# ZYM-PKU/UDiffText

Hardware: AMD Instinct MI355X
Metric: 512x512 50-step denoised images/sec (UDiffText hot path: conditioner + 50 CFG Euler steps + VAE decode) (higher is better)
Workload: dtype bf16; 1 GPU; 512x512, 50 Euler/DDIM(eta 0) steps, CFG 5.0, 9-char labels, noise_iters 0; global batch 4 per step sharded over 1 GPU(s) = 4 images per GPU in micro-batches of 4: every UNet call runs ONE batch of 4 (8 samples with CFG); 3 such batch(es) in flight per GPU on separate launch streams; BASELINE.json configs[1]; global_batch=4, weights=synthetic (name-keyed recipe), 1361.2 M parameters, launch=hipGraph replay of the sampler steps, in_flight=3, batches_per_unet_call=1

## Files before the change

### include/udt_kernels.h

```cpp
#ifndef UDT_KERNELS_H
#define UDT_KERNELS_H

#include <stddef.h>
#include <stdint.h>

#ifdef __cplusplus
extern "C" {
#endif

typedef enum {
  UDT_OK = 0,
  UDT_ERR_BAD_SHAPE = -1,
  UDT_ERR_BAD_ARG = -2,
  UDT_ERR_WORKSPACE = -3,
  UDT_ERR_HIP = -4,
  UDT_ERR_NO_DEVICE = -5,
  UDT_ERR_ASYNC = -6
} udt_status;

typedef enum {
  UDT_DTYPE_F32 = 0,
  UDT_DTYPE_BF16 = 1,
  UDT_DTYPE_FP8_E4M3 = 2
} udt_dtype;

#define UDT_GEMM_OUT_F32     (1 << 0)
#define UDT_GEMM_GEGLU       (1 << 1)
#define UDT_GEMM_RELU        (1 << 2)
#define UDT_GEMM_TRANSPOSED  (1 << 3)
#define UDT_GEMM_CONV        (1 << 4)
#define UDT_GEMM_SILU_OUT    (1 << 5)
#define UDT_GEMM_MX8         (1 << 7)

typedef struct {
  const void* a;
  const void* a2;
  const void* w;
  const float* bias;
  const void* residual;
  const float* rowvec;
  void* out;
  int32_t M, N, K;
  int32_t lda, ldo, ldr;
  int32_t ldw;
  int32_t batch;
  int64_t stride_a, stride_w, stride_out, stride_res;
  int32_t Hin, Win, C1, C2, Hout, Wout;
  int32_t ksize;
  int32_t stride;
  int32_t pad_t, pad_l;
  int32_t upsample;
  int32_t rows_per_batch;
  int32_t ld_rowvec;
  int32_t flags;
  float alpha;
  const float* colscale;
  const float* in_scsh;
  int32_t in_act;
  float* colstats;
  int32_t cu_share;
  const float* ln_colsum;
  float ln_eps;
  const void* a_scale;
  void* q8_out;
  void* q8_scale;
  int32_t ld_q8;
  int32_t q8_fixed_col;
  float q8_fixed_mul;
  float* rowstat_out;
  const float* rowstat_in;
  int32_t rowstat_in_parts;
} udt_gemm_desc;

size_t udt_gemm_workspace_bytes(const udt_gemm_desc* d);
int udt_gemm(const udt_gemm_desc* d, void* workspace, size_t workspace_bytes, void* stream);
int32_t udt_gemm_colstats_rows(const udt_gemm_desc* d);
int32_t udt_gemm_rowstat_parts(const udt_gemm_desc* d);
int32_t udt_gemm_q8_ok(const udt_gemm_desc* d);
int32_t udt_gemm_colstats_slots(const udt_gemm_desc* d);
int32_t udt_gemm_in_scsh_ok(const udt_gemm_desc* d);
int32_t udt_gemm_up4_ok(const udt_gemm_desc* d);
int udt_gn_silu_conv3x3_fwd(const udt_gemm_desc* d, void* workspace, size_t workspace_bytes, void* stream);
int udt_ln_gemm_fwd(const udt_gemm_desc* d, void* workspace, size_t workspace_bytes, void* stream);
int udt_check_async_error(void* workspace, size_t workspace_bytes, void* stream);

int udt_attn_fwd(const void* q, const void* k, const void* vt, void* o,
                 int32_t batch, int32_t heads, int32_t nq, int32_t nk,
                 int32_t ldq, int32_t ldk, int32_t ldvt, int32_t ldo,
                 int64_t q_bstride, int64_t k_bstride, int64_t vt_bstride, int64_t o_bstride,
                 float scale, void* stream);

int udt_xattn_fwd(const void* q, const void* k, const void* v, void* o, float* probs,
                  int32_t batch, int32_t heads, int32_t head_dim, int32_t nq, int32_t L,
                  int32_t ldq, int32_t ldkv, int32_t ldo, float scale, void* stream);

int udt_attn_rowv_fwd(const void* q, const void* k, const void* v, void* o,
                      int32_t batch, int32_t heads, int32_t nq, int32_t nk,
                      int32_t ldq, int32_t ldk, int32_t ldv, int32_t ldo,
                      int64_t q_bstride, int64_t k_bstride, int64_t v_bstride, int64_t o_bstride,
                      float scale, void* stream);
int udt_attn_rowv_q8_fwd(const void* q, const void* k, const void* v, void* o,
                         int32_t batch, int32_t heads, int32_t nq, int32_t nk,
                         int32_t ldq, int32_t ldk, int32_t ldv, int32_t ldo,
                         int64_t q_bstride, int64_t k_bstride, int64_t v_bstride, int64_t o_bstride,
                         float scale, void* q8_out, void* q8_scale, int32_t ld_q8, void* stream);

int udt_attn_mx8_fwd(const void* qkv8, const void* qkv_scale, void* o, int32_t batch, int32_t heads, int32_t n,
                     int32_t ld8, int32_t ldo, float scale, float v_inv, void* q8_out, void* q8_scale, int32_t ld_q8,
                     void* stream);

int udt_attn512_fwd(const void* q, const void* k, const void* v, void* o,
                    int32_t batch, int32_t nq, int32_t nk,
                    int32_t ldq, int32_t ldk, int32_t ldv, int32_t ldo,
                    int64_t q_bstride, int64_t k_bstride, int64_t v_bstride, int64_t o_bstride,
                    float scale, void* stream);

size_t udt_attn512_workspace_bytes(int32_t batch, int32_t nq, int32_t nk);
int udt_attn512_split_fwd(const void* q, const void* k, const void* v, void* o,
                          int32_t batch, int32_t nq, int32_t nk,
                          int32_t ldq, int32_t ldk, int32_t ldv, int32_t ldo,
                          int64_t q_bstride, int64_t k_bstride, int64_t v_bstride, int64_t o_bstride,
                          float scale, void* workspace, size_t workspace_bytes, void* stream);

int udt_mattn_fwd(const void* q, const void* k, const void* v, void* o, const float* mask, const uint8_t* kpm,
                  int32_t batch, int32_t heads, int32_t head_dim, int32_t nq, int32_t lk,
                  int32_t ldq, int32_t ldk, int32_t ldv, int32_t ldo, int32_t ldmask,
                  int64_t q_bstride, int64_t k_bstride, int64_t v_bstride, int64_t o_bstride, float scale, void* stream);

int32_t udt_tattn_hp(int32_t heads);
int udt_tattn_prepare(const void* kv, int32_t ldkv, const void* wq, int32_t ldwq, const void* wo, int32_t ldwo,
                      const float* gamma, const float* beta, void* A, float* sc, void* BmT, int32_t B, int32_t L,
                      int32_t C, int32_t heads, float scale, void* stream);
int udt_tattn_fused(const void* x, void* out, const void* A, const float* sc, const void* BmT, const float* bias,
                    int32_t B, int32_t n_tok, int32_t C, int32_t heads, int32_t zero_samples, float eps, void* stream);
int32_t udt_tattn_rowstat_parts(int32_t B, int32_t n_tok, int32_t C);
int udt_tattn_fused_q8(const void* x, void* out, const void* A, const float* sc, const void* BmT, const float* bias,
                       int32_t B, int32_t n_tok, int32_t C, int32_t heads, int32_t zero_samples, float eps, void* q8_out,
                       void* q8_scale, float* rowstat_out, void* stream);
int udt_tattn_fused_maps(const void* x, void* out, const void* A, const float* sc, const void* BmT, const float* bias,
                         int32_t B, int32_t n_tok, int32_t C, int32_t heads, int32_t zero_samples, float eps, float* maps,
                         int32_t L, int32_t map_from, float weight, int32_t accumulate, void* q8_out, void* q8_scale,
                         float* rowstat_out, void* stream);

int udt_softmax_rows(void* x, int64_t rows, int32_t cols, int32_t ld, void* stream);

int32_t udt_gn_nchunks(int64_t HW, int32_t C);
int udt_gn_stats(const void* x, const void* x2, float* partials, int32_t B, int64_t HW, int32_t C, int32_t C2,
                 int32_t G, void* stream);
int udt_gn_apply(const void* x, const void* x2, void* y, const float* partials, const float* gamma,
                 const float* beta, int32_t B, int64_t HW, int32_t C, int32_t C2, int32_t G, float eps, int32_t act,
                 void* stream);
int32_t udt_gn_strip_ok(int32_t B, int64_t HW, int32_t C1, int32_t C2, int32_t G);
int udt_gn_strip(const void* x, const void* x2, void* y, const float* gamma, const float* beta, int32_t B, int64_t HW,
                 int32_t C1, int32_t C2, int32_t G, float eps, int32_t act, void* stream);

int udt_gn_finalize(const float* stats1, int32_t slots1, int32_t C1, const float* stats2, int32_t slots2, int32_t C2,
                    const float* gamma, const float* beta, float* scsh, int32_t B, int64_t HW, int32_t G, float eps,
                    void* stream);

int udt_gn_apply_scsh(const void* x, const void* x2, void* y, const float* scsh, int32_t B, int64_t HW, int32_t C1,
                      int32_t C2, int32_t act, void* stream);

int udt_gn_strip_stats(const void* x, const void* x2, void* y, const float* stats1, int32_t slots1, const float* stats2,
                       int32_t slots2, const float* gamma, const float* beta, int32_t B, int64_t HW, int32_t C1, int32_t C2,
                       int32_t G, float eps, int32_t act, void* stream);

int udt_layernorm(const void* x, void* y, const float* gamma, const float* beta,
                  int64_t rows, int32_t C, float eps, void* stream);
int udt_unet_input(const float* x, void* xin, int32_t B, int32_t hw, int32_t cpad, float c_in, void* stream);
int udt_unet_input_churn(float* x, const float* noise, void* xin, int32_t B, int32_t hw, int32_t cpad, float c_in, float kn,
                         void* stream);
int udt_cfg_euler_step(float* x, const float* eps, float* denoised_out, int32_t B, int32_t hw, int32_t ld_eps,
                       float c_out, float sigma, float sigma_next, float cfg_scale, void* stream);
typedef struct {
  float kx, kd, ka, kp, kn;
  float c_out, scale;
} udt_sampler_coefs;
int udt_cfg_sampler_step(const float* xin, const float* eps, const float* aux, const float* prev, const float* noise,
                         float* xout, float* denoised_out, int32_t B, int32_t hw, int32_t ld_eps, udt_sampler_coefs k,
                         void* stream);
#define UDT_MULTISTEP_MAX 8
typedef struct {
  float c_out, scale, sigma;
  int32_t n;
  float k[UDT_MULTISTEP_MAX];
  const float* hist[UDT_MULTISTEP_MAX];
} udt_multistep_coefs;
// ... 178 lines not shown
```

### udifftext_amd/csrc/gemm.hip

```cpp
#include "common.h"
#include <stdio.h>
#include <stdlib.h>
#include <string.h>
#include <atomic>
#include <cmath>

hipError_t udt_lean_launch_gemm(int cfg, const void* lparams, int smem, int G, int geglu, int ln, hipStream_t s);
hipError_t udt_lean_launch_conv3(const void* c3params, hipStream_t s);

namespace {
#include "tile_common.h"

struct GemmParams {
  const uint16_t* a;
  const uint16_t* a2;
  const uint16_t* w;
  const uint16_t* zero;
  const float* bias;
  const uint16_t* res;
  const float* rowvec;
  void* out;
  const float* colscale;
  const float* in_scsh;
  float* colstats;
// ... 345 lines not shown

template <int BM, int BN, int WGM, int WGN, bool TRANS>
__global__ void __launch_bounds__(256) gemm_fixup_kernel(const GemmParams p) {
  const int tile = blockIdx.x;
  const long long it0 = (long long)tile * p.n_ktiles;
  const long long it1 = it0 + p.n_ktiles;
  const int g_first = (int)(it0 / p.iters_per_wg);
  const int g_last = (int)((it1 - 1) / p.iters_per_wg);
  if (g_first == g_last) return;
  const int tid = threadIdx.x;
  const int wave = tid >> 6;
  const int lane = tid & 63;
  const int wm = (WGN == 1) ? wave : (wave >> 1);
  const int wn = (WGN == 1) ? 0 : ((WGM == 1) ? wave : (wave & 1));
  f32x16 acc[2][2];
#pragma unroll
  for (int i = 0; i < 2; ++i)
#pragma unroll
    for (int j = 0; j < 2; ++j)
#pragma unroll
      for (int r = 0; r < 16; ++r) acc[i][j][r] = 0.f;
  for (int g = g_first; g <= g_last; ++g) {
    const long long gb = (long long)g * p.iters_per_wg;
    const int slot = (it0 <= gb) ? 0 : 1;
    const f32x4* slab = reinterpret_cast<const f32x4*>(p.slabs) + ((long long)g * 2 + slot) * (16 * 256);
#pragma unroll
    for (int tm = 0; tm < 2; ++tm)
#pragma unroll
      for (int tn = 0; tn < 2; ++tn)
#pragma unroll
        for (int q = 0; q < 4; ++q) {
          const f32x4 v = slab[(tm * 8 + tn * 4 + q) * 256 + tid];
#pragma unroll
          for (int r = 0; r < 4; ++r) acc[tm][tn][q * 4 + r] += v[r];
        }
  }
  int batch, m0, n0;
  decode_tile<BM, BN>(p, tile, batch, m0, n0);
  epilogue<TRANS>(p, acc, m0, n0, batch, wm, wn, lane);
}

#include "gemm8.h"
#include "conv3p.h"
#include "conv_n4.h"
#include "lean_params.h"

struct TilePlan {
  int bm, bn;
  int tiles_m, tiles_n, tiles;
  int nkt;
  long long total;
  int G, ipw;
  bool fixup;
};

constexpr int MAX_DEVICES = 16;
std::atomic<int> g_dev_cus[MAX_DEVICES];

int device_cus() {
  int dev = 0;
  if (hipGetDevice(&dev) != hipSuccess || dev < 0 || dev >= MAX_DEVICES) return 256;
  int v = g_dev_cus[dev].load(std::memory_order_relaxed);
  if (v == 0) {
    v = 256;
    int q = 0;
    if (hipDeviceGetAttribute(&q, hipDeviceAttributeMultiprocessorCount, dev) == hipSuccess && q > 0) v = q;
    g_dev_cus[dev].store(v, std::memory_order_relaxed);
  }
  return v;
}

int resident_slots_all() { return 2 * device_cus(); }

int resident_slots(const udt_gemm_desc* d) {
  const int share = d->cu_share > 0 ? d->cu_share : 1;
  const int s = resident_slots_all() / share;
  return s < 2 ? 2 : s;
}

TilePlan plan_tiles(const udt_gemm_desc* d) {
  TilePlan t;
  const int batch = d->batch > 0 ? d->batch : 1;
  const bool tall = d->M >= 1024;
  if (d->N <= 64 || (tall && (d->N % 128) != 0 && (d->N % 128) <= 64)) {
    t.bm = 256; t.bn = 64;
  } else {
    t.bm = 128; t.bn = 128;
  }
  if (d->flags & (UDT_GEMM_TRANSPOSED | UDT_GEMM_GEGLU)) { t.bm = 128; t.bn = 128; }
  t.tiles_m = (d->M + t.bm - 1) / t.bm;
  t.tiles_n = (d->N + t.bn - 1) / t.bn;
  t.tiles = t.tiles_m * t.tiles_n * batch;
  t.nkt = d->K / BK;
  t.total = (long long)t.tiles * t.nkt;
  const int slots = resident_slots(d);
  const long long share = (t.total + slots - 1) / slots;
  if (t.tiles < slots / 2 && t.nkt >= 16) {
    long long G = t.total / 8;
    if (G < 1) G = 1;
    if (G > slots) G = slots;
    t.ipw = (int)((t.total + G - 1) / G);
  } else if (t.tiles >= 8 * slots) {
    t.ipw = ((t.tiles + slots - 1) / slots) * t.nkt;
  } else if (share >= 160 && (t.tiles % slots) != 0) {
    t.ipw = (int)share;
  } else {
    t.ipw = t.nkt;
  }
  t.G = (int)((t.total + t.ipw - 1) / t.ipw);
  t.fixup = (t.ipw % t.nkt) != 0;
  return t;
}

template <int BM, int BN, int WGM, int WGN, bool CONV, bool TRANS>
hipError_t launch_cfg(const GemmParams& p, const TilePlan& t, hipStream_t s) {
  constexpr int smem = 2 * (BM + BN) * ROW_BYTES;
  static AttrOnce once;
  auto kern = gemm_kernel<BM, BN, WGM, WGN, CONV, TRANS>;
  hipError_t e = once.ensure(reinterpret_cast<const void*>(kern), smem);
  if (e != hipSuccess) return e;
  hipLaunchKernelGGL(kern, dim3(t.G), dim3(256), smem, s, p);
  e = hipGetLastError();
  if (e != hipSuccess) return e;
  if (t.fixup) {
    hipLaunchKernelGGL((gemm_fixup_kernel<BM, BN, WGM, WGN, TRANS>), dim3(t.tiles), dim3(256), 0, s, p);
    e = hipGetLastError();
  }
  return e;
}

constexpr size_t G8_HEADER_BYTES = 4096;

std::atomic<int> g_n_block{-1};
std::atomic<int> g_rows_epi{1};
#ifdef UDT_MEASURE
std::atomic<int> g_dbg_bits{0};
#endif
constexpr int INTERNAL_DIRECT_EPI = 1 << 30;
constexpr int PUBLIC_FLAGS = UDT_GEMM_OUT_F32 | UDT_GEMM_GEGLU | UDT_GEMM_RELU | UDT_GEMM_TRANSPOSED | UDT_GEMM_CONV |
                             UDT_GEMM_SILU_OUT | UDT_GEMM_MX8;
inline int k_tile(const udt_gemm_desc* d) { return (d->flags & UDT_GEMM_MX8) ? 128 : BK; }
inline int elem_bytes(const udt_gemm_desc* d) { return (d->flags & UDT_GEMM_MX8) ? 1 : 2; }

bool use_gemm8(const udt_gemm_desc* d) {
  if (d->N <= 64) return false;
  const long long ldw = d->ldw > 0 ? d->ldw : d->K;
  if (!(d->flags & UDT_GEMM_CONV) && (long long)d->M * d->lda * elem_bytes(d) >= (1LL << 31)) return false;
  return (long long)d->N * ldw * elem_bytes(d) < (1LL << 31);
}


int round_workgroups(int G) { return G > 8 ? ((G + 7) & ~7) : G; }

bool prefer_whole_tiles(const udt_gemm_desc* d, int tiles) {
  if (d->cu_share <= 1) return false;
  return (long long)tiles * 4 >= (long long)(resident_slots(d) / 2) * 3;
}

TilePlan plan_tiles8(const udt_gemm_desc* d) {
  TilePlan t;
  const int batch = d->batch > 0 ? d->batch : 1;
  const bool geglu_or_trans = (d->flags & (UDT_GEMM_TRANSPOSED | UDT_GEMM_GEGLU)) != 0;
  t.bm = 256;
  t.bn = (!geglu_or_trans && d->N % 160 == 0 && d->N % 128 != 0) ? 160 : 128;
  t.tiles_m = (d->M + t.bm - 1) / t.bm;
  t.tiles_n = (d->N + t.bn - 1) / t.bn;
  t.tiles = t.tiles_m * t.tiles_n * batch;
  t.nkt = d->K / k_tile(d);
  t.total = (long long)t.tiles * t.nkt;
  const bool whole = t.nkt < 24 || prefer_whole_tiles(d, t.tiles);
  int slots = (whole ? resident_slots_all() : resident_slots(d)) / 2;
  long long G = t.total / 4;
  if (G < 1) G = 1;
  if (G > slots) G = slots;
  t.ipw = (int)((t.total + G - 1) / G);
  if (whole) t.ipw = ((t.ipw + t.nkt - 1) / t.nkt) * t.nkt;
  t.G = round_workgroups((int)((t.total + t.ipw - 1) / t.ipw));
  t.fixup = (t.ipw % t.nkt) != 0;
  return t;
}

template <int WGM, int WGN, int TM, int TN, bool CONV, bool TRANS, bool STATS = false>
hipError_t launch8(const g8::Params& pp, const TilePlan& t, hipStream_t s) {
  constexpr int BM = WGM * TM * 32, BN = WGN * TN * 32;
  constexpr int smem = (TM == 2 && TN == 2 && !TRANS) ? 160 * 1024 : g8::NSTAGE * (BM + BN) * ROW_BYTES;
  static AttrOnce once;
  auto kern = g8::gemm8_kernel<WGM, WGN, TM, TN, CONV, TRANS, STATS>;
  hipError_t e = once.ensure(reinterpret_cast<const void*>(kern), smem);
  if (e != hipSuccess) return e;
  hipLaunchKernelGGL(kern, dim3(t.G), dim3(g8::NTHREADS), smem, s, pp);
  return hipGetLastError();
}

bool conv3p_geometry(const udt_gemm_desc* d, c3p::Geo& ge, bool gn) {
  if (!gn) return false;
  if (!(d->flags & UDT_GEMM_CONV) || d->ksize != 3 || d->stride != 1) return false;
  const bool ups = d->upsample != 0;
  if (ups) return false;
  if (d->pad_t != 1 || d->pad_l != 1 || d->N <= 64) return false;
  if (d->Hout != (d->Hin << (ups ? 1 : 0)) || d->Wout != (d->Win << (ups ? 1 : 0))) return false;
  if (d->flags & (UDT_GEMM_GEGLU | UDT_GEMM_TRANSPOSED)) return false;
  if (d->C1 <= 0 || d->C1 % 64 != 0 || d->C2 < 0 || d->C2 % 64 != 0 || (d->C2 != 0 && !gn)) return false;
  const int H = d->Hout, W = d->Wout;
  if (W % 32 == 0 && H % 8 == 0) { ge.TW = 32; ge.TH = 8; ge.NI = 1; }
  else if (W % 16 == 0 && H % 16 == 0) { ge.TW = 16; ge.TH = 16; ge.NI = 1; }
  else if (W == 8 && H == 8 && !ups) { ge.TW = 8; ge.TH = 8; ge.NI = 4; }
  else return false;
  ge.B = d->M / (H * W);
  ge.H = d->Hin; ge.W = d->Win; ge.C1 = d->C1; ge.C2 = d->C2; ge.C = d->C1 + d->C2;
  ge.tiles_x = W / ge.TW;
  ge.tiles_y = H / ge.TH;
  ge.img_groups = (ge.B + ge.NI - 1) / ge.NI;
  ge.prow_w = (ups ? ge.TW / 2 : ge.TW) + 2;
  ge.prows_img = ((ups ? ge.TH / 2 : ge.TH) + 2) * ge.prow_w;
  ge.n_pieces = (ge.NI * ge.prows_img + 7) / 8;
  ge.chunks = ge.C / 64;
  if ((long long)d->M * d->C1 * 2 >= (1LL << 31) || (long long)d->M * d->C2 * 2 >= (1LL << 31) || d->M >= (1 << 28)) return false;
  if ((long long)d->N * (d->ldw > 0 ? d->ldw : d->K) * 2 >= (1LL << 31)) return false;
  if ((long long)ge.B * ge.chunks * 512 >= (1LL << 31)) return false;
  const int bn = (d->N % 160 == 0 && d->N % 128 != 0) ? 160 : 128;
  return ge.n_pieces * 8 <= c3p::patch_rows(bn == 160 ? 5 : 2, gn) && ge.n_pieces >= 8;
}

TilePlan plan_tiles3p(const udt_gemm_desc* d, const c3p::Geo& ge) {
  TilePlan t;
  t.bm = 256;
  t.bn = (d->N % 160 == 0 && d->N % 128 != 0) ? 160 : 128;
  t.tiles_m = ge.img_groups * ge.tiles_y * ge.tiles_x;
  t.tiles_n = (d->N + t.bn - 1) / t.bn;
  t.tiles = t.tiles_m * t.tiles_n;
  t.nkt = ge.chunks;
  t.total = (long long)t.tiles * t.nkt;
  const bool whole = t.nkt * 9 < 24 || prefer_whole_tiles(d, t.tiles);
  const int slots = (whole ? resident_slots_all() : resident_slots(d)) / 2;
  long long G = t.total;
  if (G > slots) G = slots;
  t.ipw = (int)((t.total + G - 1) / G);
  if (whole) t.ipw = ((t.ipw + t.nkt - 1) / t.nkt) * t.nkt;
  t.G = round_workgroups((int)((t.total + t.ipw - 1) / t.ipw));
  t.fixup = (t.ipw % t.nkt) != 0;
  return t;
}

template <int WGM, int WGN, int TM, int TN, bool GN, bool STATS, bool UPS = false>
hipError_t launch3p(const c3p::CParams& cp, const TilePlan& t, hipStream_t s) {
  constexpr int BN = WGN * TN * 32;
  constexpr int smem = g8::NSTAGE * BN * ROW_BYTES + 2 * c3p::patch_rows(TN, GN) * ROW_BYTES + (GN ? c3p::SCSH_BYTES : 0);
  static_assert(smem <= 160 * 1024, "one workgroup per CU: at most the CU's 160 KiB of LDS");
  static AttrOnce once;
  auto kern = c3p::conv3p_kernel<WGM, WGN, TM, TN, GN, STATS, UPS>;
  hipError_t e = once.ensure(reinterpret_cast<const void*>(kern), smem);
  if (e != hipSuccess) return e;
  hipLaunchKernelGGL(kern, dim3(t.G), dim3(g8::NTHREADS), smem, s, cp);
  return hipGetLastError();
}

struct LeanPlan;
bool lean_stats_probe(const udt_gemm_desc* d, int& rows, int& slots);
int colstats_rows(const udt_gemm_desc* d) {
  if (d->flags & (UDT_GEMM_OUT_F32 | UDT_GEMM_GEGLU | UDT_GEMM_TRANSPOSED)) return 0;
  if ((d->batch > 1) || d->M <= 0 || d->N <= 0 || d->K <= 0 || d->K % BK != 0) return 0;
  int rows = 0, slots = 0;
  if (lean_stats_probe(d, rows, slots)) return rows;
  c3p::Geo ge;
  if (conv3p_geometry(d, ge, d->in_scsh != nullptr)) {
    rows = (d->N % 160 == 0 && d->N % 128 != 0) ? 32 : 64;
    if ((ge.TW * ge.TH) % rows != 0) return 0;
  } else if (use_gemm8(d) && g_rows_epi.load(std::memory_order_relaxed)) {
    rows = (plan_tiles8(d).bn == 160) ? 32 : 64;
  } else {
    return 0;
  }
  const int rpb = d->rows_per_batch > 0 ? d->rows_per_batch : d->M;
  return (rpb % rows == 0) ? rows : 0;
}

int colstats_slots(const udt_gemm_desc* d) {
  const int rows = colstats_rows(d);
  if (rows == 0) return 0;
  int lrows = 0, lslots = 0;
  if (lean_stats_probe(d, lrows, lslots)) return lslots;
  c3p::Geo ge;
  if (conv3p_geometry(d, ge, d->in_scsh != nullptr)) return ge.img_groups * ge.tiles_y * ge.tiles_x * (256 / rows);
  return ((d->M + 255) / 256) * (256 / rows);
}


std::atomic<int> g_lean{-1};
std::atomic<int> g_lean_splitk{-2};
int lean_splitk_knob() {
  int v = g_lean_splitk.load(std::memory_order_relaxed);
  if (v == -2) {
    const char* e = getenv("UDT_LEAN_SPLITK");
    v = e ? atoi(e) : -1;
// ... 67 lines not shown
  if (d->residual || d->rowvec || d->in_scsh || d->colstats || d->colscale || d->batch > 1 || d->alpha != 1.0f) return false;
  if ((d->ldw > 0 ? d->ldw : d->K) % 8 != 0 || (d->ldw > 0 && d->ldw < d->K)) return false;
  if (d->K != 9 * d->C1 || (d->lda != 0 && d->lda != d->C1) || d->q8_out || d->q8_scale || d->rowstat_out || d->in_act != 0) return false;
  if ((reinterpret_cast<uintptr_t>(d->a) | reinterpret_cast<uintptr_t>(d->w) | reinterpret_cast<uintptr_t>(d->out)) & 15) return false;
  return true;
}

bool lean_plan(const udt_gemm_desc* d, LeanPlan& t, bool want_stats) {
  const int mode = lean_mode();
  if (mode == 0) return false;
  constexpr int unsupported = UDT_GEMM_OUT_F32 | UDT_GEMM_RELU | UDT_GEMM_TRANSPOSED | UDT_GEMM_SILU_OUT;
  if (d->flags & unsupported) return false;
  const bool conv1 = (d->flags & UDT_GEMM_CONV) != 0;
  if (conv1 && (d->ksize != 1 || d->stride != 1 || d->upsample || d->pad_t != 0 || d->pad_l != 0 || d->Hout != d->Hin ||
                d->Wout != d->Win || d->C1 % BK != 0 || d->C2 % BK != 0 || d->ln_colsum || (d->flags & UDT_GEMM_GEGLU)))
    return false;
  const bool mx8 = (d->flags & UDT_GEMM_MX8) != 0;
  const bool emit = d->q8_out != nullptr;
  if (d->batch > 1 || d->in_scsh || (d->colscale != nullptr) != mx8) return false;
  const bool geglu = (d->flags & UDT_GEMM_GEGLU) != 0;
  const bool ln = d->ln_colsum != nullptr;
  if (want_stats && (geglu || ln || !lean_stats_enabled())) return false;
  if (mx8 || emit) {
    if (conv1 || d->rowvec || mode == 0 || (mode > 0 && mode != 1)) return false;
    if (mx8 && (!d->a_scale || d->K % 128 != 0 || d->lda % 16 != 0 || (d->ldw > 0 && d->ldw % 16 != 0))) return false;
    if (mx8 && ln && (!d->rowstat_in || d->rowstat_in_parts <= 0)) return false;
    if (!mx8 && geglu) return false;
    if (mx8 && geglu && !(ln && emit)) return false;
    if (mx8 && !geglu && ln && emit && d->rowstat_out) return false;
    if (emit && (want_stats || !d->q8_scale || d->ld_q8 % 8 != 0 || d->N % (geglu ? 64 : 32) != 0)) return false;
    if (d->rowstat_out && (!emit || geglu)) return false;
    if (d->q8_fixed_col > 0 && (!emit || geglu || d->q8_fixed_col % 32 != 0 || !(d->q8_fixed_mul > 0.f))) return false;
    if ((reinterpret_cast<uintptr_t>(d->q8_out) | reinterpret_cast<uintptr_t>(d->colscale)) & 15) return false;
  } else if (d->rowstat_out || d->rowstat_in) {
    return false;
  }
  const int KT = mx8 ? 128 : BK;
  if (d->N <= 64 || d->N % 8 != 0 || d->K % KT != 0 || (!conv1 && d->lda % 8 != 0) || (d->ldo % 8 != 0 && d->out)) return false;
  if (d->residual && d->ldr % 8 != 0) return false;
  if (geglu && (d->N % 64 != 0 || d->residual || d->rowvec)) return false;
  const long long ldw = d->ldw > 0 ? d->ldw : d->K;
  const long long lda_eff = conv1 ? (d->C1 > d->C2 ? d->C1 : d->C2) : d->lda;
  if ((long long)d->M * lda_eff * 2 >= (1LL << 31) || (long long)d->N * ldw * 2 >= (1LL << 31)) return false;
  if (d->M >= (1 << 28)) return false;
  if ((reinterpret_cast<uintptr_t>(d->out) | reinterpret_cast<uintptr_t>(d->residual) | reinterpret_cast<uintptr_t>(d->bias) |
       reinterpret_cast<uintptr_t>(d->rowvec) | reinterpret_cast<uintptr_t>(d->ln_colsum)) & 15) return false;
  if (d->rowvec && ((d->ld_rowvec > 0 ? d->ld_rowvec : d->N) % 4 != 0)) return false;
  if (mode > 0 && mode != 1 && mode != 6 && mode != 7) return false;
  if (!mx8 && (!emit || (ln && !geglu && !d->rowstat_out)) && (mode == 7 || (mode < 0 && rowres_on()))) {
    const bool emit_fits = !emit || ((d->q8_fixed_col <= 0 || d->q8_fixed_col % 64 == 0) && (long long)d->M * d->ld_q8 < (1LL << 31) &&
                                     (long long)d->M * (d->out ? d->ldo : 0) * 2 < (1LL << 31) && (long long)((d->N + 127) / 128) * d->M * 4 < (1LL << 31));
    if (ln && !want_stats && d->K == 320 && d->N % 64 == 0 && !d->residual && !d->rowvec && !conv1 && emit_fits &&
        (reinterpret_cast<uintptr_t>(d->a) & 15) == 0) {
      const int tiles_m = (d->M + 255) / 256, chunks = d->N / 64;
      int ns = (device_cus() + tiles_m - 1) / tiles_m;
      if (ns > chunks / 4) ns = chunks / 4;
      const int cmax = geglu ? 20 : 16;
      const int ns_min = (chunks + cmax - 1) / cmax;
      if (ns < ns_min) ns = ns_min;
      const long long wgs = (long long)tiles_m * ns;
      if (ns >= 1 && (mode == 7 || emit || (geglu ? wgs * 4 >= 3LL * device_cus() : wgs >= device_cus()))) {
        t.cfg = 7; t.stats_rows = 0; t.nw = 4; t.bm = 256; t.bn = 64; t.smem = 0;
        t.tiles_m = tiles_m; t.kt_per = (chunks + ns - 1) / ns; t.tiles_n = (chunks + t.kt_per - 1) / t.kt_per;
        t.tiles = t.tiles_m * t.tiles_n; t.nkt = d->K / BK; t.splitk = 1; t.n_block = 1;
        t.G = round_workgroups(t.tiles);
        return true;
      }
    }
    if (mode == 7 || (emit && ln)) return false;
  }
  t.cfg = (mode > 0) ? mode : 1;
  if (!mx8 && !emit) {
  if (!geglu && d->N % 160 == 0 && d->N % 128 != 0 && t.cfg == 1) t.cfg = 5;
  if (mode <= 0 && d->N >= 768 && (long long)((d->M + 255) / 256) * ((d->N + 255) / 256) >= 2LL * device_cus() &&
      (d->cu_share <= 1 || lean256_under_lanes())) t.cfg = 6;
  }
  t.stats_rows = 0;
  if (want_stats) {
    if (t.cfg != 1 && t.cfg != 5) {
      if (mode > 0) return false;
      t.cfg = (d->N % 160 == 0 && d->N % 128 != 0) ? 5 : 1;
    }
    if (mx8) t.cfg = 1;
    t.stats_rows = t.cfg == 1 ? 64 : 32;
    const int rpb = d->rows_per_batch > 0 ? d->rows_per_batch : d->M;
    if (rpb % t.stats_rows != 0) return false;
  }
  switch (t.cfg) {
    case 1: t.nw = 4; t.bm = 128; t.bn = 128; t.smem = 2 * (128 + 128) * ROW_BYTES; break;
    case 5: t.nw = 4; t.bm = 128; t.bn = 160; t.smem = 128 * 160 * 4; break;
    case 6: t.nw = 8; t.bm = 256; t.bn = 256; t.smem = 2 * (256 + 256) * ROW_BYTES; break;
    default: return false;
  }
  {
    const int epi = (t.cfg == 6 ? t.bm * t.bn : t.bm * t.bn * 4) + ((ln && t.cfg != 5) ? t.bm * 8 : 0);
    if (t.smem < epi) t.smem = epi;
  }
  t.tiles_m = (d->M + t.bm - 1) / t.bm;
  t.tiles_n = (d->N + t.bn - 1) / t.bn;
  t.tiles = t.tiles_m * t.tiles_n;
  t.nkt = d->K / KT;
  int slots = device_cus() * ((t.cfg == 1 || t.cfg == 5) ? 2 : 1) / share_of(d);
  if (slots < 1) slots = 1;
  int sk = 1;
  const int knob = lean_splitk_knob();
  if (!ln && t.tiles <= 1023) {
    if (knob > 1) sk = knob;
    else if (knob < 0 && t.tiles * 2 <= slots && t.nkt >= (mx8 ? 20 : 40)) { sk = slots / t.tiles; if (sk > t.nkt / (mx8 ? 8 : 16)) sk = t.nkt / (mx8 ? 8 : 16); }
    if (sk > t.nkt / 4) sk = t.nkt / 4;
    while (sk > 1 && (long long)t.tiles * sk * t.bm * t.bn * 4 > (64LL << 20)) --sk;
    if (sk < 1) sk = 1;
  }
  t.kt_per = (t.nkt + sk - 1) / sk;
  t.splitk = (t.nkt + t.kt_per - 1) / t.kt_per;
  const int units = t.tiles * t.splitk;
  t.G = round_workgroups(units);
  int nb = g_n_block.load(std::memory_order_relaxed);
  if (nb <= 0) nb = (t.tiles_m <= 8) ? t.tiles_n : 8;
  if (nb > t.tiles_n) nb = t.tiles_n;
  t.n_block = nb;
  return true;
}

size_t lean_workspace(const LeanPlan& t) {
  return t.splitk > 1 ? G8_HEADER_BYTES + (size_t)t.tiles * t.splitk * t.bm * t.bn * sizeof(float) : 0;
}

std::atomic<int> g_lean_conv{-1};
std::atomic<int> g_wide_conv{-2};
int wide_conv_mode() {
  int v = g_wide_conv.load(std::memory_order_relaxed);
  if (v == -2) {
    const char* e = getenv("UDT_WIDE_CONV");
    v = e ? atoi(e) : -1;
    g_wide_conv.store(v, std::memory_order_relaxed);
  }
  return v;
}
#ifdef UDT_MEASURE
std::atomic<int> g_lconv_dbg{0};
#endif

std::atomic<int> g_wide_lanes_eff{-2};
double wide_lanes_eff() {
  int v = g_wide_lanes_eff.load(std::memory_order_relaxed);
  if (v == -2) {
    const char* e = getenv("UDT_WIDE_LANES_EFF");
    v = e ? atoi(e) : 70;
    g_wide_lanes_eff.store(v, std::memory_order_relaxed);
  }
  return v / 100.0;
}

int conv_chunk_slices(long long tiles, int slots, int chunks, int knob) {
  long long sk = 1;
  if (tiles <= 1023) {
    if (knob > 1) { sk = knob; if (sk > chunks) sk = chunks; }
    else if (knob < 0 && tiles * 2 <= slots && chunks >= 10) { sk = slots / tiles; if (sk > chunks / 4) sk = chunks / 4; }
    if (sk < 1) sk = 1;
  }
  return (int)sk;
}

bool lean_conv_plan(const udt_gemm_desc* d, lg::C3Params& c, bool want_stats) {
  int on = g_lean_conv.load(std::memory_order_relaxed);
  if (on < 0) {
    const char* e = getenv("UDT_LEAN_CONV");
    on = (e && e[0] == '0') ? 0 : 1;
    g_lean_conv.store(on, std::memory_order_relaxed);
  }
  if (!on || lean_mode() == 0) return false;
  if (d->flags != UDT_GEMM_CONV || d->ksize != 3 || d->stride != 1 || d->pad_t != 1 || d->pad_l != 1) return false;
  if (d->C2 != 0 || d->in_scsh || d->colscale || d->batch > 1) return false;
  if (want_stats && !lean_stats_enabled()) return false;
  if (d->N < 128 || d->N % 8 != 0 || d->C1 <= 0 || d->C1 % 64 != 0) return false;
  if (d->upsample != 0 && d->upsample != 1 && d->upsample != 2) return false;
  const bool phase = d->upsample == 2, ups = d->upsample == 1;
  const int nph = phase ? 4 : 1;
  if (d->Hout != (d->Hin << (d->upsample ? 1 : 0)) || d->Wout != (d->Win << (d->upsample ? 1 : 0))) return false;
  if (phase && d->ldw > 0 && d->ldw < 4 * d->C1) return false;
  const int Ht = phase ? d->Hin : d->Hout, Wt = phase ? d->Win : d->Wout;
  c.bn = 128; c.wgm = 2;
  bool wide = false;
  int wide_slots = device_cus();
  {
    const int wm = wide_conv_mode();
    if (wm != 0 && !ups && d->N % 160 == 0 && Wt % 16 == 0 && Ht % 16 == 0) {
      const int cus = device_cus(), share = d->cu_share > 1 ? d->cu_share : 1;
      wide_slots = cus / share > 0 ? cus / share : 1;
      const long long wt = (long long)(d->M / 256) * (d->N / 160);
      const long long sk = conv_chunk_slices(wt, wide_slots, d->C1 / 64, lean_splitk_knob());
      const long long units = wt * sk;
      const long long rounds = (units + cus - 1) / cus;
      const double eff = units > cus ? (double)units / (double)(rounds * cus) : ((double)units * share >= cus ? 1.0 : (double)units * share / cus);
      wide = (wm > 0) || (sk <= 2 && eff >= ((share >= 3 && share_of(d) >= 3) ? wide_lanes_eff() : 0.85));
    }
  }
  if (wide) { c.geo = phase ? 6 : 3; c.tw = 16; c.th = 16; c.bn = 160; c.wgm = 4; }
  else if (Wt % 16 == 0 && Ht % 8 == 0) { c.geo = ups ? 2 : phase ? 4 : 0; c.tw = 16; c.th = 8; }
  else if (!ups && Wt % 8 == 0 && Ht % 8 == 0) { c.geo = phase ? 5 : 1; c.tw = 8; c.th = 8; }
  else return false;
  if (d->ldo % 8 != 0 || (d->residual && d->ldr % 8 != 0)) return false;
  const long long ldw = d->ldw > 0 ? d->ldw : (phase ? 4LL * d->C1 : (long long)d->K);
  if (ldw % 8 != 0) return false;
  c.w_phase = phase ? (d->stride_w > 0 ? d->stride_w : (long long)d->N * ldw) : 0;
  if (phase && (c.w_phase < (long long)d->N * ldw || c.w_phase % 8 != 0)) return false;
  if ((long long)d->M * d->C1 * 2 >= (1LL << 31) || (long long)d->N * ldw * 2 >= (1LL << 31)) return false;
  if ((reinterpret_cast<uintptr_t>(d->out) | reinterpret_cast<uintptr_t>(d->residual) | reinterpret_cast<uintptr_t>(d->bias) |
       reinterpret_cast<uintptr_t>(d->rowvec)) & 15) return false;
  if (d->rowvec && ((d->ld_rowvec > 0 ? d->ld_rowvec : d->N) % 4 != 0)) return false;
  c.dbg = 0;
#ifdef UDT_MEASURE
  c.dbg = g_lconv_dbg.load(std::memory_order_relaxed);
#endif
  c.N = d->N; c.C = d->C1; c.H = d->Hin; c.W = d->Win; c.B = d->M / (d->Hout * d->Wout);
  c.ldw = (int)ldw; c.ldo = d->ldo; c.ldr = d->ldr; c.ldrv = d->ld_rowvec > 0 ? d->ld_rowvec : d->N;
  c.alpha = d->alpha;
  c.tiles_x = Wt / c.tw; c.tiles_y = Ht / c.th;
  c.tiles_m = c.B * c.tiles_x * c.tiles_y;
  c.tiles_n = (d->N + c.bn - 1) / c.bn;
  c.tiles = c.tiles_m * c.tiles_n;
  c.chunks = c.C / 64;
  const int slots = wide ? wide_slots : (2 * device_cus() / share_of(d) > 0 ? 2 * device_cus() / share_of(d) : 1);
  int sk = conv_chunk_slices((long long)c.tiles * nph, slots, c.chunks, lean_splitk_knob());
  while (sk > 1 && (long long)c.tiles * nph * sk * c.tw * c.th * c.bn * 4 > (64LL << 20)) --sk;
  c.ch_per = (c.chunks + sk - 1) / sk;
  c.splitk = (c.chunks + c.ch_per - 1) / c.ch_per;
  c.G = round_workgroups(c.tiles * nph * c.splitk);
  {
    const double patch = (double)((ups ? c.tw / 2 : c.tw) + 2) * ((ups ? c.th / 2 : c.th) + 2) * c.C * 2.0, wtile = (phase ? 4.0 : 9.0) * c.bn * c.C * 2.0;
    int nb = g_n_block.load(std::memory_order_relaxed);
    if (nb <= 0) nb = (int)(std::sqrt(64.0 * patch / wtile) + 0.5);
    if (nb < 1) nb = 1;
    if (nb > c.tiles_n) nb = c.tiles_n;
    c.n_block = nb;
  }
  c.a_bytes = (unsigned)((long long)c.B * d->Hin * d->Win * d->C1 * 2);
  c.w_bytes = (unsigned)((long long)d->N * ldw * 2);
  c.counters = nullptr; c.slabs = nullptr;
  return true;
}

int lean_conv_phases(const lg::C3Params& c) { return c.geo >= 4 ? 4 : 1; }

size_t lean_conv_workspace(const lg::C3Params& c) {
  return c.splitk > 1 ? G8_HEADER_BYTES + (size_t)c.tiles * lean_conv_phases(c) * c.splitk * c.tw * c.th * c.bn * sizeof(float) : 0;
}

bool lean_stats_probe(const udt_gemm_desc* d, int& rows, int& slots) {
  if (d->in_scsh) return false;
  {
    lg::C3Params c3;
    if (lean_conv_plan(d, c3, true)) {
      rows = c3.tw * c3.th / c3.wgm;
      slots = c3.tiles_m * c3.wgm * lean_conv_phases(c3);
      return true;
    }
  }
  if ((d->flags & UDT_GEMM_CONV) && d->ksize == 3) return false;
  LeanPlan lt;
  if (lean_plan(d, lt, true)) {
    rows = lt.stats_rows;
    slots = lt.tiles_m * (lt.bm / lt.stats_rows);
    return true;
  }
  return false;
}
}

extern "C" int udt_debug_set(const char* key, int32_t value) {
  if (!key) return UDT_ERR_BAD_ARG;
  if (!strcmp(key, "n_block")) { g_n_block.store(value); return UDT_OK; }
  if (!strcmp(key, "rows_epi")) { g_rows_epi.store(value ? 1 : 0); return UDT_OK; }
  if (!strcmp(key, "lean")) { g_lean.store(value < 0 ? -2 : value); return UDT_OK; }
  if (!strcmp(key, "rowres")) { g_rowres.store(value < 0 ? 1 : (value ? 1 : 0)); return UDT_OK; }
  if (!strcmp(key, "wide_lanes_eff")) { g_wide_lanes_eff.store(value < 0 ? -2 : value); return UDT_OK; }
  if (!strcmp(key, "conv_n4")) { g_conv_n4.store(value < 0 ? -2 : (value ? 1 : 0)); return UDT_OK; }
  if (!strcmp(key, "lean256_lanes")) { g_lean256_lanes.store(value < 0 ? -2 : (value ? 1 : 0)); return UDT_OK; }
// ... 88 lines not shown
      return G8_HEADER_BYTES + (size_t)t3.G * t3.bm * t3.bn * sizeof(float);
    }
  }
  if (use_gemm8(d)) {
    TilePlan t8 = plan_tiles8(d);
    if (!t8.fixup) return 0;
    return G8_HEADER_BYTES + (size_t)t8.G * t8.bm * t8.bn * sizeof(float);
  }
  TilePlan t = plan_tiles(d);
  if (t.bm != 256 || !t.fixup) return 0;
  return G8_HEADER_BYTES + (size_t)t.G * 2 * SLAB_FLOATS * sizeof(float);
}

extern "C" int udt_gemm(const udt_gemm_desc* d, void* workspace, size_t workspace_bytes, void* stream) {
  if (!d || !d->a || !d->w) return UDT_ERR_BAD_ARG;
  if (d->M <= 0 || d->N <= 0 || d->K <= 0) return UDT_ERR_BAD_SHAPE;
  if (d->K % k_tile(d) != 0) return UDT_ERR_BAD_SHAPE;
  if (d->N % 4 != 0) return UDT_ERR_BAD_SHAPE;
  const bool mx8 = (d->flags & UDT_GEMM_MX8) != 0;
  if (mx8 || d->q8_out || d->rowstat_out || d->rowstat_in) {
    LeanPlan lt8;
    if (!lean_plan(d, lt8, d->colstats != nullptr)) return UDT_ERR_BAD_ARG;
  } else if (d->colscale) {
    return UDT_ERR_BAD_ARG;
  }
  const bool conv = (d->flags & UDT_GEMM_CONV) != 0;
  const bool trans = (d->flags & UDT_GEMM_TRANSPOSED) != 0;
  const int batch = d->batch > 0 ? d->batch : 1;
  if (conv) {
    if (d->ksize != 1 && d->ksize != 3) return UDT_ERR_BAD_SHAPE;
    if (d->C1 <= 0 || d->C1 % BK != 0 || d->C2 % BK != 0) return UDT_ERR_BAD_SHAPE;
    if (d->C2 > 0 && !d->a2) return UDT_ERR_BAD_ARG;
    if (d->K != d->ksize * d->ksize * (d->C1 + d->C2)) return UDT_ERR_BAD_SHAPE;
    if (d->Hout <= 0 || d->Wout <= 0 || d->M % (d->Hout * d->Wout) != 0) return UDT_ERR_BAD_SHAPE;
    if (d->stride != 1 && d->stride != 2) return UDT_ERR_BAD_SHAPE;
    if (trans || batch != 1) return UDT_ERR_BAD_ARG;
  } else {
    if (d->lda < d->K || d->lda % 8 != 0) return UDT_ERR_BAD_SHAPE;
  }
  if (!d->out && !d->q8_out) return UDT_ERR_BAD_ARG;
  if (trans) {
    if (d->rows_per_batch <= 0 || d->rows_per_batch % 4 != 0 || d->M % d->rows_per_batch != 0)
      return UDT_ERR_BAD_SHAPE;
    if (d->flags & (UDT_GEMM_OUT_F32 | UDT_GEMM_GEGLU | UDT_GEMM_RELU | UDT_GEMM_SILU_OUT)) return UDT_ERR_BAD_ARG;
    if (d->residual || d->rowvec || batch != 1) return UDT_ERR_BAD_ARG;
  } else {
    if (d->ldo % 4 != 0) return UDT_ERR_BAD_SHAPE;
    if (d->residual && d->ldr % 4 != 0) return UDT_ERR_BAD_SHAPE;
  }
  if (d->flags & UDT_GEMM_GEGLU) {
    if (d->N % 64 != 0 || (d->flags & UDT_GEMM_OUT_F32) || d->residual || d->rowvec) return UDT_ERR_BAD_ARG;
  }
  if (d->rowvec && d->rows_per_batch <= 0) return UDT_ERR_BAD_ARG;

  hipStream_t s = reinterpret_cast<hipStream_t>(stream);
  if (conv_n4_applies(d)) {
    cn4::Params cp;
    cp.a = reinterpret_cast<const uint16_t*>(d->a); cp.w = reinterpret_cast<const uint16_t*>(d->w); cp.bias = d->bias;
    cp.out = reinterpret_cast<float*>(d->out);
    cp.B = d->M / (d->Hout * d->Wout); cp.H = d->Hin; cp.W = d->Win; cp.C = d->C1;
    cp.ldw = d->ldw > 0 ? d->ldw : d->K; cp.ldo = d->ldo;
    cp.tiles_x = (d->Win + 7) / 8; cp.tiles_y = (d->Hin + 7) / 8;
    const size_t smem = (size_t)100 * (d->C1 + 8) * 2 + (size_t)4 * 9 * d->C1 * 2;
    static AttrOnce once;
    hipError_t ea = once.ensure(reinterpret_cast<const void*>(cn4::conv3x3_n4_kernel), 100 * (512 + 8) * 2 + 4 * 9 * 512 * 2);
    if (ea != hipSuccess) return udt_set_hip_error(ea);
    UdtProfScope profn(0, s);
    if (profn.rec) {
      char tag[96];
      snprintf(tag, sizeof(tag), "conv_n4 M=%d N=%d K=%d %dx%d", d->M, d->N, d->K, d->Hin, d->Win);
      udt_prof_tag(profn.rec, tag);
    }
    hipLaunchKernelGGL(cn4::conv3x3_n4_kernel, dim3((unsigned)(cp.B * cp.tiles_x * cp.tiles_y)), dim3(256), smem, s, cp);
    UDT_CHECK_LAUNCH();
    return UDT_OK;
  }
  TilePlan t = plan_tiles(d);

  GemmParams p;
  p.a = reinterpret_cast<const uint16_t*>(d->a);
  p.a2 = reinterpret_cast<const uint16_t*>(d->a2);
  p.w = reinterpret_cast<const uint16_t*>(d->w);
  p.zero = udt_zero_page();
  if (!p.zero) return UDT_ERR_HIP;
  p.bias = d->bias;
  p.res = reinterpret_cast<const uint16_t*>(d->residual);
  p.rowvec = d->rowvec;
  p.out = d->out;
  p.colscale = d->colscale;
  p.in_scsh = d->in_scsh;
  p.in_act = d->in_act;
  p.colstats = d->colstats;
  p.slabs = nullptr;
  if (d->colstats && colstats_rows(d) == 0) return UDT_ERR_BAD_ARG;
  if (d->in_scsh && !udt_gemm_in_scsh_ok(d)) return UDT_ERR_BAD_ARG;
  if (d->in_act != 0 && d->in_act != 1) return UDT_ERR_BAD_ARG;
  p.M = d->M; p.N = d->N; p.K = d->K;
  p.lda = d->lda; p.ldo = d->ldo; p.ldr = d->ldr;
  p.ldw = d->ldw > 0 ? d->ldw : d->K;
  if (d->upsample == 2) {
    if (!udt_gemm_up4_ok(d)) return UDT_ERR_BAD_SHAPE;
  } else if (p.ldw < d->K || p.ldw % 8 != 0) return UDT_ERR_BAD_SHAPE;
  if (mx8 && d->lda < d->K) return UDT_ERR_BAD_SHAPE;
  p.sA = d->stride_a; p.sW = d->stride_w; p.sO = d->stride_out; p.sR = d->stride_res;
  p.Hin = d->Hin; p.Win = d->Win; p.C1 = d->C1; p.C2 = d->C2; p.Hout = d->Hout; p.Wout = d->Wout;
  p.ksz = d->ksize; p.stride = d->stride; p.pad_t = d->pad_t; p.pad_l = d->pad_l; p.ups = d->upsample ? 1 : 0;
  p.rows_per_batch = d->rows_per_batch > 0 ? d->rows_per_batch : d->M;
  p.ldrv = d->ld_rowvec > 0 ? d->ld_rowvec : d->N;
  if (d->flags & ~PUBLIC_FLAGS) return UDT_ERR_BAD_ARG;
  p.flags = d->flags | (g_rows_epi.load(std::memory_order_relaxed) ? 0 : INTERNAL_DIRECT_EPI);
#ifdef UDT_MEASURE
  p.flags |= g_dbg_bits.load(std::memory_order_relaxed);
#endif
  p.n_block = 1;
  p.alpha = d->alpha;
  const int cls = (conv && d->ksize == 3) ? 0 : 1;
  {
    LeanPlan lt;
    if (lean_plan(d, lt, d->colstats != nullptr)) {
      lg::LParams lp;
      lp.colstats = d->colstats;
      const bool conv1 = (d->flags & UDT_GEMM_CONV) != 0;
      lp.a = p.a; lp.a2 = (conv1 && d->C2 > 0) ? p.a2 : nullptr; lp.w = p.w; lp.bias = p.bias; lp.res = p.res; lp.rowvec = p.rowvec;
      lp.ln_s = d->ln_colsum;
      lp.out = reinterpret_cast<uint16_t*>(d->out);
      lp.M = d->M; lp.N = d->N; lp.K = d->K;
      lp.lda = conv1 ? d->C1 : p.lda; lp.ldw = p.ldw; lp.ldo = p.ldo; lp.ldr = p.ldr; lp.ldrv = p.ldrv; lp.rows_per_batch = p.rows_per_batch;
      lp.lda2 = conv1 ? d->C2 : 0;
      lp.kt_split = (conv1 && d->C2 > 0) ? d->C1 / BK : lt.nkt;
      lp.a2_bytes = (unsigned)((long long)d->M * (conv1 ? d->C2 : 0) * 2);
      lp.alpha = d->alpha; lp.ln_eps = d->ln_eps;
      lp.tiles_m = lt.tiles_m; lp.tiles_n = lt.tiles_n; lp.n_block = lt.n_block; lp.tiles = lt.tiles;
      lp.nkt = lt.nkt; lp.splitk = lt.splitk; lp.kt_per = lt.kt_per;
      lp.a_bytes = (unsigned)((long long)d->M * lp.lda * elem_bytes(d));
      lp.w_bytes = (unsigned)((long long)d->N * p.ldw * elem_bytes(d));
      lp.a_scale = mx8 ? reinterpret_cast<const uint32_t*>(d->a_scale) : nullptr;
      lp.colscale = d->colscale;
      lp.rowstat_in = d->rowstat_in; lp.rowstat_in_parts = d->rowstat_in_parts;
      lp.q8_out = reinterpret_cast<uint8_t*>(d->q8_out); lp.q8_scale = reinterpret_cast<uint32_t*>(d->q8_scale); lp.ld_q8 = d->ld_q8;
      lp.rowstat_out = d->rowstat_out;
      lp.q8_fixed_col = d->q8_fixed_col > 0 ? d->q8_fixed_col : 0x7fffffff;
      lp.q8_fixed_mul = d->q8_fixed_mul;
      lp.G = lt.G;
      lp.counters = nullptr; lp.slabs = nullptr;
      if (lt.splitk > 1) {
        if (!workspace || workspace_bytes < lean_workspace(lt)) return UDT_ERR_WORKSPACE;
        lp.counters = reinterpret_cast<int*>(workspace);
        lp.slabs = reinterpret_cast<float*>(reinterpret_cast<char*>(workspace) + G8_HEADER_BYTES);
      }
      UdtProfScope profl(cls, s);
      if (profl.rec) {
        char tag[96];
        snprintf(tag, sizeof(tag), "lean%d%s%s M=%d N=%d K=%d fl=0x%x ln=%d tile=%dx%d units=%d splitk=%d", lt.cfg, mx8 ? "-mx8" : "", d->q8_out ? "+q8" : "",
                 d->M, d->N, d->K, d->flags, d->ln_colsum ? 1 : 0, lt.bm, lt.bn, lt.tiles * lt.splitk, lt.splitk);
        udt_prof_tag(profl.rec, tag);
      }
      const bool geglu = (d->flags & UDT_GEMM_GEGLU) != 0, ln = d->ln_colsum != nullptr;
      hipError_t el;
      el = udt_lean_launch_gemm(lt.cfg, &lp, lt.smem, lt.G, geglu ? 1 : 0, ln ? 1 : 0, s);
      if (el != hipSuccess) return udt_set_hip_error(el);
      return UDT_OK;
    }
  }
  if (d->ln_colsum) return UDT_ERR_BAD_ARG;
  {
    lg::C3Params c3;
    if (lean_conv_plan(d, c3, d->colstats != nullptr)) {
      c3.colstats = d->colstats;
      c3.a = p.a; c3.w = p.w; c3.bias = p.bias; c3.res = p.res; c3.rowvec = p.rowvec; c3.out = reinterpret_cast<uint16_t*>(d->out);
      if (c3.splitk > 1) {
        if (!workspace || workspace_bytes < lean_conv_workspace(c3)) return UDT_ERR_WORKSPACE;
        c3.counters = reinterpret_cast<int*>(workspace);
        c3.slabs = reinterpret_cast<float*>(reinterpret_cast<char*>(workspace) + G8_HEADER_BYTES);
      }
      UdtProfScope profc(cls, s);
      if (profc.rec) {
        char tag[96];
        snprintf(tag, sizeof(tag), "%s%s M=%d N=%d K=%d %dx%d tile=%dx%d units=%d splitk=%d nb=%d%s", (c3.geo == 3 || c3.geo == 6) ? "wconv3" : "lconv3",
                 (d->upsample && c3.geo != 6) ? "+up" : "", d->M, d->N, d->K,
                 d->Hin, d->Win, c3.tw, c3.th, c3.tiles * lean_conv_phases(c3) * c3.splitk, c3.splitk, c3.n_block,
                 d->upsample == 2 ? " up4" : "");
        udt_prof_tag(profc.rec, tag);
      }
      const hipError_t ec = udt_lean_launch_conv3(&c3, s);
      if (ec != hipSuccess) return udt_set_hip_error(ec);
      return UDT_OK;
    }
  }
  {
    c3p::CParams cp;
    if (conv3p_geometry(d, cp.geo, d->in_scsh != nullptr)) {
      const TilePlan t3 = plan_tiles3p(d, cp.geo);
      p.tiles_m = t3.tiles_m; p.tiles_n = t3.tiles_n; p.tiles_per_batch = t3.tiles_m * t3.tiles_n;
      {
        const double patch = (double)cp.geo.prows_img * cp.geo.NI * cp.geo.C * 2.0;
        const double wtile = 9.0 * t3.bn * cp.geo.C * 2.0;
        const double S = (double)(t3.tiles < t3.G ? t3.tiles : t3.G) / 8.0;
        int nb = (int)(std::sqrt((S < 1.0 ? 1.0 : S) * patch / wtile) + 0.5);
        if (nb < 1) nb = 1;
        if (nb > t3.tiles_n) nb = t3.tiles_n;
        p.n_block = nb;
      }
      p.n_ktiles = t3.nkt;
      p.total_iters = t3.total;
      p.iters_per_wg = t3.ipw;
      p.G = t3.G;
      const long long in_px = (long long)cp.geo.B * d->Hin * d->Win;
      cp.base.a_bytes = (unsigned)(in_px * d->C1 * 2);
      cp.a2_bytes = (unsigned)((long long)d->M * d->C2 * 2);
      cp.scsh_bytes = (unsigned)((long long)cp.geo.B * cp.geo.chunks * 512);
      cp.base.w_bytes = (unsigned)((long long)d->N * p.ldw * 2);
      cp.base.g = p;
      cp.base.flags = nullptr; cp.base.err = nullptr; cp.base.slab_base = nullptr;
      if (t3.fixup) {
        const size_t need = G8_HEADER_BYTES + (size_t)t3.G * t3.bm * t3.bn * sizeof(float);
        if (!workspace || workspace_bytes < need) return UDT_ERR_WORKSPACE;
        cp.base.flags = reinterpret_cast<int*>(workspace);
        cp.base.err = cp.base.flags + 1023;
        cp.base.slab_base = reinterpret_cast<float*>(reinterpret_cast<char*>(workspace) + G8_HEADER_BYTES);
      }
      UdtProfScope prof3(cls, s);
      if (prof3.rec) {
        char tag[96];
        snprintf(tag, sizeof(tag), "conv3p%s%s M=%d N=%d K=%d %dx%d tile=%dx%dx%d bn=%d G=%d ipw=%d", d->in_scsh ? "+gn" : "", d->upsample ? "+up" : "", d->M,
                 d->N, d->K, d->Hin, d->Win, cp.geo.TW, cp.geo.TH, cp.geo.NI, t3.bn, t3.G, t3.ipw);
        udt_prof_tag(prof3.rec, tag);
      }
      hipError_t e3;
      const bool st3 = d->colstats != nullptr;
      if (t3.bn == 160) e3 = st3 ? launch3p<8, 1, 1, 5, true, true>(cp, t3, s) : launch3p<8, 1, 1, 5, true, false>(cp, t3, s);
      else e3 = st3 ? launch3p<4, 2, 2, 2, true, true>(cp, t3, s) : launch3p<4, 2, 2, 2, true, false>(cp, t3, s);
      if (e3 != hipSuccess) return udt_set_hip_error(e3);
      return UDT_OK;
    }
  }
  if (use_gemm8(d)) {
    const TilePlan t8 = plan_tiles8(d);
    p.tiles_m = t8.tiles_m; p.tiles_n = t8.tiles_n; p.tiles_per_batch = t8.tiles_m * t8.tiles_n;
    const int n_block_knob = g_n_block.load(std::memory_order_relaxed);
    if (n_block_knob != 0 && !conv) {
      const long long wt = (long long)t8.bn * d->K * elem_bytes(d);
      long long nb = 1;
      if (n_block_knob > 0) nb = n_block_knob;
      else if (t8.tiles_m <= 8 || trans) nb = t8.tiles_n;
      else if (t8.tiles_n >= 8) nb = (4LL << 20) / (wt > 0 ? wt : 1);
      if (nb < 1) nb = 1;
      if (nb > t8.tiles_n) nb = t8.tiles_n;
      p.n_block = (int)nb;
    }
    p.n_ktiles = t8.nkt;
    p.total_iters = t8.total;
    p.iters_per_wg = t8.ipw;
    p.G = t8.G;
    g8::Params pp;
    pp.g = p;
    pp.flags = nullptr; pp.err = nullptr; pp.slab_base = nullptr;
    pp.a_bytes = conv ? 0u : (unsigned)((long long)d->M * d->lda * elem_bytes(d));
    pp.w_bytes = (unsigned)((long long)d->N * p.ldw * elem_bytes(d));
    if (t8.fixup) {
      const size_t need = G8_HEADER_BYTES + (size_t)t8.G * t8.bm * t8.bn * sizeof(float);
      if (!workspace || workspace_bytes < need) return UDT_ERR_WORKSPACE;
      pp.flags = reinterpret_cast<int*>(workspace);
      pp.err = pp.flags + 1023;
      pp.slab_base = reinterpret_cast<float*>(reinterpret_cast<char*>(workspace) + G8_HEADER_BYTES);
    }
    UdtProfScope prof8(cls, s);
    if (prof8.rec) {
      char tag[96];
      snprintf(tag, sizeof(tag), "gemm8 M=%d N=%d K=%d conv=%d ks=%d fl=0x%x tile=%dx%d G=%d ipw=%d b=%d",
               d->M, d->N, d->K, conv ? 1 : 0, d->ksize, d->flags, t8.bm, t8.bn, t8.G, t8.ipw, batch);
      udt_prof_tag(prof8.rec, tag);
    }
    hipError_t e8;
    const bool st = d->colstats != nullptr;
    if (t8.bn == 160) {
      if (st) e8 = conv ? launch8<8, 1, 1, 5, true, false, true>(pp, t8, s) : launch8<8, 1, 1, 5, false, false, true>(pp, t8, s);
      else e8 = conv ? launch8<8, 1, 1, 5, true, false>(pp, t8, s) : launch8<8, 1, 1, 5, false, false>(pp, t8, s);
    } else if (trans) {
      e8 = launch8<4, 2, 2, 2, false, true>(pp, t8, s);
    } else if (st) {
      e8 = conv ? launch8<4, 2, 2, 2, true, false, true>(pp, t8, s) : launch8<4, 2, 2, 2, false, false, true>(pp, t8, s);
    } else {
      e8 = conv ? launch8<4, 2, 2, 2, true, false>(pp, t8, s) : launch8<4, 2, 2, 2, false, false>(pp, t8, s);
    }
    if (e8 != hipSuccess) return udt_set_hip_error(e8);
    return UDT_OK;
  }

  p.tiles_m = t.tiles_m; p.tiles_n = t.tiles_n; p.tiles_per_batch = t.tiles_m * t.tiles_n;
  p.n_ktiles = t.nkt;
  p.total_iters = t.total;
  p.iters_per_wg = t.ipw;
  p.G = t.G;

  if (t.fixup) {
    const size_t need = G8_HEADER_BYTES + (size_t)t.G * 2 * SLAB_FLOATS * sizeof(float);
    if (!workspace || workspace_bytes < need) return UDT_ERR_WORKSPACE;
    p.slabs = reinterpret_cast<float*>(reinterpret_cast<char*>(workspace) + G8_HEADER_BYTES);
  }

  UdtProfScope prof(cls, s);
  if (prof.rec) {
    char tag[96];
    snprintf(tag, sizeof(tag), "gemm M=%d N=%d K=%d conv=%d ks=%d fl=0x%x tile=%dx%d G=%d ipw=%d b=%d", d->M, d->N, d->K,
             conv ? 1 : 0, d->ksize, d->flags, t.bm, t.bn, t.G, t.ipw, batch);
    udt_prof_tag(prof.rec, tag);
  }

  if (t.bm != 256) return UDT_ERR_BAD_SHAPE;
  const hipError_t e = conv ? launch_cfg<256, 64, 4, 1, true, false>(p, t, s) : launch_cfg<256, 64, 4, 1, false, false>(p, t, s);
  if (e != hipSuccess) return udt_set_hip_error(e);
  return UDT_OK;
}
```

### udifftext_amd/csrc/lean.h

```cpp
#pragma once

namespace lg {

using g8::wait_vm;
UDT_DEVINL void raw_barrier() {
  asm volatile("s_waitcnt lgkmcnt(0)" ::: "memory");
  __builtin_amdgcn_s_barrier();
  asm volatile("" ::: "memory");
}
using g8::buf_lds16;
using g8::OOB;

typedef __attribute__((ext_vector_type(2))) __bf16 bf2_t;
UDT_DEVINL float dot2_bf16(uint32_t a, uint32_t b, float c) {
  return __builtin_amdgcn_fdot2_f32_bf16(__builtin_bit_cast(bf2_t, a), __builtin_bit_cast(bf2_t, b), c, false);
}

template <int CPR, int RPI>
UDT_DEVINL void wave_colstats(char* wl, int lane, const float (&cs)[8], const float (&cq)[8], float* dst, bool col_ok) {
#pragma unroll
  for (int h = 0; h < 2; ++h) {
    f32x4 a = {cs[4 * h + 0], cs[4 * h + 1], cs[4 * h + 2], cs[4 * h + 3]};
    f32x4 b = {cq[4 * h + 0], cq[4 * h + 1], cq[4 * h + 2], cq[4 * h + 3]};
    *reinterpret_cast<f32x4*>(wl + lane * 64 + h * 16) = a;
// ... 404 lines not shown
        uint32_t sb;
        const u32x2 q8 = mx8_quant_row8(f, sb);
        if (m < p.M && col_ok) {
          *reinterpret_cast<u32x2*>(p.q8_out + (long long)m * p.ld_q8 + n_out) = q8;
          if (ch == 0) reinterpret_cast<uint8_t*>(p.q8_scale)[((long long)(n_out >> 7) * p.M + m) * 4 + ((n_out >> 5) & 3)] = (uint8_t)sb;
          if (p.out) *reinterpret_cast<u32x4*>(p.out + (long long)m * p.ldo + n_out) = v;
        }
      } else {
        if (m < p.M && col_ok) *reinterpret_cast<u32x4*>(p.out + (long long)m * p.ldo + n_out) = v;
      }
    }
  } else {
    char* const wl = smem + wave * EPI_WAVE;
    constexpr int PROWS = TMB * 32;
    constexpr int CPR = TN * 4;
    constexpr int RPI = 64 / CPR;
    constexpr int NIT = (PROWS + RPI - 1) / RPI;
    const int rl = lane / CPR;
    const int c8 = lane - rl * CPR;
    const int n = n0 + col0 + c8 * 8;
    const bool col_ok = (rl < RPI) && (n < p.N);
    f32x4 b0 = {0.f, 0.f, 0.f, 0.f}, b1 = b0, s0 = b0, s1 = b0;
    if (p.bias && col_ok) {
      b0 = *reinterpret_cast<const f32x4*>(p.bias + n);
      b1 = *reinterpret_cast<const f32x4*>(p.bias + n + 4);
    }
    if constexpr (LN) {
      if (col_ok) {
        s0 = *reinterpret_cast<const f32x4*>(p.ln_s + n);
        s1 = *reinterpret_cast<const f32x4*>(p.ln_s + n + 4);
      }
    }
    f32x4 w0 = {1.f, 1.f, 1.f, 1.f}, w1 = w0;
    if constexpr (FP8) {
      if (col_ok) {
        w0 = *reinterpret_cast<const f32x4*>(p.colscale + n);
        w1 = *reinterpret_cast<const f32x4*>(p.colscale + n + 4);
      }
    }
    float cs[8], cq[8];
#pragma unroll
    for (int j = 0; j < 8; ++j) cs[j] = cq[j] = 0.f;
#pragma unroll
    for (int pass = 0; pass < TM / TMB; ++pass) {
      const int prow0 = pass * PROWS;
      u32x4 rv[NIT];
      if (p.res) {
#pragma unroll
        for (int i = 0; i < NIT; ++i) {
          const int row = i * RPI + rl;
          const int m = m0 + row0 + prow0 + row;
          u32x4 z = {0u, 0u, 0u, 0u};
          rv[i] = z;
          if (col_ok && row < PROWS && m < p.M) rv[i] = *reinterpret_cast<const u32x4*>(p.res + (long long)m * p.ldr + n);
        }
      }
#pragma unroll
      for (int tb = 0; tb < TMB; ++tb) {
        const int row = tb * 32 + l31;
#pragma unroll
        for (int tn = 0; tn < TN; ++tn)
#pragma unroll
          for (int q = 0; q < 4; ++q) {
            const int chunk = (tn * 8 + q * 2 + hi) ^ (row & 7);
            const f32x16& a16 = acc[pass * TMB + tb][tn];
            f32x4 v = {a16[q * 4 + 0], a16[q * 4 + 1], a16[q * 4 + 2], a16[q * 4 + 3]};
            *reinterpret_cast<f32x4*>(wl + row * EROW + chunk * 16) = v;
          }
      }
#pragma unroll
      for (int i = 0; i < NIT; ++i) {
        const int row = i * RPI + rl;
        const int m = m0 + row0 + prow0 + row;
        const bool ok = col_ok && row < PROWS && m < p.M;
        const int rr = row < PROWS ? row : 0;
        const char* rp = wl + rr * EROW;
        const int sw = rr & 7;
        const f32x4 v0 = *reinterpret_cast<const f32x4*>(rp + (((2 * c8) ^ sw) << 4));
        const f32x4 v1 = *reinterpret_cast<const f32x4*>(rp + (((2 * c8 + 1) ^ sw) << 4));
        float o[8];
#pragma unroll
        for (int j = 0; j < 4; ++j) {
          o[j] = v0[j];
          o[4 + j] = v1[j];
        }
        if constexpr (FP8) {
#pragma unroll
          for (int j = 0; j < 4; ++j) o[j] *= w0[j], o[4 + j] *= w1[j];
        }
        if constexpr (LN) {
          float mean, rstd;
          row_stats(prow0 + rr, mean, rstd);
#pragma unroll
          for (int j = 0; j < 4; ++j) {
            o[j] = rstd * (o[j] - mean * s0[j]);
            o[4 + j] = rstd * (o[4 + j] - mean * s1[j]);
          }
        }
#pragma unroll
        for (int j = 0; j < 4; ++j) {
          o[j] = o[j] * p.alpha + b0[j];
          o[4 + j] = o[4 + j] * p.alpha + b1[j];
        }
        if (p.rowvec && ok) {
          const float* rvp = p.rowvec + (long long)(m / p.rows_per_batch) * p.ldrv + n;
          const f32x4 r0 = *reinterpret_cast<const f32x4*>(rvp);
          const f32x4 r1 = *reinterpret_cast<const f32x4*>(rvp + 4);
// ... 412 lines not shown
```

### udifftext_amd/csrc/lean_params.h

```cpp
#pragma once

namespace lg {

struct LParams {
  const uint16_t* a;
  const uint16_t* a2;
  const uint16_t* w;
  const float* bias;
  const uint16_t* res;
  const float* rowvec;
  const float* ln_s;
  uint16_t* out;
  int M, N, K;
  int lda, ldw, ldo, ldr, ldrv, rows_per_batch;
  float alpha, ln_eps;
  int tiles_m, tiles_n, n_block, tiles;
  int nkt;
  int splitk, kt_per;
  unsigned a_bytes, w_bytes;
  int kt_split, lda2;
  unsigned a2_bytes;
  int G;
  int* counters;
  float* slabs;
  float* colstats;
  const uint32_t* a_scale;
  const float* colscale;
  const float* rowstat_in;
  int rowstat_in_parts;
  uint8_t* q8_out;
  uint32_t* q8_scale;
  int ld_q8;
  int q8_fixed_col;
  float q8_fixed_mul;
  float* rowstat_out;
};

struct C3Params {
  const uint16_t* a;
  const uint16_t* w;
  const float* bias;
  const uint16_t* res;
  const float* rowvec;
  uint16_t* out;
  int N, C;
  int B, H, W;
  int ldw, ldo, ldr, ldrv;
  float alpha;
  int tiles_x, tiles_y, tiles_m, tiles_n, n_block, tiles;
  int chunks, splitk, ch_per;
  unsigned a_bytes, w_bytes;
  int G;
  int* counters;
  float* slabs;
  float* colstats;
  int geo, tw, th;
  int bn, wgm;
  long long w_phase;
  int dbg;
};

}
```

### udifftext_amd/csrc/tattn.hip

```cpp
#include "common.h"
#include <stdio.h>
#include <stdlib.h>

namespace {

constexpr int TA_THREADS = 512;
constexpr int TA_WAVES = TA_THREADS / 64;

struct TattnParams {
  const uint16_t* x;
  uint16_t* out;
  const uint16_t* A;
  const float* sc;
  const uint16_t* BmT;
  const float* bias;
  const uint16_t* zero;
  int M, C, hp, n_tok, zero_samples;
  int nsplit;
  float eps;
  uint8_t* q8_out;
  uint32_t* q8_scale;
  float* rowstat_out;
  float* maps;
  int heads, map_L, map_from, map_acc;
  float map_scale;
};

UDT_DEVINL f32x16 zero16() {
  f32x16 z;
#pragma unroll
  for (int r = 0; r < 16; ++r) z[r] = 0.f;
  return z;
}

template <int TT, int NKT, int NKS, bool Q8 = false, bool MAPS = false>
__global__ void __launch_bounds__(TA_THREADS) tattn_fused_kernel(const TattnParams p) {
  extern __shared__ __attribute__((aligned(16))) char smem[];
  constexpr int C = NKT * 64, hp = NKS * 16;
  constexpr int nkt = NKT;
  constexpr int TA_AHEAD = NKT <= 10 ? NKT : 8;
  char* const xs = smem;
  float* const stats = reinterpret_cast<float*>(smem + (size_t)nkt * TT * 128);
  const int prs = hp * 2 + 16;
  char* const pl = reinterpret_cast<char*>(stats + TT * 2);
  const int tid = threadIdx.x;
  const int wave = __builtin_amdgcn_readfirstlane(tid >> 6);
  const int lane = tid & 63;
  const int l31 = lane & 31, hi = lane >> 5;
  const long long tok0 = (long long)blockIdx.x * TT;
  const int b = (int)(tok0 / p.n_tok);
  const uint16_t* xg = p.x + tok0 * C;
  uint16_t* og = p.out + tok0 * C;
  float* const rst = reinterpret_cast<float*>(pl + (size_t)TT * prs);
  const int ct_lo = (int)blockIdx.y * (C >> 5) / p.nsplit, ct_hi = ((int)blockIdx.y + 1) * (C >> 5) / p.nsplit;
  auto q8_row_stats = [&]() {
    __syncthreads();
    if (tid < TT && tok0 + tid < p.M) {
      float s = 0.f, q = 0.f;
      for (int ct = ct_lo; ct < ct_hi; ++ct) {
        const f32x2 v = *reinterpret_cast<const f32x2*>(rst + ((size_t)tid * (C >> 5) + ct) * 2);
        s += v[0];
        q += v[1];
      }
      f32x2 o = {s, q};
      reinterpret_cast<f32x2*>(p.rowstat_out)[(long long)blockIdx.y * p.M + tok0 + tid] = o;
    }
  };


  const uint16_t* Ab = p.A + (long long)b * hp * C;
  constexpr int jt = hp >> 5;
  constexpr int tiles1 = jt * (TT / 32);
  bf16x8_t ar[TA_AHEAD][4];
  const bool live = b >= p.zero_samples;
  if (live && wave < tiles1) {
    const uint16_t* arow = Ab + (long long)(wave / (TT / 32)) * (32 * C) + lane * 8;
#pragma unroll
    for (int u = 0; u < TA_AHEAD; ++u)
#pragma unroll
      for (int ks = 0; ks < 4; ++ks) ar[u][ks] = *reinterpret_cast<const bf16x8_t*>(arow + (u * 4 + ks) * 512);
  }

  {
    const int pieces = nkt * (TT / 8);
    const int l3 = lane >> 3, ps = lane & 7;
    for (int pc = wave; pc < pieces; pc += TA_WAVES) {
      const int kt = pc / (TT / 8), rg = pc - kt * (TT / 8);
      const int row = rg * 8 + l3;
      const int slot = ps ^ ((row >> 1) & 7);
      const uint16_t* src = (tok0 + row < p.M) ? (xg + (long long)row * C + kt * 64 + slot * 8) : p.zero;
      glds16(src, xs + (size_t)pc * 1024);
    }
    wait_vmcnt0();
  }
  __syncthreads();

  if (b < p.zero_samples) {
    const int ch_lo = ct_lo * 4, ch_hi = ct_hi * 4;
    const int nch = ch_hi - ch_lo;
    for (int i0 = 0; i0 < TT * nch; i0 += TA_THREADS) {
      const int i = i0 + tid;
      const bool act = i < TT * nch;
      const int row = act ? i / nch : 0, ch = ch_lo + (act ? i - row * nch : 0);
      const bool ok = act && tok0 + row < p.M;
// ... 244 lines not shown
  const long long idx = (long long)blockIdx.x * 256 + threadIdx.x;
  if (idx >= (long long)B * C * hp) return;
  const int j = (int)(idx % hp);
  const long long bc = idx / hp;
  const int c = (int)(bc % C), b = (int)(bc / C);
  const int h = j >> 4, i = j & 15;
  float a = 0.f;
  if (h < heads && i < L) {
    const uint16_t* vr = kv + ((long long)b * L + i) * ldkv + v_off + h * 64;
    const uint16_t* wr = wo + (long long)c * ldwo + h * 64;
#pragma unroll 8
    for (int d = 0; d < 64; ++d) a += bf16_bits_to_f32(vr[d]) * bf16_bits_to_f32(wr[d]);
  }
  const long long off = ((((long long)(c >> 5) * (hp >> 4) + (j >> 4)) * 64) + ((j >> 3) & 1) * 32 + (c & 31)) * 8 + (j & 7);
  BmT[(long long)b * C * hp + off] = (uint16_t)(pack_bf16x2(a, 0.f) & 0xffffu);
}

}

extern "C" int32_t udt_tattn_hp(int32_t heads) { return ((heads * 16 + 31) / 32) * 32; }

extern "C" int udt_tattn_prepare(const void* kv, int32_t ldkv, const void* wq, int32_t ldwq, const void* wo, int32_t ldwo,
                                 const float* gamma, const float* beta, void* A, float* sc, void* BmT, int32_t B, int32_t L,
                                 int32_t C, int32_t heads, float scale, void* stream) {
  if (!kv || !wq || !wo || !gamma || !beta || !A || !sc || !BmT) return UDT_ERR_BAD_ARG;
  if (B <= 0 || L <= 0 || L > 12 || heads <= 0 || C != heads * 64 || ldkv < 2 * C || ldwq < C || ldwo < C) return UDT_ERR_BAD_SHAPE;
  const int hp = udt_tattn_hp(heads);
  hipStream_t s = reinterpret_cast<hipStream_t>(stream);
  UdtProfScope prof(3, s);
  hipLaunchKernelGGL(tattn_prepare_a_kernel, dim3(hp, B), dim3(256), 0, s, reinterpret_cast<const uint16_t*>(kv), ldkv,
                     reinterpret_cast<const uint16_t*>(wq), ldwq, gamma, beta, reinterpret_cast<uint16_t*>(A), sc, L, C, hp, heads, scale);
  UDT_CHECK_LAUNCH();
  const long long n = (long long)B * C * hp;
  hipLaunchKernelGGL(tattn_prepare_b_kernel, dim3((unsigned)((n + 255) / 256)), dim3(256), 0, s,
                     reinterpret_cast<const uint16_t*>(kv), ldkv, C, reinterpret_cast<const uint16_t*>(wo), ldwo,
                     reinterpret_cast<uint16_t*>(BmT), B, L, C, hp, heads);
  UDT_CHECK_LAUNCH();
  return UDT_OK;
}

namespace {
int tattn_tt(int C) { return C >= 640 ? 32 : 64; }
int tattn_nsplit(int M, int TT) {
  const unsigned grid = (unsigned)(M / TT);
  constexpr unsigned target = 256u;
  int nsplit = 1;
  while (nsplit < 8 && grid * nsplit < target) nsplit *= 2;
  return nsplit;
}

int tattn_launch(const void* x, void* out, const void* A, const float* sc, const void* BmT, const float* bias, int32_t B, int32_t n_tok,
                 int32_t C, int32_t heads, int32_t zero_samples, float eps, void* q8_out, void* q8_scale, float* rowstat_out, void* stream,
                 bool with_maps = false, float* maps = nullptr, int32_t L = 0, int32_t map_from = 0, float weight = 0.f,
                 int32_t accumulate = 0) {
  if (with_maps && !maps) return UDT_ERR_BAD_ARG;
  if (!x || !out || !bias || (zero_samples < B && (!A || !sc || !BmT))) return UDT_ERR_BAD_ARG;
  if (B <= 0 || n_tok <= 0 || heads <= 0 || C != heads * 64 || C > 1280 || zero_samples < 0 || zero_samples > B) return UDT_ERR_BAD_SHAPE;
  const int TT = tattn_tt(C);
  if (n_tok % TT != 0) return UDT_ERR_BAD_SHAPE;
  if (with_maps && (L < 1 || L > 12 || map_from < zero_samples || map_from > B)) return UDT_ERR_BAD_SHAPE;
  const bool q8 = q8_out != nullptr;
  if (q8 && (!q8_scale || !rowstat_out || C % 128 != 0)) return UDT_ERR_BAD_ARG;
  TattnParams p;
  p.x = reinterpret_cast<const uint16_t*>(x); p.out = reinterpret_cast<uint16_t*>(out);
  p.A = reinterpret_cast<const uint16_t*>(A); p.sc = sc; p.BmT = reinterpret_cast<const uint16_t*>(BmT); p.bias = bias;
  p.zero = udt_zero_page();
  if (!p.zero) return UDT_ERR_HIP;
  p.M = B * n_tok; p.C = C; p.hp = udt_tattn_hp(heads); p.n_tok = n_tok; p.zero_samples = zero_samples; p.eps = eps;
  p.q8_out = reinterpret_cast<uint8_t*>(q8_out); p.q8_scale = reinterpret_cast<uint32_t*>(q8_scale); p.rowstat_out = rowstat_out;
  p.maps = maps; p.heads = heads; p.map_L = L; p.map_from = map_from; p.map_acc = accumulate != 0; p.map_scale = weight / (float)heads;
  const size_t smem = (size_t)TT * C * 2 + (size_t)TT * 2 * sizeof(float) + (size_t)TT * (p.hp * 2 + 16) + (q8 ? (size_t)TT * (C / 32) * 8 : 0);
  hipStream_t s = reinterpret_cast<hipStream_t>(stream);
  UdtProfScope prof(3, s);
  if (prof.rec) {
    char tag[96];
    snprintf(tag, sizeof(tag), "tattn_fused%s%s B=%d n=%d C=%d zero=%d", q8 ? "+q8" : "", with_maps ? "+maps" : "", B, n_tok, C, zero_samples);
    udt_prof_tag(prof.rec, tag);
  }
  static bool attr_done[10] = {};
  const unsigned grid = (unsigned)(p.M / TT);
  p.nsplit = tattn_nsplit(p.M, TT);
  const void* fn = nullptr;
  int which = -1;
#define UDT_TATTN_FN(...) (with_maps ? reinterpret_cast<const void*>(tattn_fused_kernel<__VA_ARGS__, true>) : reinterpret_cast<const void*>(tattn_fused_kernel<__VA_ARGS__, false>))
  if (C == 320 && p.hp == 96 && !q8) { fn = UDT_TATTN_FN(64, 5, 6, false); which = 0; }
  else if (C == 640 && p.hp == 160) { fn = q8 ? UDT_TATTN_FN(32, 10, 10, true) : UDT_TATTN_FN(32, 10, 10, false); which = q8 ? 3 : 1; }
  else if (C == 1280 && p.hp == 320) { fn = q8 ? UDT_TATTN_FN(32, 20, 20, true) : UDT_TATTN_FN(32, 20, 20, false); which = q8 ? 4 : 2; }
#undef UDT_TATTN_FN
  else return UDT_ERR_BAD_SHAPE;
  if (with_maps) which += 5;
  if (!attr_done[which]) {
    hipError_t e = hipFuncSetAttribute(fn, hipFuncAttributeMaxDynamicSharedMemorySize, 128 * 1024);
    if (e != hipSuccess) return udt_set_hip_error(e);
    attr_done[which] = true;
  }
  void* args[] = {&p};
  hipError_t el = hipLaunchKernel(fn, dim3(grid, p.nsplit), dim3(TA_THREADS), args, smem, s);
  if (el != hipSuccess) return udt_set_hip_error(el);
  UDT_CHECK_LAUNCH();
  return UDT_OK;
}
}

extern "C" int udt_tattn_fused(const void* x, void* out, const void* A, const float* sc, const void* BmT, const float* bias,
                               int32_t B, int32_t n_tok, int32_t C, int32_t heads, int32_t zero_samples, float eps, void* stream) {
  return tattn_launch(x, out, A, sc, BmT, bias, B, n_tok, C, heads, zero_samples, eps, nullptr, nullptr, nullptr, stream);
}

extern "C" int32_t udt_tattn_rowstat_parts(int32_t B, int32_t n_tok, int32_t C) {
  if (B <= 0 || n_tok <= 0 || (C != 640 && C != 1280)) return 0;
  const int TT = tattn_tt(C);
  if (n_tok % TT != 0) return 0;
  return tattn_nsplit(B * n_tok, TT);
}

extern "C" int udt_tattn_fused_q8(const void* x, void* out, const void* A, const float* sc, const void* BmT, const float* bias,
                                  int32_t B, int32_t n_tok, int32_t C, int32_t heads, int32_t zero_samples, float eps, void* q8_out,
                                  void* q8_scale, float* rowstat_out, void* stream) {
  if (!q8_out) return UDT_ERR_BAD_ARG;
  return tattn_launch(x, out, A, sc, BmT, bias, B, n_tok, C, heads, zero_samples, eps, q8_out, q8_scale, rowstat_out, stream);
}

extern "C" int udt_tattn_fused_maps(const void* x, void* out, const void* A, const float* sc, const void* BmT, const float* bias,
                                    int32_t B, int32_t n_tok, int32_t C, int32_t heads, int32_t zero_samples, float eps, float* maps,
                                    int32_t L, int32_t map_from, float weight, int32_t accumulate, void* q8_out, void* q8_scale,
                                    float* rowstat_out, void* stream) {
  return tattn_launch(x, out, A, sc, BmT, bias, B, n_tok, C, heads, zero_samples, eps, q8_out, q8_scale, rowstat_out, stream, true, maps, L,
                      map_from, weight, accumulate);
}
```

### udifftext_amd/lib.py

```python
from __future__ import annotations

import ctypes as C
import os

_HERE = os.path.dirname(os.path.abspath(__file__))
LIB_PATH = os.path.join(_HERE, "libudt_kernels.so")

GEMM_OUT_F32 = 1 << 0
DTYPE_F32, DTYPE_BF16, DTYPE_FP8_E4M3 = 0, 1, 2
GEMM_GEGLU = 1 << 1
GEMM_RELU = 1 << 2
GEMM_TRANSPOSED = 1 << 3
GEMM_CONV = 1 << 4
GEMM_SILU_OUT = 1 << 5
GEMM_MX8 = 1 << 7

PROF_CONV3X3, PROF_GEMM, PROF_ATTN, PROF_XATTN, PROF_NORM, PROF_ELEMENTWISE = range(6)


class GemmDesc(C.Structure):
    _fields_ = [
        ("a", C.c_void_p), ("a2", C.c_void_p), ("w", C.c_void_p), ("bias", C.c_void_p),
        ("residual", C.c_void_p), ("rowvec", C.c_void_p), ("out", C.c_void_p),
        ("M", C.c_int32), ("N", C.c_int32), ("K", C.c_int32),
        ("lda", C.c_int32), ("ldo", C.c_int32), ("ldr", C.c_int32), ("ldw", C.c_int32),
        ("batch", C.c_int32),
        ("stride_a", C.c_int64), ("stride_w", C.c_int64), ("stride_out", C.c_int64), ("stride_res", C.c_int64),
        ("Hin", C.c_int32), ("Win", C.c_int32), ("C1", C.c_int32), ("C2", C.c_int32),
        ("Hout", C.c_int32), ("Wout", C.c_int32),
        ("ksize", C.c_int32), ("stride", C.c_int32), ("pad_t", C.c_int32), ("pad_l", C.c_int32),
        ("upsample", C.c_int32), ("rows_per_batch", C.c_int32), ("ld_rowvec", C.c_int32), ("flags", C.c_int32),
        ("alpha", C.c_float), ("colscale", C.c_void_p), ("in_scsh", C.c_void_p), ("in_act", C.c_int32), ("colstats", C.c_void_p),
        ("cu_share", C.c_int32), ("ln_colsum", C.c_void_p), ("ln_eps", C.c_float),
        ("a_scale", C.c_void_p), ("q8_out", C.c_void_p), ("q8_scale", C.c_void_p), ("ld_q8", C.c_int32),
        ("q8_fixed_col", C.c_int32), ("q8_fixed_mul", C.c_float),
        ("rowstat_out", C.c_void_p), ("rowstat_in", C.c_void_p), ("rowstat_in_parts", C.c_int32),
    ]


class SamplerCoefs(C.Structure):
    _fields_ = [("kx", C.c_float), ("kd", C.c_float), ("ka", C.c_float), ("kp", C.c_float), ("kn", C.c_float),
                ("c_out", C.c_float), ("scale", C.c_float)]


class BucketSegment(C.Structure):
    _fields_ = [("p", C.c_void_p), ("shadow", C.c_void_p), ("offset", C.c_int64), ("n", C.c_int64)]


BUCKET_CHUNK = 4096
BUCKET_ADAMW, BUCKET_EMA = 1, 2

MULTISTEP_MAX = 8


class MultistepCoefs(C.Structure):
    _fields_ = [("c_out", C.c_float), ("scale", C.c_float), ("sigma", C.c_float), ("n", C.c_int32),
                ("k", C.c_float * MULTISTEP_MAX), ("hist", C.c_void_p * MULTISTEP_MAX)]


_vp, _i32, _i64, _f32, _fp = C.c_void_p, C.c_int32, C.c_int64, C.c_float, C.c_void_p
SYMBOLS = {
    "udt_gemm_workspace_bytes": (C.c_size_t, [C.POINTER(GemmDesc)]),
    "udt_gemm": (C.c_int, [C.POINTER(GemmDesc), _vp, C.c_size_t, _vp]),
    "udt_gemm_fwd": (C.c_int, [C.POINTER(GemmDesc), _vp, C.c_size_t, _vp]),
    "udt_conv1x1_fwd": (C.c_int, [C.POINTER(GemmDesc), _vp, C.c_size_t, _vp]),
    "udt_workspace_bytes": (C.c_size_t, [C.POINTER(GemmDesc)]),
    "udt_pack_linear": (C.c_int, [_fp, _fp, _i32, _i32, _i32, _i32, C.POINTER(_vp), _vp]),
    "udt_pack_conv": (C.c_int, [_fp, _fp, _i32, _i32, _i32, _i32, C.POINTER(_i32), _i32, _i32, C.POINTER(_vp), _vp]),
    "udt_packed_weight": (_vp, [_vp]),
    "udt_packed_bias": (_vp, [_vp]),
    "udt_packed_colscale": (_vp, [_vp]),
    "udt_packed_dim": (_i32, [_vp, _i32]),
    "udt_free_packed": (C.c_int, [_vp]),
    "udt_check_async_error": (C.c_int, [_vp, C.c_size_t, _vp]),
    "udt_gemm_colstats_rows": (_i32, [C.POINTER(GemmDesc)]),
    "udt_gemm_colstats_slots": (_i32, [C.POINTER(GemmDesc)]),
    "udt_gemm_rowstat_parts": (_i32, [C.POINTER(GemmDesc)]),
    "udt_gemm_q8_ok": (_i32, [C.POINTER(GemmDesc)]),
    "udt_gemm_in_scsh_ok": (_i32, [C.POINTER(GemmDesc)]),
    "udt_gemm_up4_ok": (_i32, [C.POINTER(GemmDesc)]),
    "udt_gn_silu_conv3x3_fwd": (C.c_int, [C.POINTER(GemmDesc), _vp, C.c_size_t, _vp]),
    "udt_ln_gemm_fwd": (C.c_int, [C.POINTER(GemmDesc), _vp, C.c_size_t, _vp]),
    "udt_gn_finalize": (C.c_int, [_fp, _i32, _i32, _fp, _i32, _i32, _fp, _fp, _fp, _i32, _i64, _i32, _f32, _vp]),
    "udt_gn_apply_scsh": (C.c_int, [_vp, _vp, _vp, _fp, _i32, _i64, _i32, _i32, _i32, _vp]),
    "udt_gn_strip_stats": (C.c_int, [_vp, _vp, _vp, _fp, _i32, _fp, _i32, _fp, _fp, _i32, _i64, _i32, _i32, _i32, _f32, _i32, _vp]),
    "udt_attn_fwd": (C.c_int, [_vp, _vp, _vp, _vp, _i32, _i32, _i32, _i32, _i32, _i32, _i32, _i32,
                               _i64, _i64, _i64, _i64, _f32, _vp]),
    "udt_attn_rowv_fwd": (C.c_int, [_vp, _vp, _vp, _vp, _i32, _i32, _i32, _i32, _i32, _i32, _i32, _i32,
                                    _i64, _i64, _i64, _i64, _f32, _vp]),
    "udt_attn_rowv_q8_fwd": (C.c_int, [_vp, _vp, _vp, _vp, _i32, _i32, _i32, _i32, _i32, _i32, _i32, _i32,
                                       _i64, _i64, _i64, _i64, _f32, _vp, _vp, _i32, _vp]),
    "udt_attn_mx8_fwd": (C.c_int, [_vp, _vp, _vp, _i32, _i32, _i32, _i32, _i32, _f32, _f32, _vp, _vp, _i32, _vp]),
    "udt_attn512_fwd": (C.c_int, [_vp, _vp, _vp, _vp, _i32, _i32, _i32, _i32, _i32, _i32, _i32, _i64, _i64, _i64, _i64, _f32, _vp]),
    "udt_attn512_workspace_bytes": (C.c_size_t, [_i32, _i32, _i32]),
    "udt_attn512_split_fwd": (C.c_int, [_vp, _vp, _vp, _vp, _i32, _i32, _i32, _i32, _i32, _i32, _i32, _i64, _i64, _i64, _i64, _f32,
                                        _vp, C.c_size_t, _vp]),
    "udt_xattn_fwd": (C.c_int, [_vp, _vp, _vp, _vp, _fp, _i32, _i32, _i32, _i32, _i32, _i32, _i32, _i32, _f32, _vp]),
    "udt_mattn_fwd": (C.c_int, [_vp, _vp, _vp, _vp, _fp, _vp, _i32, _i32, _i32, _i32, _i32, _i32, _i32, _i32, _i32, _i32,
                                _i64, _i64, _i64, _i64, _f32, _vp]),
    "udt_softmax_rows": (C.c_int, [_vp, _i64, _i32, _i32, _vp]),
    "udt_tattn_hp": (_i32, [_i32]),
    "udt_tattn_prepare": (C.c_int, [_vp, _i32, _vp, _i32, _vp, _i32, _fp, _fp, _vp, _fp, _vp, _i32, _i32, _i32, _i32, _f32, _vp]),
    "udt_tattn_fused": (C.c_int, [_vp, _vp, _vp, _fp, _vp, _fp, _i32, _i32, _i32, _i32, _i32, _f32, _vp]),
    "udt_tattn_rowstat_parts": (_i32, [_i32, _i32, _i32]),
    "udt_tattn_fused_q8": (C.c_int, [_vp, _vp, _vp, _fp, _vp, _fp, _i32, _i32, _i32, _i32, _i32, _f32, _vp, _vp, _fp, _vp]),
    "udt_tattn_fused_maps": (C.c_int, [_vp, _vp, _vp, _fp, _vp, _fp, _i32, _i32, _i32, _i32, _i32, _f32, _fp, _i32, _i32, _f32, _i32,
                                       _vp, _vp, _fp, _vp]),
    "udt_gn_nchunks": (_i32, [_i64, _i32]),
    "udt_gn_stats": (C.c_int, [_vp, _vp, _fp, _i32, _i64, _i32, _i32, _i32, _vp]),
    "udt_gn_apply": (C.c_int, [_vp, _vp, _vp, _fp, _fp, _fp, _i32, _i64, _i32, _i32, _i32, _f32, _i32, _vp]),
    "udt_gn_strip_ok": (_i32, [_i32, _i64, _i32, _i32, _i32]),
    "udt_gn_strip": (C.c_int, [_vp, _vp, _vp, _fp, _fp, _i32, _i64, _i32, _i32, _i32, _f32, _i32, _vp]),
    "udt_layernorm": (C.c_int, [_vp, _vp, _fp, _fp, _i64, _i32, _f32, _vp]),
    "udt_unet_input": (C.c_int, [_fp, _vp, _i32, _i32, _i32, _f32, _vp]),
    "udt_unet_input_churn": (C.c_int, [_fp, _fp, _vp, _i32, _i32, _i32, _f32, _f32, _vp]),
    "udt_cfg_euler_step": (C.c_int, [_fp, _fp, _fp, _i32, _i32, _i32, _f32, _f32, _f32, _f32, _vp]),
    "udt_cfg_sampler_step": (C.c_int, [_fp, _fp, _fp, _fp, _fp, _fp, _fp, _i32, _i32, _i32, SamplerCoefs, _vp]),
    "udt_cfg_multistep_step": (C.c_int, [_fp, _fp, _fp, _fp, _i32, _i32, _i32, MultistepCoefs, _vp]),
    "udt_precond_unet_input": (C.c_int, [_fp, _fp, _vp, _i32, _i32, _i32, _f32, _f32, _i32, _vp]),
    "udt_precond_euler_step": (C.c_int, [_fp, _fp, _fp, _i32, _i32, _i32, _f32, _f32, _f32, _f32, _f32, _i32, _vp]),
    "udt_precond_sampler_step": (C.c_int, [_fp, _fp, _fp, _fp, _fp, _fp, _fp, _i32, _i32, _i32, SamplerCoefs, _f32, _i32, _vp]),
    "udt_precond_multistep_step": (C.c_int, [_fp, _fp, _fp, _fp, _i32, _i32, _i32, MultistepCoefs, _f32, _i32, _vp]),
    "udt_sampler_step": (C.c_int, [_fp, _fp, _fp, _i32, _i32, _i32, _f32, _f32, _f32, _f32, _vp]),
    "udt_posterior_sample": (C.c_int, [_fp, _fp, _fp, _i32, _i32, _i32, _f32, _vp]),
    "udt_nchw_to_nhwc": (C.c_int, [_fp, _vp, _i32, _i32, _i64, _i32, _f32, _vp]),
    "udt_nhwc_to_nchw": (C.c_int, [_vp, _fp, _i32, _i32, _i64, _i32, _i32, _vp]),
    "udt_nhwc_set_channels": (C.c_int, [_fp, _vp, _i32, _i32, _i64, _i32, _i32, _vp]),
    "udt_embed_tokens": (C.c_int, [_vp, _fp, _fp, _vp, _i32, _i32, _i32, _vp]),
    "udt_timestep_embedding": (C.c_int, [_fp, _vp, _i32, _i32, _vp]),
    "udt_mask_downsample": (C.c_int, [_fp, _fp, _i32, _i32, _i32, _vp]),
    "udt_local_loss": (C.c_int, [_fp, _fp, _fp, _fp, _fp, _i32, _i32, _i32, _i32, _i32, _i32, _i32, _vp]),
    "udt_local_loss_tiled": (C.c_int, [_fp, _fp, _fp, _fp, _fp, _i32, _i32, _i32, _i32, _i32, _i32, _i32, _i32, _vp]),
    "udt_attn_bwd": (C.c_int, [_vp, _vp, _vp, _vp, _vp, _vp, _vp, _vp, _fp, _fp, _i32, _i32, _i32, _i32, _i32, _i32, _f32, _vp]),
    "udt_attn512_bwd": (C.c_int, [_vp, _vp, _vp, _vp, _vp, _vp, _vp, _vp, _fp, _fp, _i32, _i32, _i32, _i32, _i32, _i32, _i32, _i32, _i64,
                                  _i64, _i64, _i64, _i64, _i64, _f32, _vp]),
    "udt_denoised_f32": (C.c_int, [_fp, _fp, _fp, _fp, _fp, _i32, _i32, _i32, _vp]),
    "udt_seed_add_bf16": (C.c_int, [_vp, _fp, _fp, _i32, _i32, _i32, _vp]),
    "udt_xattn_bwd": (C.c_int, [_vp, _vp, _fp, _fp, _vp, _vp, _i32, _i32, _i32, _i32, _i32, _i32, _i32, _i32, _f32, _vp]),
    "udt_local_loss_bwd": (C.c_int, [_fp, _fp, _fp, _fp, _fp, _fp, _fp, _i32, _i32, _i32, _i32, _i32, _i32, _i32, _i32, _f32, _vp]),
    "udt_local_loss_bwd_hw": (C.c_int, [_fp, _fp, _fp, _fp, _fp, _fp, _fp, _i32, _i32, _i32, _i32, _i32, _i32, _i32, _i32, _i32, _f32,
                                        _vp]),
    "udt_local_loss_tiled_hw": (C.c_int, [_fp, _fp, _fp, _fp, _fp, _fp, _i32, _i32, _i32, _i32, _i32, _i32, _i32, _i32, _i32, _vp]),
    "udt_layernorm_bwd": (C.c_int, [_vp, _vp, _fp, _vp, _vp, _i64, _i32, _f32, _vp]),
    "udt_gn_bwd": (C.c_int, [_vp, _vp, _fp, _fp, _vp, _vp, _fp, _i32, _i32, _i32, _i32, _f32, _i32, _vp]),
    "udt_geglu_fwd": (C.c_int, [_vp, _vp, _i64, _i32, _vp]),
    "udt_geglu_bwd": (C.c_int, [_vp, _vp, _vp, _i64, _i32, _vp]),
    "udt_sum2x2_bf16": (C.c_int, [_vp, _vp, _i32, _i32, _i32, _i32, _vp]),
    "udt_axpy_f32": (C.c_int, [_fp, _fp, _f32, _i64, _vp]),
    "udt_aae_row_update_f32": (C.c_int, [_fp, _fp, _fp, _vp, _vp, _vp, _i32, _i64, _f32, _f32, _i32, _i32, _vp]),
    "udt_crop_resize_aa_f32": (C.c_int, [_fp, _vp, _fp, _i32, _i32, _i32, _i32, _i32, _i32, _i32, _f32, _f32, _vp]),
    "udt_crop_resize_aa_bwd_f32": (C.c_int, [_fp, _vp, _fp, _i32, _i32, _i32, _i32, _i32, _i32, _i32, _f32, _vp]),
    "udt_resize_bilinear_f32": (C.c_int, [_fp, _fp, _i64, _i32, _i32, _i32, _i32, _vp]),
    "udt_mattn_bwd": (C.c_int, [_vp, _vp, _vp, _vp, _vp, _vp, _vp, _fp, _vp, _i32, _i32, _i32, _i32, _i32,
                                _i32, _i32, _i32, _i32, _i32, _i32, _i32, _i32, _i64, _i64, _i64, _i64, _i64, _i64, _i64, _f32, _vp]),
    "udt_gelu_fwd": (C.c_int, [_vp, _vp, _i64, _i32, _vp]),
    "udt_gelu_bwd": (C.c_int, [_vp, _vp, _vp, _i64, _i32, _vp]),
# ... 81 lines not shown
```

### udifftext_amd/ops.py

```python
from __future__ import annotations

import contextlib
import ctypes as C
import os
import threading
from typing import NamedTuple, Optional, Sequence

import torch

from . import lib as L
from .packing import conv_out_hw

WORKSPACE_BYTES = 96 << 20


class Workspace:

    def __init__(self, device, nbytes: int = WORKSPACE_BYTES):
        if torch.device(device).type != "cuda":
            raise L.UdtError("udifftext_amd workspaces live on the GPU (no CPU fallback)")
        self.buf = torch.zeros(nbytes, dtype=torch.uint8, device=device)

    def check(self, stream: Optional[int] = None) -> None:
        L.check(L.load().udt_check_async_error(self.buf.data_ptr(), self.buf.numel(), _stream() if stream is None else stream),
                "udt_check_async_error")


class _Ctx(threading.local):
    cu_share = 1
    workspace: Optional[Workspace] = None


_ctx = _Ctx()
_default_ws: dict = {}


@contextlib.contextmanager
def launch_context(cu_share: Optional[int] = None, workspace: Optional[Workspace] = None):
    prev = (_ctx.cu_share, _ctx.workspace)
    if cu_share is not None:
        _ctx.cu_share = max(1, int(cu_share))
    if workspace is not None:
        _ctx.workspace = workspace
    try:
        yield
    finally:
        _ctx.cu_share, _ctx.workspace = prev


def _stream() -> int:
    return torch.cuda.current_stream().cuda_stream


def _ptr(t: Optional[torch.Tensor]) -> Optional[int]:
    if t is None:
        return None
    if not t.is_cuda:
        raise L.UdtError("udifftext_amd ops need device tensors (no CPU fallback)")
    return t.data_ptr()


def _ws(nbytes: int, device) -> torch.Tensor:
    ws = _ctx.workspace
    if ws is None:
        key = (device.type, device.index, _stream())
        ws = _default_ws.get(key)
        if ws is None:
            ws = _default_ws[key] = Workspace(device)
    if ws.buf.numel() < nbytes:
        raise L.UdtError(f"stream-K workspace of {ws.buf.numel()} bytes is too small for this launch ({nbytes})")
    return ws.buf


def check_async_errors() -> None:
    for (_, _, stream), ws in list(_default_ws.items()):
        ws.check(stream)


WORK_COUNTER: Optional[dict] = None


def count_work(kind: str, amount: float) -> None:
    if WORK_COUNTER is not None:
        WORK_COUNTER[kind] = WORK_COUNTER.get(kind, 0.0) + amount


def _bf16(t: torch.Tensor) -> None:
    if t.dtype != torch.bfloat16:
        raise ValueError(f"expected bf16 tensor, got {t.dtype}")


class GnStats(NamedTuple):
    data: torch.Tensor
    slots_per_sample: int


def gn_stats_of(t: Optional[torch.Tensor]) -> Optional[GnStats]:
    return getattr(t, "gn_stats", None) if t is not None else None


class Mx8Act(NamedTuple):
    data: torch.Tensor
    scale: torch.Tensor
    stats: Optional[torch.Tensor] = None


def mx8_of(t: Optional[torch.Tensor]) -> Optional[Mx8Act]:
    return getattr(t, "mx8", None) if t is not None else None


def _drop_sidecars(t: torch.Tensor) -> torch.Tensor:
    attrs = vars(t)
    attrs.pop("gn_stats", None)
    attrs.pop("mx8", None)
    return t


def gemm_desc(**kw) -> L.GemmDesc:
    d = L.GemmDesc()
    d.batch = 1
    d.alpha = 1.0
    d.cu_share = _ctx.cu_share
    for k, v in kw.items():
        setattr(d, k, v)
    return d


def run_gemm(d: L.GemmDesc, device, fused_gn: bool = False, entry: str = "udt_gemm", check: bool = True) -> int:
    if fused_gn:
        entry = "udt_gn_silu_conv3x3_fwd"
    lib = L.load()
    need = lib.udt_gemm_workspace_bytes(C.byref(d))
    ws_ptr, ws_bytes = None, 0
    if need:
        ws = _ws(need, device)
        ws_ptr, ws_bytes = ws.data_ptr(), ws.numel()
    rc = getattr(lib, entry)(C.byref(d), ws_ptr, ws_bytes, _stream())
    if check:
        L.check(rc, entry)
    return rc


def _count_gemm(kind: str, flops: float, nbytes: Optional[float] = None) -> None:
    count_work(kind, flops)
    if nbytes is not None:
        count_work(kind + "_bytes", nbytes)
    count_work(kind + "_launches", 1.0)


GN_STRIP = True


def _attach_colstats(d: L.GemmDesc, out: torch.Tensor, n_cols: int, rows_per_batch: int) -> bool:
    lib = L.load()
    rows = lib.udt_gemm_colstats_rows(C.byref(d))
    if rows <= 0:
        return False
    slots = lib.udt_gemm_colstats_slots(C.byref(d))
    st = torch.empty((slots, n_cols, 2), dtype=torch.float32, device=out.device)
    d.colstats = st.data_ptr()
    out.gn_stats = GnStats(st, rows_per_batch // rows)
    return True


def _mx8_alloc(M: int, cols: int, device) -> Mx8Act:
    return Mx8Act(torch.empty((M, cols), dtype=torch.uint8, device=device),
                  torch.empty(((cols + 127) // 128, M), dtype=torch.int32, device=device))


def _attach_q8(d: L.GemmDesc, M: int, cols: int, device, rowstats: bool, fixed: Optional[tuple] = None) -> Optional[Mx8Act]:
    q = _mx8_alloc(M, cols, device)
    d.q8_out, d.q8_scale, d.ld_q8 = q.data.data_ptr(), q.scale.data_ptr(), cols
    if fixed is not None:
        d.q8_fixed_col, d.q8_fixed_mul = int(fixed[0]), float(fixed[1])
    lib = L.load()
    parts = lib.udt_gemm_rowstat_parts(C.byref(d)) if rowstats else 0
    if not lib.udt_gemm_q8_ok(C.byref(d)) or (rowstats and parts <= 0):
        d.q8_out, d.q8_scale, d.ld_q8, d.q8_fixed_col = None, None, 0, 0
        return None
    if rowstats:
        st = torch.empty((parts, M, 2), dtype=torch.float32, device=device)
        d.rowstat_out = st.data_ptr()
        q = Mx8Act(q.data, q.scale, st)
    return q


def linear(x: torch.Tensor, w: torch.Tensor, bias: Optional[torch.Tensor] = None, *, out: Optional[torch.Tensor] = None,
           residual: Optional[torch.Tensor] = None, rowvec: Optional[torch.Tensor] = None, rows_per_batch: int = 0,
           flags: int = 0, alpha: float = 1.0, n_out: Optional[int] = None, colstats: bool = False,
           emit_q8: bool = False, emit_rowstats: bool = False) -> torch.Tensor:
    _bf16(x); _bf16(w)
    K = x.shape[-1]
    x2 = x.reshape(-1, K) if x.is_contiguous() else x
    assert x2.dim() == 2 and x2.stride(1) == 1
    M = x2.shape[0]
    N = w.shape[0] if n_out is None else n_out
    assert w.shape[1] == K and w.is_contiguous()
    n_cols = N // 2 if (flags & L.GEMM_GEGLU) else N
    if out is None:
        dt = torch.float32 if (flags & L.GEMM_OUT_F32) else torch.bfloat16
        if flags & L.GEMM_TRANSPOSED:
            assert rows_per_batch > 0
            out = torch.empty((M // rows_per_batch, N, rows_per_batch), dtype=dt, device=x.device)
        else:
            out = torch.empty((M, n_cols), dtype=dt, device=x.device)
    else:
        _drop_sidecars(out)
    ldo = out.stride(0) if not (flags & L.GEMM_TRANSPOSED) else 0
    d = gemm_desc(a=_ptr(x2), w=_ptr(w), bias=_ptr(bias), residual=_ptr(residual), rowvec=_ptr(rowvec), out=_ptr(out),
                  M=M, N=N, K=K, lda=x2.stride(0), ldo=ldo, ldr=(residual.stride(0) if residual is not None else 0),
                  rows_per_batch=rows_per_batch, ld_rowvec=(rowvec.stride(0) if rowvec is not None else 0), flags=flags,
                  alpha=alpha)
    if colstats and rows_per_batch > 0 and out.is_contiguous():
        _attach_colstats(d, out, n_cols, rows_per_batch)
    q8 = None
    if emit_q8 and not (flags & (L.GEMM_OUT_F32 | L.GEMM_TRANSPOSED | L.GEMM_GEGLU)) and d.colstats is None and rowvec is None:
        q8 = _attach_q8(d, M, n_cols, x.device, emit_rowstats)
    run_gemm(d, x.device)
    if q8 is not None:
        out.mx8 = q8
    if WORK_COUNTER is not None:
        _count_gemm("gemm", 2.0 * M * N * K, 2.0 * (M * K + N * K) + out.numel() * out.element_size()
                    + (2.0 * M * n_cols if residual is not None else 0.0))
    return out


def linear_mx8(x: Mx8Act, wq: torch.Tensor, colscale: torch.Tensor, bias: Optional[torch.Tensor] = None, *,
               out: Optional[torch.Tensor] = None, residual: Optional[torch.Tensor] = None, rows_per_batch: int = 0,
               flags: int = 0, n_out: Optional[int] = None, colstats: bool = False, emit_q8: bool = False,
               emit_rowstats: bool = False, ln_c: Optional[torch.Tensor] = None, ln_s: Optional[torch.Tensor] = None,
               eps: float = 1e-5, want_bf16: bool = True, q8_fixed: Optional[tuple] = None):
    xq = x.data
    assert xq.dtype == torch.uint8 and wq.dtype == torch.uint8 and xq.is_contiguous() and wq.is_contiguous()
    M, K = xq.shape
    N = wq.shape[0] if n_out is None else n_out
    assert wq.shape[1] == K and K % 128 == 0 and colscale.dtype == torch.float32 and colscale.numel() >= N
    assert x.scale.dtype == torch.int32 and x.scale.shape == (K // 128, M) and x.scale.is_contiguous()
    geglu = bool(flags & L.GEMM_GEGLU)
    n_cols = N // 2 if geglu else N
    only_q8 = emit_q8 and not want_bf16
    if out is not None:
        _drop_sidecars(out)
    elif not only_q8:
        out = torch.empty((M, n_cols), dtype=torch.bfloat16, device=xq.device)
    d = gemm_desc(a=_ptr(xq), w=_ptr(wq), bias=_ptr(ln_c if ln_c is not None else bias), residual=_ptr(residual),
                  out=_ptr(out), M=M, N=N, K=K, lda=K, ldo=(out.stride(0) if out is not None else 0),
                  ldr=(residual.stride(0) if residual is not None else 0), rows_per_batch=rows_per_batch,
                  flags=flags | L.GEMM_MX8, colscale=_ptr(colscale), a_scale=_ptr(x.scale))
    if ln_s is not None:
        if x.stats is None:
            raise L.UdtError("linear_mx8: a LayerNorm-folded MX8 GEMM needs the row statistics of its input (Mx8Act.stats)")
        assert x.stats.dtype == torch.float32 and x.stats.is_contiguous() and x.stats.shape[1:] == (M, 2)
        d.ln_colsum, d.ln_eps = _ptr(ln_s), eps
        d.rowstat_in, d.rowstat_in_parts = _ptr(x.stats), x.stats.shape[0]
    if out is not None and colstats and rows_per_batch > 0 and out.is_contiguous():
        _attach_colstats(d, out, n_cols, rows_per_batch)
    q8 = None
    if emit_q8:
        q8 = _attach_q8(d, M, n_cols, xq.device, emit_rowstats and not geglu, fixed=q8_fixed)
        if q8 is None:
            raise L.UdtError(f"udt_gemm has no MX8-emitting plan for M={M} N={N} K={K} flags={flags:#x}")
    run_gemm(d, xq.device)
    if WORK_COUNTER is not None:
        _count_gemm("gemm_fp8", 2.0 * M * N * K)
    if only_q8:
# ... 15 lines not shown
    N = w_folded.shape[0] if n_out is None else n_out
    n_cols = N // 2 if (flags & L.GEMM_GEGLU) else N
    only_q8 = emit_q8 and not want_bf16
    if out is not None:
        _drop_sidecars(out)
    elif not only_q8:
        out = torch.empty((M, n_cols), dtype=torch.bfloat16, device=x.device)
    d = gemm_desc(a=_ptr(x2), w=_ptr(w_folded), bias=_ptr(c), residual=_ptr(residual), out=_ptr(out), M=M, N=N, K=K,
                  lda=x2.stride(0), ldo=(out.stride(0) if out is not None else 0),
                  ldr=(residual.stride(0) if residual is not None else 0), flags=flags, ln_colsum=_ptr(s), ln_eps=eps)
    q8 = None
    if emit_q8:
        q8 = _attach_q8(d, M, n_cols, x.device, False, fixed=q8_fixed)
        if q8 is None:
            if q8_or_none:
                return None
            raise L.UdtError(f"udt_ln_gemm_fwd has no MX8-emitting plan for M={M} N={N} K={K}")
    rc = run_gemm(d, x.device, entry="udt_ln_gemm_fwd", check=False)
    if rc in (-1, -2) and x.is_cuda:
        raise L.UdtError(f"udt_ln_gemm_fwd declined M={M} N={N} K={K} flags={flags:#x} (status {rc}): the LayerNorm-folded GEMM "
                         "needs the lean kernel family (UDT_LEAN / udt_debug_set('lean') != 0) and 16-byte aligned operands; "
                         "set UDT_LN_GEMM=0 to run layernorm + GEMM instead")
    L.check(rc, "udt_ln_gemm_fwd")
    if WORK_COUNTER is not None:
        _count_gemm("gemm", 2.0 * M * N * K, 2.0 * (M * K + N * K) + (2.0 if out is not None else 0.0) * M * n_cols
                    + (1.0 * M * n_cols if q8 is not None else 0.0) + (2.0 * M * n_cols if residual is not None else 0.0))
    if only_q8:
        return q8
    if q8 is not None:
        out.mx8 = q8
    return out


def bmm_nt(a: torch.Tensor, w: torch.Tensor, *, out: Optional[torch.Tensor] = None, alpha: float = 1.0) -> torch.Tensor:
    _bf16(a); _bf16(w)
    B, M, K = a.shape
    N = w.shape[1]
    assert a.stride(2) == 1 and w.stride(2) == 1 and w.shape[0] == B and w.shape[2] == K
    out = _drop_sidecars(out) if out is not None else torch.empty((B, M, N), dtype=torch.bfloat16, device=a.device)
    d = gemm_desc(a=_ptr(a), w=_ptr(w), out=_ptr(out), M=M, N=N, K=K, lda=a.stride(1), ldw=w.stride(1),
                  ldo=out.stride(1), batch=B, stride_a=a.stride(0), stride_w=w.stride(0), stride_out=out.stride(0),
                  alpha=alpha)
    run_gemm(d, a.device)
    if WORK_COUNTER is not None:
        _count_gemm("gemm", 2.0 * B * M * N * K, 2.0 * B * (M * K + N * K + M * N))
    return out


def conv2d(x: torch.Tensor, w: torch.Tensor, bias: Optional[torch.Tensor] = None, *, ksize: int = 3, stride: int = 1,
           pad: Optional[tuple] = None, upsample: bool = False, x2: Optional[torch.Tensor] = None,
           out_hw: Optional[tuple] = None, residual: Optional[torch.Tensor] = None,
           rowvec: Optional[torch.Tensor] = None, flags: int = 0, n_out: Optional[int] = None,
           out: Optional[torch.Tensor] = None, colstats: bool = False, in_scsh: Optional[torch.Tensor] = None,
           in_act: int = 0, probe_in_scsh: bool = False, w_up4: Optional[torch.Tensor] = None):
    _bf16(x); _bf16(w)
    assert x.is_contiguous() and w.is_contiguous()
    B, H, W_, C1 = x.shape
    C2 = 0
    if x2 is not None:
        _bf16(x2)
        assert x2.is_contiguous() and x2.shape[:3] == x.shape[:3]
        C2 = x2.shape[3]
    if pad is None:
        pad = (ksize // 2, ksize // 2)
    Ho, Wo = conv_out_hw(H, W_, ksize, stride, pad, upsample) if out_hw is None else out_hw
    N = w.shape[0] if n_out is None else n_out
    K = ksize * ksize * (C1 + C2)
    assert w.shape[1] == K, (w.shape, K)
    M = B * Ho * Wo
    if probe_in_scsh:
        pass
    elif out is None:
        dt = torch.float32 if (flags & L.GEMM_OUT_F32) else torch.bfloat16
        out = torch.empty((B, Ho, Wo, N), dtype=dt, device=x.device)
    else:
        _drop_sidecars(out)
    d = gemm_desc(a=_ptr(x), a2=_ptr(x2), w=_ptr(w), bias=_ptr(bias), residual=_ptr(residual), rowvec=_ptr(rowvec),
                  out=_ptr(out), M=M, N=N, K=K, lda=0, ldo=(out.stride(2) if out is not None else N),
                  ldr=(residual.stride(2) if residual is not None else 0),
                  Hin=H, Win=W_, C1=C1, C2=C2, Hout=Ho, Wout=Wo, ksize=ksize, stride=stride, pad_t=pad[0], pad_l=pad[1],
                  upsample=1 if upsample else 0, rows_per_batch=Ho * Wo,
                  ld_rowvec=(rowvec.stride(0) if rowvec is not None else 0), flags=flags | L.GEMM_CONV)
    if probe_in_scsh:
        return bool(L.load().udt_gemm_in_scsh_ok(C.byref(d)))
    if w_up4 is not None and upsample and ksize == 3 and x2 is None and in_scsh is None:
        _bf16(w_up4)
        assert w_up4.is_contiguous() and w_up4.dim() == 3 and w_up4.shape[0] == 4 and w_up4.shape[1] >= N and w_up4.shape[2] == 4 * C1, \
            (w_up4.shape, N, C1)
        d.upsample, d.w, d.ldw, d.stride_w = 2, _ptr(w_up4), w_up4.shape[2], w_up4.stride(0)
        if not L.load().udt_gemm_up4_ok(C.byref(d)):
            d.upsample, d.w, d.ldw, d.stride_w = 1, _ptr(w), 0, 0
    if in_scsh is not None:
        assert in_scsh.dtype == torch.float32 and in_scsh.is_contiguous() and in_scsh.numel() == B * (C1 + C2) * 2
        d.in_scsh = in_scsh.data_ptr()
        d.in_act = int(in_act)
    if colstats:
        _attach_colstats(d, out, N, Ho * Wo)
    run_gemm(d, x.device, fused_gn=in_scsh is not None)
    return out


def _strides(*views: Optional[torch.Tensor], between: tuple = ()) -> tuple:
    return (*[0 if t is None else t.stride(1) for t in views], *between, *[0 if t is None else t.stride(0) for t in views])


def _count_attn(kind: str, flops: float, nbytes: float) -> None:
    count_work(kind, flops)
    count_work(kind + "_bytes", nbytes)
    count_work(kind + "_launches", 1.0)


def attention(q: torch.Tensor, k: torch.Tensor, vt: torch.Tensor, heads: int, scale: float,
              out: Optional[torch.Tensor] = None) -> torch.Tensor:
    _bf16(q); _bf16(k); _bf16(vt)
    B, Nq = q.shape[0], q.shape[1]
    Nk = k.shape[1]
    assert q.stride(2) == 1 and k.stride(2) == 1 and vt.stride(2) == 1
    out = _drop_sidecars(out) if out is not None else torch.empty((B, Nq, heads * 64), dtype=torch.bfloat16, device=q.device)
    L.check(L.load().udt_attn_fwd(_ptr(q), _ptr(k), _ptr(vt), _ptr(out), B, heads, Nq, Nk, *_strides(q, k, vt, out), scale, _stream()),
            "udt_attn_fwd")
    if WORK_COUNTER is not None:
        _count_attn("attn", 4.0 * B * heads * Nq * Nk * 64, 2.0 * B * heads * 64 * (2 * Nq + 2 * Nk))
    return out


def attention_rowv(q: torch.Tensor, k: torch.Tensor, v: torch.Tensor, heads: int, scale: float,
                   out: Optional[torch.Tensor] = None, emit_q8: bool = False) -> torch.Tensor:
    _bf16(q); _bf16(k); _bf16(v)
    B, Nq = q.shape[0], q.shape[1]
    Nk = k.shape[1]
    assert q.stride(2) == 1 and k.stride(2) == 1 and v.stride(2) == 1 and v.shape[1] == Nk
    out = _drop_sidecars(out) if out is not None else torch.empty((B, Nq, heads * 64), dtype=torch.bfloat16, device=q.device)
    args = (_ptr(q), _ptr(k), _ptr(v), _ptr(out), B, heads, Nq, Nk, *_strides(q, k, v, out), scale)
    if emit_q8 and heads % 2 == 0 and out.is_contiguous():
        q8 = _mx8_alloc(B * Nq, heads * 64, q.device)
# ... 65 lines not shown

def _masks(mask: Optional[torch.Tensor], key_padding_mask: Optional[torch.Tensor], B: int, Nq: int, Lk: int) -> tuple:
    if mask is not None:
        mask = mask.float().contiguous()
        assert mask.shape == (Nq, Lk)
    if key_padding_mask is not None:
        key_padding_mask = key_padding_mask.to(torch.uint8).contiguous()
        assert key_padding_mask.shape == (B, Lk)
    return mask, key_padding_mask


def masked_attention(q: torch.Tensor, k: torch.Tensor, v: torch.Tensor, heads: int, scale: float,
                     mask: Optional[torch.Tensor] = None, key_padding_mask: Optional[torch.Tensor] = None,
                     out: Optional[torch.Tensor] = None) -> torch.Tensor:
    _bf16(q); _bf16(k); _bf16(v)
    B, Nq, Cq = q.shape
    Lk = k.shape[1]
    D = Cq // heads
    assert q.stride(2) == 1 and k.stride(2) == 1 and v.stride(2) == 1
    out = _drop_sidecars(out) if out is not None else torch.empty((B, Nq, heads * D), dtype=torch.bfloat16, device=q.device)
    mask, key_padding_mask = _masks(mask, key_padding_mask, B, Nq, Lk)
    L.check(L.load().udt_mattn_fwd(_ptr(q), _ptr(k), _ptr(v), _ptr(out), _ptr(mask), _ptr(key_padding_mask), B, heads, D,
                                   Nq, Lk, *_strides(q, k, v, out, between=(Lk,)), scale, _stream()), "udt_mattn_fwd")
    return out


class TattnTables(NamedTuple):
    A: torch.Tensor
    sc: torch.Tensor
    BmT: torch.Tensor

    def rows(self, begin: int, end: Optional[int] = None) -> "TattnTables":
        return TattnTables(self.A[begin:end], self.sc[begin:end], self.BmT[begin:end])


def tattn_prepare(kv: torch.Tensor, wq: torch.Tensor, wo: torch.Tensor, gamma: torch.Tensor, beta: torch.Tensor, heads: int,
                  scale: float, out: Optional[TattnTables] = None) -> TattnTables:
    _bf16(kv); _bf16(wq); _bf16(wo)
    B, Lc, two_c = kv.shape
    Cc = heads * 64
    assert two_c == 2 * Cc and kv.is_contiguous() and wq.is_contiguous() and wo.is_contiguous()
    hp = L.load().udt_tattn_hp(heads)
    if out is None:
        out = TattnTables(torch.empty((B, hp, Cc), dtype=torch.bfloat16, device=kv.device),
                          torch.empty((B, hp, 2), dtype=torch.float32, device=kv.device),
                          torch.empty((B, Cc, hp), dtype=torch.bfloat16, device=kv.device))
    L.check(L.load().udt_tattn_prepare(_ptr(kv), two_c, _ptr(wq), wq.stride(0), _ptr(wo), wo.stride(0), _ptr(gamma), _ptr(beta),
                                       _ptr(out.A), _ptr(out.sc), _ptr(out.BmT), B, Lc, Cc, heads, scale, _stream()),
            "udt_tattn_prepare")
    return out


def tattn_fused(x: torch.Tensor, tables: Optional[TattnTables], bias: torch.Tensor, heads: int, zero_samples: int, eps: float,
                out: Optional[torch.Tensor] = None, emit_q8: bool = False) -> torch.Tensor:
    _bf16(x)
    assert x.is_contiguous()
    B, N, Cc = x.shape
    out = _drop_sidecars(out) if out is not None else torch.empty_like(x)
    assert out.is_contiguous()
    if tables is not None:
        assert tables.A.is_contiguous() and tables.sc.is_contiguous() and tables.BmT.is_contiguous() and tables.A.shape[0] == B
    parts = L.load().udt_tattn_rowstat_parts(B, N, Cc) if emit_q8 else 0
    if parts > 0:
        q = _mx8_alloc(B * N, Cc, x.device)
        q = Mx8Act(q.data, q.scale, torch.empty((parts, B * N, 2), dtype=torch.float32, device=x.device))
        L.check(L.load().udt_tattn_fused_q8(_ptr(x), _ptr(out), _ptr(tables.A) if tables else None, _ptr(tables.sc) if tables else None,
                                            _ptr(tables.BmT) if tables else None, _ptr(bias), B, N, Cc, heads, zero_samples, eps,
                                            _ptr(q.data), _ptr(q.scale), _ptr(q.stats), _stream()), "udt_tattn_fused_q8")
        out.mx8 = q
        return out
    L.check(L.load().udt_tattn_fused(_ptr(x), _ptr(out), _ptr(tables.A) if tables else None, _ptr(tables.sc) if tables else None,
                                     _ptr(tables.BmT) if tables else None, _ptr(bias), B, N, Cc, heads, zero_samples, eps, _stream()),
            "udt_tattn_fused")
    return out


def tattn_fused_maps(x: torch.Tensor, tables: TattnTables, bias: torch.Tensor, heads: int, zero_samples: int, eps: float,
                     maps: torch.Tensor, map_from: int, weight: float = 1.0, accumulate: bool = False,
                     out: Optional[torch.Tensor] = None, emit_q8: bool = False) -> torch.Tensor:
    _bf16(x)
    assert x.is_contiguous()
    B, N, Cc = x.shape
    out = _drop_sidecars(out) if out is not None else torch.empty_like(x)
    assert out.is_contiguous()
    assert tables is not None and tables.A.is_contiguous() and tables.sc.is_contiguous() and tables.BmT.is_contiguous()
    assert tables.A.shape[0] == B
    assert maps.dtype == torch.float32 and maps.dim() == 3 and maps.is_contiguous() and maps.device == x.device
    assert maps.shape[0] == B - map_from and maps.shape[2] == N, f"maps {tuple(maps.shape)} for B={B} map_from={map_from} N={N}"
    Lc = maps.shape[1]
    q = None
    parts = L.load().udt_tattn_rowstat_parts(B, N, Cc) if emit_q8 else 0
    if parts > 0:
        q = _mx8_alloc(B * N, Cc, x.device)
        q = Mx8Act(q.data, q.scale, torch.empty((parts, B * N, 2), dtype=torch.float32, device=x.device))
    L.check(L.load().udt_tattn_fused_maps(_ptr(x), _ptr(out), _ptr(tables.A), _ptr(tables.sc), _ptr(tables.BmT), _ptr(bias), B, N, Cc, heads,
                                          zero_samples, eps, _ptr(maps), Lc, map_from, float(weight), int(bool(accumulate)),
                                          _ptr(q.data) if q else None, _ptr(q.scale) if q else None, _ptr(q.stats) if q else None,
                                          _stream()), "udt_tattn_fused_maps")
    if q is not None:
        out.mx8 = q
    return out


def softmax_rows_(x: torch.Tensor) -> torch.Tensor:
    _bf16(x)
    assert x.is_contiguous()
    cols = x.shape[-1]
    _drop_sidecars(x)
    L.check(L.load().udt_softmax_rows(_ptr(x), x.numel() // cols, cols, cols, _stream()), "udt_softmax_rows")
    return x
# ... 934 lines not shown
```

### udifftext_amd/sgm/modules/attention.py

```python
from __future__ import annotations

import os
from typing import List, Optional

import torch
import torch.nn as nn

from udifftext_amd import ops, packing

from . import hipnn as H
from .diffusionmodules.util import zero_module


TATTN_FUSED = True

FF_PROJ = os.environ.get("UDT_FF_PROJ", "1") != "0"


class GEGLU(H._Packed):
    def __init__(self, dim_in: int, dim_out: int):
        super().__init__()
        self.proj = H.Linear(dim_in, dim_out * 2)

    def _sources(self):
# ... 148 lines not shown
        B, N, C = x.shape
        x2 = x.reshape(B * N, C)
        mx = ln is not None and x8 is not None
        a8 = ln is not None and H.fp8_attention() and N % 4 == 0
        scale = self.dim_head ** -0.5
        o = None
        if mx:
            wq, cs, c, sv = self.packed_ln_mx8(ln)
            if a8:
                qkv8 = ops.linear_mx8(x8, wq, cs, ln_c=c, ln_s=sv, eps=ln.eps, emit_q8=True, want_bf16=False,
                                      q8_fixed=(2 * inner, self.v_mul8))
                o = ops.attention_mx8(qkv8, B, self.heads, scale, self.v_mul8, emit_q8=True)
            else:
                qkv = ops.linear_mx8(x8, wq, cs, ln_c=c, ln_s=sv, eps=ln.eps).reshape(B, N, 3 * inner)
        elif ln is not None:
            wf, c, sv = self.packed_ln(ln)
            qkv8 = None
            if a8 and C == 320:
                qkv8 = ops.ln_linear(x2, wf, c, sv, eps=ln.eps, emit_q8=True, want_bf16=False, q8_fixed=(2 * inner, self.v_mul),
                                     q8_or_none=True)
            if qkv8 is not None:
                o = ops.attention_mx8(qkv8, B, self.heads, scale, self.v_mul)
            else:
                qkv = ops.ln_linear(x2, wf, c, sv, eps=ln.eps).reshape(B, N, 3 * inner)
        else:
            qkv = ops.linear(x2, self.packed()[0]).reshape(B, N, 3 * inner)
        if o is None:
            o = ops.attention_rowv(qkv[..., :inner], qkv[..., inner:2 * inner], qkv[..., 2 * inner:], self.heads, scale, emit_q8=mx)
        res = residual.reshape(B * N, -1) if residual is not None else None
        return self.to_out[0](o.reshape(B * N, inner), residual=res, x8=ops.mx8_of(o) if mx else None).reshape(B, N, -1)


class BasicTransformerBlock(nn.Module):
    def __init__(self, dim, n_heads, d_head, dropout=0.0, t_context_dim=None, v_context_dim=None, gated_ff=True):
        super().__init__()
        self.attn1 = MemoryEfficientCrossAttention(query_dim=dim, heads=n_heads, dim_head=d_head)
        if t_context_dim is not None and t_context_dim > 0:
            self.t_attn = CrossAttention(query_dim=dim, context_dim=t_context_dim, heads=n_heads, dim_head=d_head)
            self.t_norm = H.LayerNorm(dim)
        if v_context_dim is not None and v_context_dim > 0:
            raise NotImplementedError("v_attn is not configured in UDiffText (v_context_dim unset)")
        self.norm1 = H.LayerNorm(dim)
        self.norm3 = H.LayerNorm(dim)
        self.ff = FeedForward(dim, dropout=dropout, glu=gated_ff)

    char_map = None

    def fused_tattn_ok(self, n_tokens: int) -> bool:
        C = self.t_attn.heads * self.t_attn.dim_head
        return (TATTN_FUSED and self.t_attn.dim_head == 64 and C in (320, 640, 1280) and self.t_attn.heads * 64 == C
                and n_tokens % (32 if C >= 640 else 64) == 0)

    def forward(self, x, t_context=None, v_context=None, t_kv=None, emit_map: bool = False, zero_ctx_rows: int = 0,
                t_fused=None, x8=None, emit_rowstats: bool = False, defer_ff_out: bool = False, hw=None):
        fold = H.LN_GEMM
        mx = fold and x8 is not None and H.mx8_width(x.shape[-1])
        x = self.attn1(x, residual=x, ln=self.norm1, x8=x8 if mx else None) if fold else self.attn1(self.norm1(x), residual=x)
        if hasattr(self, "t_attn"):
            n0 = 0 if emit_map else min(int(zero_ctx_rows), x.shape[0])
            if self.char_map is not None:
                if emit_map or t_fused is None or n0 >= x.shape[0] or not self.fused_tattn_ok(x.shape[1]):
                    raise NotImplementedError(f"character maps of a t_attn layer with {x.shape[1]} tokens: the fused text attention "
                                              "does not run here (no tables, a map-emitting call, or a token count it does not take)")
                maps, map_from, weight, acc = self.char_map
                _, bo = self.t_attn.to_out[0].packed()
                x = ops.tattn_fused_maps(x, t_fused, bo, self.t_attn.heads, n0, self.t_norm.eps, maps, map_from, weight, acc, emit_q8=mx)
            elif t_fused is not None and not emit_map and n0 < x.shape[0] and self.fused_tattn_ok(x.shape[1]):
                _, bo = self.t_attn.to_out[0].packed()
                x = ops.tattn_fused(x, t_fused, bo, self.t_attn.heads, n0, self.t_norm.eps, emit_q8=mx)
            elif n0 > 0 and t_kv is not None:
                y = torch.empty_like(x)
                self.t_attn.zero_context_residual(x[:n0], y[:n0])
                if n0 < x.shape[0]:
                    xc = x[n0:]
                    self.t_attn(self.t_norm(xc), kv=t_kv[n0:], residual=xc, out=y[n0:])
                x = y
            else:
                x = self.t_attn(self.t_norm(x), context=t_context, kv=t_kv, residual=x, emit_map=emit_map, hw=hw)
        B, N, C = x.shape
        x2 = x.reshape(B * N, C)
        if fold:
            x8b = ops.mx8_of(x) if mx else None
            if defer_ff_out and x8b is None:
                return self.ff.net[0](x2, ln=self.norm3), x2
            out = self.ff(x2, residual=x2, ln=self.norm3, x8=x8b, emit_q8=x8b is not None, emit_rowstats=emit_rowstats)
            return H.carry_mx8(out.reshape(B, N, C), out)
        return self.ff(self.norm3(x2), residual=x2).reshape(B, N, C)

    def prepare_ln(self) -> int:
        folded = ((self.attn1, self.norm1), (self.ff.net[0], self.norm3))
        pks = [mod.packed_ln(norm) for mod, norm in folded]
        if H.mx8_width(self.norm1.dim):
            pks += [mod.packed_ln_mx8(norm) for mod, norm in folded]
            pks += [lin.packed_fp8() for lin in (self.attn1.to_out[0], self.ff.net[2])]
        return H.nbytes(*pks)


class SpatialTransformer(nn.Module):
    def __init__(self, in_channels, n_heads, d_head, depth=1, dropout=0.0, t_context_dim=None, v_context_dim=None,
                 use_linear=False):
        super().__init__()
        if not use_linear:
            raise NotImplementedError("use_linear_in_transformer: True is the UDiffText configuration")
        self.in_channels = in_channels
        inner = n_heads * d_head
        self.norm = H.GroupNorm(32, in_channels, eps=1e-6)
        self.proj_in = H.Linear(in_channels, inner)
        self.transformer_blocks = nn.ModuleList(
            [BasicTransformerBlock(inner, n_heads, d_head, dropout=dropout, t_context_dim=t_context_dim,
                                   v_context_dim=v_context_dim) for _ in range(depth)])
        self.proj_out = zero_module(H.Linear(inner, in_channels))
        self.use_linear = use_linear

    def project_context(self, context_bf16) -> List[torch.Tensor]:
        return [blk.t_attn.project_context(context_bf16) for blk in self.transformer_blocks]

    def prepare_fused(self, kv_list, out=None) -> list:
        return [blk.t_attn.prepare_fused(kv, blk.t_norm, out=(out[i] if out is not None else None))
                for i, (blk, kv) in enumerate(zip(self.transformer_blocks, kv_list))]

    def forward(self, x, t_context=None, v_context=None, t_kv: Optional[list] = None, emit_map: bool = False,
                zero_ctx_rows: int = 0, t_fused: Optional[list] = None):
        B, Hh, Ww, C = x.shape
        N = Hh * Ww
        mx = H.mx8_width(self.proj_in.out_features)
        t2 = self.proj_in(self.norm(x).reshape(B * N, C), emit_q8=mx, emit_rowstats=mx)
        t = H.carry_mx8(t2.reshape(B, N, -1), t2)
        nb = len(self.transformer_blocks)
        defer = FF_PROJ and H.LN_GEMM and not mx
        for i, blk in enumerate(self.transformer_blocks):
            t = blk(t, t_context=t_context, t_kv=(t_kv[i] if t_kv is not None else None), emit_map=emit_map,
                    zero_ctx_rows=zero_ctx_rows, t_fused=(t_fused[i] if t_fused is not None else None),
                    x8=ops.mx8_of(t) if mx else None, emit_rowstats=(i + 1 < nb), defer_ff_out=(defer and i + 1 == nb),
                    hw=(Hh, Ww))
        if isinstance(t, tuple):
            hid, t3 = t
            w, b = self.packed_ffproj()
            st = H.want_stats(B, N, w.shape[0])
            out = ops.conv2d(hid.reshape(B, Hh, Ww, -1), w, b, x2=t3.reshape(B, Hh, Ww, -1), ksize=1, pad=(0, 0), residual=x,
                             n_out=w.shape[0], colstats=st)
            if ops.WORK_COUNTER is not None:
                inner = hid.shape[-1]
                H.count_flops("gemm", 2.0 * B * N * C * (inner + C))
                H.count_flops("gemm_bytes", 2.0 * B * N * (inner + 3 * C) + 2.0 * C * (inner + C))
                H.count_flops("gemm_launches", 1.0)
            return out
        out = self.proj_out(t.reshape(B * N, -1), residual=x.reshape(B * N, C), rows_per_batch=N, colstats=True,
                            x8=ops.mx8_of(t) if mx else None)
        return H.carry_stats(out.reshape(B, Hh, Ww, C), out)

    def _sources(self):
        lin2, po = self.transformer_blocks[-1].ff.net[2], self.proj_out
        return lin2.weight, lin2.bias, po.weight, po.bias

    def _pack_ffproj(self):
        lin2, po = self.transformer_blocks[-1].ff.net[2], self.proj_out
        w2, wpo = lin2.weight.float(), po.weight.float()
        wf = torch.cat([wpo @ w2, wpo], dim=1)
        bias = wpo @ lin2.bias.float() + po.bias.float()
        return packing.pack_conv(wf[:, :, None, None], [w2.shape[1], wpo.shape[1]]), packing.pad_bias(bias)

    def packed_ffproj(self):
        return H.layout(self, "ffproj", self._pack_ffproj)

    def prepare_ffproj(self) -> int:
        return H.nbytes(self.packed_ffproj()) if FF_PROJ and H.LN_GEMM else 0

    def prepare_mx8(self) -> int:
        return H.nbytes(self.proj_out.packed_fp8()) if H.mx8_width(self.proj_in.out_features) else 0
```

### udifftext_amd/sgm/modules/diffusionmodules/openaimodel.py

```python
from __future__ import annotations

import os

from typing import List, Optional

import torch
import torch.nn as nn

from udifftext_amd import ops, packing

from ...util import default, exists, require_gpu
from .. import hipnn as H
from ..attention import SpatialTransformer
from .util import zero_module

CPAD = packing.KPAD


class Timestep(nn.Module):
    def __init__(self, dim):
        super().__init__()
        self.dim = dim

    def forward(self, t):
# ... 15 lines not shown
        self.conv.upsamples = True

    def forward(self, x):
        assert x.shape[-1] == self.channels
        return self.conv(x, upsample=True)


class Downsample(nn.Module):
    def __init__(self, channels, use_conv, dims=2, out_channels=None, padding=1, third_down=False):
        super().__init__()
        assert dims == 2 and use_conv
        self.channels = channels
        self.out_channels = out_channels or channels
        self.op = H.Conv2d(channels, self.out_channels, 3, stride=2, padding=padding)
        self.op.emit_colstats = True

    def forward(self, x):
        assert x.shape[-1] == self.channels
        return self.op(x)


class ResBlock(TimestepBlock):
    def __init__(self, channels, emb_channels, dropout, out_channels=None, use_conv=False, use_scale_shift_norm=False,
                 dims=2, up=False, down=False, kernel_size=3, exchange_temb_dims=False, skip_t_emb=False):
        super().__init__()
        if use_scale_shift_norm or up or down or use_conv or skip_t_emb or dims != 2 or kernel_size != 3:
            raise NotImplementedError("ResBlock variant not used by configs/test/textdesign_sd_2.yaml")
        self.channels = channels
        self.emb_channels = emb_channels
        self.out_channels = out_channels or channels
        self.in_layers = nn.Sequential(H.GroupNorm(32, channels), nn.Identity(),
                                       H.Conv2d(channels, self.out_channels, 3, padding=1))
        self.emb_layers = nn.Sequential(nn.Identity(), H.Linear(emb_channels, self.out_channels))
        self.out_layers = nn.Sequential(H.GroupNorm(32, self.out_channels), nn.Identity(), nn.Identity(),
                                        zero_module(H.Conv2d(self.out_channels, self.out_channels, 3, padding=1)))
        if self.out_channels == channels:
            self.skip_connection = nn.Identity()
        else:
            self.skip_connection = H.Conv2d(channels, self.out_channels, 1)

    def forward(self, x, emb_rows, x2=None):
        emb_out = emb_rows[:, self.emb_offset:self.emb_offset + self.out_channels]
        h = self.in_layers[2](x, x2=x2, rowvec=emb_out, norm=self.in_layers[0], norm_silu=True, colstats=True)
        if isinstance(self.skip_connection, nn.Identity):
            assert x2 is None
            skip = x
        else:
            skip = self.skip_connection(x, x2=x2)
        return self.out_layers[3](h, residual=skip, norm=self.out_layers[0], norm_silu=True, colstats=True)


class TimestepEmbedSequential(nn.Sequential, TimestepBlock):
    def forward(self, x, emb_rows=None, t_context=None, v_context=None, x2=None, t_kv=None, emit_map=False,
                zero_ctx_rows=0, t_fused=None):
        for layer in self:
            if isinstance(layer, ResBlock):
                x = layer(x, emb_rows, x2=x2)
                x2 = None
            elif isinstance(layer, SpatialTransformer):
                kv = t_kv[layer.st_index] if t_kv is not None else None
                tf = t_fused[layer.st_index] if t_fused is not None else None
                x = layer(x, t_context, v_context, t_kv=kv, emit_map=emit_map, zero_ctx_rows=zero_ctx_rows, t_fused=tf)
            else:
                x = layer(x)
        return x


class UnifiedUNetModel(nn.Module):
    def __init__(self, in_channels, ctrl_channels, model_channels, out_channels, num_res_blocks, attention_resolutions,
                 dropout=0, channel_mult=(1, 2, 4, 8), save_attn_type=None, save_attn_layers=[], conv_resample=True,
                 dims=2, use_label=None, num_heads=-1, num_head_channels=-1, num_heads_upsample=-1,
                 use_scale_shift_norm=False, resblock_updown=False, transformer_depth=1, t_context_dim=None,
                 v_context_dim=None, num_attention_blocks=None, use_linear_in_transformer=False, adm_in_channels=None,
                 transformer_depth_middle=None):
        super().__init__()
        if ctrl_channels or use_label is not None or resblock_updown or dims != 2 or not conv_resample:
            raise NotImplementedError("option not used by configs/test/textdesign_sd_2.yaml")
        if num_head_channels == -1:
            assert num_heads != -1, "Either num_heads or num_head_channels has to be set"
        self.in_channels, self.ctrl_channels = in_channels, ctrl_channels
        self.model_channels, self.out_channels = model_channels, out_channels
        channel_mult = tuple(channel_mult)
        depth = len(channel_mult) * [transformer_depth]
        depth_mid = default(transformer_depth_middle, depth[-1])
        self.num_res_blocks = len(channel_mult) * [num_res_blocks]
        self.attention_resolutions = tuple(attention_resolutions)
        self.channel_mult = channel_mult
        self.use_label = use_label
        self.num_heads, self.num_head_channels = num_heads, num_head_channels

        ted = model_channels * 4
        self.time_embed = nn.Sequential(H.Linear(model_channels, ted), nn.Identity(), H.Linear(ted, ted))

        def heads_of(ch):
            return (num_heads, ch // num_heads) if num_head_channels == -1 else (ch // num_head_channels, num_head_channels)

        def transformer(ch, d):
            nh, dh = heads_of(ch)
            st = SpatialTransformer(ch, nh, dh, depth=d, t_context_dim=t_context_dim, v_context_dim=v_context_dim,
                                    use_linear=use_linear_in_transformer)
            st.ds = ds
            return st

        self.input_blocks = nn.ModuleList([TimestepEmbedSequential(H.Conv2d(in_channels, model_channels, 3, padding=1))])
        self.input_blocks[0][0].emit_colstats = True
        chans = [model_channels]
        ch, ds = model_channels, 1
        for level, mult in enumerate(channel_mult):
            for nr in range(self.num_res_blocks[level]):
                layers = [ResBlock(ch, ted, dropout, out_channels=mult * model_channels)]
                ch = mult * model_channels
                if ds in self.attention_resolutions and (not exists(num_attention_blocks) or nr < num_attention_blocks[level]):
                    layers.append(transformer(ch, depth[level]))
                self.input_blocks.append(TimestepEmbedSequential(*layers))
                chans.append(ch)
# ... 94 lines not shown

    def char_map_plan(self, h: int, w: int, n_ctx: int, layers=None):
        blocks = self.char_map_blocks(layers)
        hws = {(-(-h // ds), -(-w // ds)) for _, _, ds in blocks}
        if len(hws) != 1:
            raise RuntimeError(f"character maps: the selected layers have different map sizes {sorted(hws)}")
        hm, wm = next(iter(hws))
        for name, blk, _ in blocks:
            if not 2 <= n_ctx <= 12 or not blk.fused_tattn_ok(hm * wm):
                raise NotImplementedError(f"character maps: {name} with {hm * wm} tokens ({hm} x {wm}) and a context of {n_ctx} "
                                          "tokens is not covered by the fused text attention (udt_tattn_fused_maps)")
        return blocks, (hm, wm)

    def char_maps_from_cache(self, rows_from: int = 0, layers=None, attn_type="t_attn") -> torch.Tensor:
        blocks = self.char_map_blocks(layers, attn_type)
        items = [getattr(blk, attn_type).attn_map_cache for _, blk, _ in blocks]
        if any(it is None or it["attn_map"] is None for it in items):
            raise RuntimeError("character maps: a selected layer has no cached map — run a map-emitting UNet call first")
        hws = {it["hw"] for it in items}
        if len(hws) != 1:
            raise RuntimeError(f"character maps: the selected layers have different map sizes {sorted(hws)}")
        hm, wm = next(iter(hws))
        m = torch.stack([it["attn_map"].detach().float() for it in items], dim=0).mean(dim=0)
        _, n, l = m.shape
        m = m.reshape(-1, items[0]["heads"], n, l).mean(dim=1)
        return m[rows_from:].permute(0, 2, 1).reshape(-1, l, hm, wm).contiguous()

    def _sources(self):
        return [p for rb in self._resblocks for p in (rb.emb_layers[1].weight, rb.emb_layers[1].bias)]

    def _pack_emb(self):
        lins = [rb.emb_layers[1] for rb in self._resblocks]
        return (packing.pack_linear(torch.cat([m.weight for m in lins], 0)),
                torch.cat([m.bias for m in lins], 0).float().contiguous())

    def _emb_pack(self):
        return H.layout(self, "emb", self._pack_emb)

    def time_embedding_rows(self, timesteps: torch.Tensor) -> torch.Tensor:
        t_emb = ops.timestep_embedding(timesteps.float().contiguous(), self.model_channels)
        e = self.time_embed[0](t_emb, flags=H.GEMM_SILU_OUT)
        se = self.time_embed[2](e, flags=H.GEMM_SILU_OUT)
        w, b = self._emb_pack()
        return ops.linear(se, w, b, flags=H.GEMM_OUT_F32)

    def project_context(self, t_context: torch.Tensor) -> List[list]:
        ctx = t_context.to(torch.bfloat16).contiguous()
        return [st.project_context(ctx) for st in self._transformers]

    def prepare_fused_tattn(self, t_kv: List[list], out: Optional[List[list]] = None) -> List[list]:
        return [st.prepare_fused(kv, out=(out[i] if out is not None else None))
                for i, (st, kv) in enumerate(zip(self._transformers, t_kv))]

    def forward_nhwc(self, xin: torch.Tensor, emb_rows: torch.Tensor, t_kv: List[list], emit_maps: bool = False,
                     zero_ctx_rows: int = 0, t_fused: Optional[List[list]] = None, char_maps: Optional[torch.Tensor] = None,
                     map_from: int = 0, map_layers=None) -> torch.Tensor:
        asked = []
        if char_maps is not None:
            B, hl, wl, _ = xin.shape
            if emit_maps or t_fused is None:
                raise NotImplementedError("character maps come out of the fused text attention: not from a map-emitting call, and not "
                                          "without its tables")
            blocks, (hm, wm) = self.char_map_plan(hl, wl, char_maps.shape[1], map_layers)
            assert char_maps.dtype == torch.float32 and char_maps.is_contiguous()
            assert char_maps.shape[0] == B - map_from and char_maps[0, 0].numel() == hm * wm and map_from >= min(zero_ctx_rows, B), \
                f"char_maps {tuple(char_maps.shape)}: expected [{B - map_from}, L, {hm} * {wm}] with map_from >= {zero_ctx_rows}"
            flat = char_maps.view(char_maps.shape[0], char_maps.shape[1], hm * wm)
            for i, (_, blk, _) in enumerate(blocks):
                blk.char_map = (flat, int(map_from), 1.0 / len(blocks), i > 0)
                asked.append(blk)
        hs = []
        h = xin
        kw = dict(t_kv=t_kv, emit_map=emit_maps, zero_ctx_rows=zero_ctx_rows, t_fused=t_fused)
        try:
            for block in self.input_blocks:
                h = block(h, emb_rows, **kw)
                hs.append(h)
            h = self.middle_block(h, emb_rows, **kw)
            for block in self.output_blocks:
                h = block(h, emb_rows, x2=hs.pop(), **kw)
        finally:
            for blk in asked:
                blk.char_map = None
        return self.out[2](h, norm=self.out[0], norm_silu=True, flags=H.GEMM_OUT_F32, colstats=False)

    def forward(self, x, timesteps=None, t_context=None, v_context=None, y=None, **kwargs):
        assert (y is not None) == (self.use_label is not None), \
            "must specify y if and only if the model is class-conditional"
        require_gpu(x, "UnifiedUNetModel.forward")
        self.clear_attn_map()
        B, Cc, h, w = x.shape
        assert Cc == self.in_channels
        xin = ops.nchw_to_nhwc(x.float().contiguous(), CPAD)
        emb_rows = self.time_embedding_rows(timesteps)
        t_kv = self.project_context(t_context)
        eps = self.forward_nhwc(xin, emb_rows, t_kv, emit_maps=self.cache_attn_maps)
        return ops.nhwc_to_nchw(eps, self.out_channels).type(x.dtype)
```

### udifftext_amd/sgm/modules/diffusionmodules/sampling.py

```python
from __future__ import annotations

import os
import sys
from typing import Dict, NamedTuple, Optional, Union

import numpy as np
import torch

from udifftext_amd import ops, packing, rng

from ...util import default, instantiate_from_config, require_gpu
from .denoiser import Denoiser, DiscreteDenoiser
from .denoiser_scaling import EDMScaling, EpsScaling, VScaling
from .guiders import IdentityGuider, VanillaCFG
from .sampling_utils import NoDynamicThresholding, to_d

DEFAULT_GUIDER = {"target": "sgm.modules.diffusionmodules.guiders.IdentityGuider"}


class BaseDiffusionSampler:
    def __init__(self, discretization_config, num_steps: Union[int, None] = None, guider_config=None,
                 verbose: bool = False, device: str = "cuda"):
        self.num_steps = num_steps
        self.discretization = instantiate_from_config(discretization_config)
        self.guider = instantiate_from_config(default(guider_config, DEFAULT_GUIDER))
        self.verbose = verbose
        self.device = device

    def prepare_sampling_loop(self, x, cond, uc=None, num_steps=None):
        sigmas = self.discretization(self.num_steps if num_steps is None else num_steps, device=self.device)
        uc = default(uc, cond)
        x *= torch.sqrt(1.0 + sigmas[0] ** 2.0)
        s_in = x.new_ones([x.shape[0]])
        return x, s_in, sigmas, len(sigmas), cond, uc

    def denoise(self, x, model, sigma, cond, uc):
        denoised = model.denoiser(model.model, *self.guider.prepare_inputs(x, sigma, cond, uc))
        return self.guider(denoised, sigma)

    def get_sigma_gen(self, num_sigmas, init_step=0):
        gen = range(init_step, num_sigmas - 1)
        if self.verbose:
            try:
                from tqdm import tqdm
                gen = tqdm(gen, total=num_sigmas - 1 - init_step,
                           desc=f"Sampling with {self.__class__.__name__} for {num_sigmas - 1 - init_step} steps")
            except ImportError:
                pass
        return gen


class SingleStepDiffusionSampler(BaseDiffusionSampler):
    def sampler_step(self, sigma, next_sigma, denoiser, x, cond, uc, *args, **kwargs):
        raise NotImplementedError

    def euler_step(self, x, d, dt):
        return x + dt * d


class EDMSampler(SingleStepDiffusionSampler):
    def __init__(self, s_churn=0.0, s_tmin=0.0, s_tmax=float("inf"), s_noise=1.0, *args, **kwargs):
        super().__init__(*args, **kwargs)
        self.s_churn, self.s_tmin, self.s_tmax, self.s_noise = s_churn, s_tmin, s_tmax, s_noise


NOISE_BATCH = os.environ.get("UDT_NOISE_BATCH", "1") != "0"
DUAL_STREAM = os.environ.get("UDT_DUAL_STREAM", "0") != "0"


def _all_zero(t: torch.Tensor) -> bool:
    flag = getattr(t, "_udt_all_zero", None)
    return bool(flag) if flag is not None else not bool(t.any())


class Precond(NamedTuple):
    c_skip: float
    c_out: float
    c_in: float
    c_noise: float


def _quantise(table: torch.Tensor, value: float):
    idx = int((table - value).abs().argmin())
    return idx, float(table[idx])


def check_denoiser(denoiser) -> None:
    if type(denoiser) not in (Denoiser, DiscreteDenoiser):
        raise NotImplementedError(f"the fused MI355X step implements Denoiser and DiscreteDenoiser, not {type(denoiser).__name__}")
    if type(denoiser.scaling) not in (EpsScaling, VScaling, EDMScaling):
        raise NotImplementedError(f"the fused MI355X step implements EpsScaling, VScaling and EDMScaling, not "
                                  f"{type(denoiser.scaling).__name__}")


def precond_coefs(denoiser, sigma: float, table: Optional[torch.Tensor] = None) -> Precond:
    check_denoiser(denoiser)
    if type(denoiser) is DiscreteDenoiser:
        table = denoiser.sigmas.detach().float().cpu() if table is None else table
        s = _quantise(table, sigma)[1]
    else:
        s = float(sigma)
    scaling = denoiser.scaling
    if type(scaling) is EpsScaling:
        p = Precond(1.0, -s, 1.0 / (s * s + 1.0) ** 0.5, s)
    elif type(scaling) is VScaling:
        d = s * s + 1.0
        p = Precond(1.0 / d, -s / d ** 0.5, 1.0 / d ** 0.5, s)
    else:
        sd = float(scaling.sigma_data)
        d = s * s + sd * sd
        log_s = float(torch.log(torch.tensor(s, dtype=torch.float64)))
        p = Precond(sd * sd / d, s * sd / d ** 0.5, 1.0 / d ** 0.5, 0.25 * log_s)
    if type(denoiser) is DiscreteDenoiser and denoiser.quantize_c_noise:
        p = p._replace(c_noise=float(_quantise(table, p.c_noise)[0]))
    return p


def _table_key(denoiser):
    sigmas = getattr(denoiser, "sigmas", None)
    if sigmas is None:
        return None
    state = (sigmas.data_ptr(), sigmas._version)
    cached = denoiser.__dict__.get("_udt_table_key")
    if cached is None or cached[0] != state:
        cached = (state, hash(sigmas.detach().float().cpu().numpy().tobytes()))
# ... 76 lines not shown
    return e.churn if isinstance(e, (EulerEval, Eval)) else 0.0


def plan_noise_slots(plans) -> Dict[int, int]:
    if any(isinstance(e, Eval) and e.kn != 0.0 for _, plan in plans for e in plan):
        return {i: k for k, (i, _) in enumerate(plans)}
    churned = [i for i, plan in plans if any(_churn(e) != 0.0 for e in plan)]
    return {i: k for k, i in enumerate(churned)}


def char_map_step(n_sigmas: int, init_step: int = 0) -> int:
    mid = (n_sigmas - 1) // 2
    if init_step > mid:
        raise ValueError(f"character maps are taken at step {mid} of {n_sigmas - 1}; init_step {init_step} starts behind it")
    return mid


def plans_with_char_maps(plans, n_sigmas: int, init_step: int = 0) -> list:
    mid = char_map_step(n_sigmas, init_step)
    out = [(i, ((plan[0]._replace(maps=True),) + tuple(plan[1:])) if i == mid else plan) for i, plan in plans]
    assert sum(e.maps for _, plan in out for e in plan) == 1, f"step {mid} is not among the plans"
    return out


def plans_emit_maps(plans) -> bool:
    return any(e.maps for _, plan in plans for e in plan)


def plans_add_noise(plans) -> bool:
    return bool(plan_noise_slots(plans))


class _Stepper:

    def __init__(self, model, cond: dict, uc: dict, batch_size: int, latent_hw, scale: float, two_streams=None, pair: bool = True):
        self.engine = model
        self.unet = model.model.diffusion_model
        self.scale = float(scale)
        self.B = batch_size
        self.pair = bool(pair)
        self.rows = 2 * batch_size if self.pair else batch_size
        h, w = latent_hw
        dev = cond["concat"].device
        self.den = model.denoiser
        sigmas = getattr(self.den, "sigmas", None)
        self.table = sigmas.detach().float().cpu() if sigmas is not None else None
        self.eps_cfg = self.pair and type(self.den) is DiscreteDenoiser and type(self.den.scaling) is EpsScaling
        ctx = torch.cat((uc["t_crossattn"], cond["t_crossattn"]), 0) if self.pair else cond["t_crossattn"]
        self.ctx_len = int(ctx.shape[1])
        self.latent_hw = (int(h), int(w))
        self.t_kv = self.unet.project_context(ctx)
        self.t_fused = self.unet.prepare_fused_tattn(self.t_kv)
        self.zero_ctx_rows = batch_size if self.pair and _all_zero(uc["t_crossattn"]) else 0
        self.dual = self.pair and (DUAL_STREAM if two_streams is None else bool(two_streams))
        if self.dual:
            self.side = torch.cuda.Stream(device=dev)
            self.eps = torch.empty((2 * batch_size, h, w, 4), dtype=torch.float32, device=dev)
            self.t_kv_u = [[kv[:batch_size] for kv in lst] for lst in self.t_kv]
            self.t_kv_c = [[kv[batch_size:] for kv in lst] for lst in self.t_kv]
            self.t_fused_u = [[tb.rows(0, batch_size) if tb is not None else None for tb in lst] for lst in self.t_fused]
            self.t_fused_c = [[tb.rows(batch_size) if tb is not None else None for tb in lst] for lst in self.t_fused]
        self.xin = torch.zeros((self.rows, h, w, packing.KPAD), dtype=torch.bfloat16, device=dev)
        concat = (torch.cat((uc["concat"], cond["concat"]), 0) if self.pair else cond["concat"]).float().contiguous()
        ops.nhwc_set_channels(concat, self.xin, 4)
        self._emb_cache: Dict[float, torch.Tensor] = {}
        self.dev = dev
        self.ws = ops.Workspace(dev)
        self.ws_side = ops.Workspace(dev) if self.dual else None
        self.cu_share = max(1, int(ops._ctx.cu_share))

    def coefs(self, sigma: float) -> Precond:
        return precond_coefs(self.den, sigma, self.table)

    def emb_rows(self, c_noise: float) -> torch.Tensor:
        c_noise = float(c_noise)
        rows = self._emb_cache.get(c_noise)
        if rows is None:
            t = torch.full((self.rows,), c_noise, dtype=torch.float32, device=self.dev)
            rows = self.unet.time_embedding_rows(t)
            self._emb_cache[c_noise] = rows
        return rows

    def new_char_maps(self) -> torch.Tensor:
        _, (hm, wm) = self.unet.char_map_plan(*self.latent_hw, self.ctx_len)
        return torch.zeros((self.B, self.ctx_len, hm, wm), dtype=torch.float32, device=self.dev)

    def unet_eps(self, x: torch.Tensor, sigma: float, emit_maps: bool = False, churn: float = 0.0,
                 noise: Optional[torch.Tensor] = None, char_maps: Optional[torch.Tensor] = None):
        k = self.coefs(sigma)
        if churn != 0.0 and noise is None:
            raise ValueError("a churned evaluation needs the step's draw (draw_step_noise)")
        if not self.eps_cfg:
            ops.precond_unet_input(x, self.xin, k.c_in, self.pair, noise if churn != 0.0 else None, churn)
        elif churn != 0.0:
            ops.unet_input_churn(x, noise, self.xin, k.c_in, churn)
        else:
            ops.unet_input(x, self.xin, k.c_in)
        if emit_maps:
            self.unet.clear_attn_map()
        emb = self.emb_rows(k.c_noise)
        if self.dual and not emit_maps:
            eps = self._forward_two_streams(emb, char_maps)
        else:
            with ops.launch_context(cu_share=self.cu_share, workspace=self.ws):
                eps = self.unet.forward_nhwc(self.xin, emb, self.t_kv, emit_maps=emit_maps, zero_ctx_rows=self.zero_ctx_rows,
                                             t_fused=self.t_fused, char_maps=char_maps, map_from=self.B if self.pair else 0)
        return eps, k

    def step(self, x: torch.Tensor, sigma: float, sigma_next: float, emit_maps: bool = False,
             denoised: Optional[torch.Tensor] = None, churn: float = 0.0, noise: Optional[torch.Tensor] = None,
             char_maps: Optional[torch.Tensor] = None) -> None:
        eps, k = self.unet_eps(x, sigma, emit_maps, churn, noise, char_maps)
        if self.eps_cfg:
            ops.cfg_euler_step(x, eps, sigma, sigma_next, self.scale, denoised=denoised, c_out=k.c_out)
        else:
            ops.precond_euler_step(x, eps, k.c_skip, k.c_out, sigma, sigma_next, self.scale, self.pair, denoised=denoised)

    def run_plan(self, bufs: Dict[str, torch.Tensor], plan, noise: Optional[torch.Tensor] = None,
                 char_maps: Optional[torch.Tensor] = None) -> None:
        for e in plan:
            src = bufs[e.src]
            cm = char_maps if e.maps else None
            if e.maps and cm is None:
                raise ValueError("an evaluation of the plan emits character maps and no buffer was given (new_char_maps)")
            if isinstance(e, EulerEval):
                self.step(src, e.sigma, e.sigma_next, churn=e.churn, noise=noise, char_maps=cm)
                continue
            if isinstance(e, MultistepEval):
                eps, k = self.unet_eps(src, e.sigma, char_maps=cm)
                ms = dict(hist=[bufs[b] for b, _ in e.hist], d_out=bufs[e.d_out], out=bufs[e.out])
                ks = (e.k0,) + tuple(kj for _, kj in e.hist)
                if self.eps_cfg:
                    ops.cfg_multistep_step(src, eps, k.c_out, self.scale, e.sigma, ks, **ms)
                else:
                    ops.precond_multistep_step(src, eps, k.c_skip, k.c_out, self.scale, self.pair, e.sigma, ks, **ms)
                continue
            eps, k = self.unet_eps(src, e.sigma, churn=e.churn, noise=noise, char_maps=cm)
            terms = dict(aux=bufs[e.aux] if e.aux else None, ka=e.ka, prev=bufs[e.prev] if e.prev else None, kp=e.kp,
                         noise=noise if e.kn != 0.0 else None, kn=e.kn, out=bufs[e.out],
                         denoised=bufs[e.den_out] if e.den_out else None)
            if self.eps_cfg:
                ops.cfg_sampler_step(src, eps, k.c_out, self.scale, e.kx, e.kd, **terms)
            else:
                ops.precond_sampler_step(src, eps, k.c_skip, k.c_out, self.scale, self.pair, e.kx, e.kd, **terms)

    def check(self) -> None:
        self.ws.check()
        if self.ws_side is not None:
            self.ws_side.check(self.side.cuda_stream)

    def _forward_two_streams(self, emb: torch.Tensor, char_maps: Optional[torch.Tensor] = None) -> torch.Tensor:
        B = self.B
        main = torch.cuda.current_stream()
        share = 2 * self.cu_share
        self.side.wait_stream(main)
        with torch.cuda.stream(self.side), ops.launch_context(cu_share=share, workspace=self.ws_side):
            eps_c = self.unet.forward_nhwc(self.xin[B:], emb[B:], self.t_kv_c, zero_ctx_rows=0, t_fused=self.t_fused_c,
                                           char_maps=char_maps, map_from=0)
            self.eps[B:].copy_(eps_c)
        with ops.launch_context(cu_share=share, workspace=self.ws):
            eps_u = self.unet.forward_nhwc(self.xin[:B], emb[:B], self.t_kv_u, zero_ctx_rows=self.zero_ctx_rows,
                                           t_fused=self.t_fused_u)
            self.eps[:B].copy_(eps_u)
        main.wait_stream(self.side)
        return self.eps


class _GraphedSteps:

    def __init__(self, model, cond, uc, batch_size, latent_hw, scale, sig, cu_share: int = 1, plans=None, pair: bool = True):
        self.cu_share = int(cu_share)
        self.st = _Stepper(model, cond, uc, batch_size, latent_hw, scale, two_streams=None if cu_share == 1 else False, pair=pair)
        self.st.cu_share = self.cu_share
        self.fingerprint = weights_fingerprint(model)
        if plans is None:
            plans = [(i, (EulerEval(sig[i], sig[i + 1]),)) for i in range(len(sig) - 1)]
        self.plans = dict(plans)
        h, w = latent_hw
        self.x = torch.zeros((batch_size, 4, h, w), dtype=torch.float32, device=self.st.dev)
        self.bufs = {"x": self.x}
        for name in plan_buffers(plans):
            self.bufs[name] = torch.zeros_like(self.x)
        self.slots = plan_noise_slots(plans)
        self.noise = (torch.zeros((len(self.slots),) + tuple(self.x.shape), dtype=torch.float32, device=self.st.dev)
                      if self.slots else None)
        self.maps = self.st.new_char_maps() if plans_emit_maps(plans) else None
        self.graphs: Dict[int, torch.cuda.CUDAGraph] = {}
        self.pool = torch.cuda.graph_pool_handle()
        self.capture_stream = torch.cuda.Stream(device=self.st.dev)
        self.warm = False
        self.last_replay: Optional[torch.cuda.Event] = None

    def rebind(self, cond, uc) -> bool:
        st = self.st
        zero_rows = st.B if st.pair and _all_zero(uc["t_crossattn"]) else 0
        if zero_rows != st.zero_ctx_rows or cond["concat"].shape[0] != st.B:
            return False
        ctx = torch.cat((uc["t_crossattn"], cond["t_crossattn"]), 0) if st.pair else cond["t_crossattn"]
        for dst_list, src_list in zip(st.t_kv, st.unet.project_context(ctx)):
            for dst, src in zip(dst_list, src_list):
                dst.copy_(src)
        st.unet.prepare_fused_tattn(st.t_kv, out=st.t_fused)
        concat = (torch.cat((uc["concat"], cond["concat"]), 0) if st.pair else cond["concat"]).float().contiguous()
        ops.nhwc_set_channels(concat, st.xin, 4)
        return True

    def load(self, x: torch.Tensor, noise: Optional[torch.Tensor] = None) -> None:
        self.x.copy_(x)
        if self.noise is not None and noise is not None:
            self.noise.copy_(noise)

    def _capture(self, i: int) -> torch.cuda.CUDAGraph:
        st, plan = self.st, self.plans[i]
        noise = self.noise[self.slots[i]] if i in self.slots else None
        for e in plan:
            st.emb_rows(st.coefs(e.sigma).c_noise)
        if not self.warm:
            torch.cuda.synchronize()
            with torch.cuda.stream(self.capture_stream):
                keep = {k: v.clone() for k, v in self.bufs.items()}
                st.run_plan(self.bufs, plan, noise, self.maps)
                for k, v in keep.items():
                    self.bufs[k].copy_(v)
            torch.cuda.synchronize()
            self.warm = True
        g = torch.cuda.CUDAGraph()
        with torch.cuda.graph(g, pool=self.pool, stream=self.capture_stream, capture_error_mode="thread_local"):
            st.run_plan(self.bufs, plan, noise, self.maps)
        self.graphs[i] = g
        return g

    def capture(self) -> None:
        missing = [i for i in self.plans if i not in self.graphs]
        if missing:
            lane = torch.cuda.current_stream()
            self.capture_stream.wait_stream(lane)
            for i in missing:
                self._capture(i)
            lane.wait_stream(self.capture_stream)


class _RunnerKey(NamedTuple):
    model: int
    shape: tuple
    scale: float
    device: Optional[int]
    plans: tuple
    slot: int = 0
    n_lanes: int = 1
# ... 629 lines not shown
```

### udifftext_amd/sgm/modules/hipnn.py

```python
from __future__ import annotations

import math
import os
from typing import Optional

import torch
import torch.nn as nn

from udifftext_amd import lib as L
from udifftext_amd import ops, packing

from ..util import init_skipped


def count_flops(kind: str, flops: float) -> None:
    ops.count_work(kind, flops)


FUSE_GN = os.environ.get("UDT_FUSE_GN", "0") != "0"

GN_EPI = os.environ.get("UDT_GN_EPI", "1") != "0" and os.environ.get("UDT_LEAN", "") != "0"
EMIT_STATS = FUSE_GN or GN_EPI


def want_stats(B: int, HW: int, C: int) -> bool:
    return FUSE_GN or (GN_EPI and C % 8 == 0)


FP8_LINEARS = os.environ.get("UDT_FP8", "0") != "0"


FP8_ATTENTION = os.environ.get("UDT_FP8_ATTN", "1") != "0"


def fp8_attention() -> bool:
    return FP8_LINEARS and LN_GEMM and FP8_ATTENTION


def v_fixed_mul(w_v: torch.Tensor, c_v: torch.Tensor) -> float:
    bound = 12.0 * float(w_v.float().norm(dim=1).max()) + float(c_v.float().abs().max())
    return float(2.0 ** math.floor(math.log2(448.0 / max(bound, 1e-20))))


def mx8_width(c: int) -> bool:
    return FP8_LINEARS and LN_GEMM and c % 128 == 0

LN_GEMM = os.environ.get("UDT_LN_GEMM", "1") != "0" and os.environ.get("UDT_LEAN", "") != "0"


def carry_stats(dst: torch.Tensor, src: torch.Tensor) -> torch.Tensor:
    st = ops.gn_stats_of(src)
    if st is not None:
        dst.gn_stats = st
    return dst


def carry_mx8(dst: torch.Tensor, src: torch.Tensor) -> torch.Tensor:
    q = ops.mx8_of(src)
    if q is not None:
        dst.mx8 = q
    return dst


def _init_uniform_(p: torch.Tensor, fan_in: int) -> None:
    if init_skipped():
        return
    bound = 1.0 / math.sqrt(max(fan_in, 1))
    with torch.no_grad():
        p.uniform_(-bound, bound)


class _Layouts(dict):
    frozen = False


def _layouts(mod: nn.Module) -> _Layouts:
    store = mod.__dict__.get("_layouts")
    if store is None:
        store = mod.__dict__["_layouts"] = _Layouts()
    return store


def layout(mod: nn.Module, tag: str, build, *inputs):
    store = _layouts(mod)
    hit = store.get(tag)
    if store.frozen:
        if hit is None:
            raise L.UdtError(f"{type(mod).__name__}: layout {tag!r} was not built before prepare(free_masters=True) released the "
                             "fp32 masters; reload the checkpoint into a fresh engine to change the launch path")
        return hit[1]
    key = [(t.data_ptr(), t._version, t.device) if isinstance(t, torch.Tensor) else t for t in (*mod._sources(), *inputs)]
    if hit is None or hit[0] != key:
        with torch.no_grad():
            hit = store[tag] = (key, build())
    return hit[1]


def has_layout(mod: nn.Module, tag: str) -> bool:
    return tag in mod.__dict__.get("_layouts", ())

# ... 5 lines not shown
def drop_layouts(root: nn.Module) -> None:
    for m in root.modules():
        store = m.__dict__.get("_layouts")
        if store is not None and not store.frozen:
            store.clear()


def nbytes(*layouts) -> int:
    ts = [t for pk in layouts for t in (pk if isinstance(pk, (tuple, list)) else (pk,))]
    return sum(t.numel() * t.element_size() for t in ts if isinstance(t, torch.Tensor))


class _Packed(nn.Module):

    def _sources(self):
        return self._parameters.values()

    def fused_children(self):
        return []

    def packed(self):
        return layout(self, "plain", self._pack)

    def packed_fp8(self):
        return layout(self, "fp8", self._pack_fp8)

    def packed_ln(self, norm):
        return layout(self, "ln", lambda: self._pack_ln(norm.weight, norm.bias), norm.weight, norm.bias)

    def packed_ln_mx8(self, norm):
        return layout(self, "ln_mx8", lambda: self._pack_ln_mx8(norm.weight, norm.bias), norm.weight, norm.bias)


class Linear(_Packed):
    def __init__(self, in_features: int, out_features: int, bias: bool = True):
        super().__init__()
        self.in_features, self.out_features = in_features, out_features
        self.weight = nn.Parameter(torch.empty(out_features, in_features))
        _init_uniform_(self.weight, in_features)
        if bias:
            self.bias = nn.Parameter(torch.empty(out_features))
            _init_uniform_(self.bias, in_features)
        else:
            self.register_parameter("bias", None)

    def _pack(self):
        return packing.pack_linear(self.weight), packing.pad_bias(self.bias)

    def _pack_fp8(self):
        wq, cs = packing.pack_linear_fp8(self.weight)
        return wq, cs, packing.pad_bias(self.bias)

    def forward(self, x, residual=None, flags: int = 0, out=None, rowvec=None, rows_per_batch: int = 0,
                colstats: bool = False, x8=None, emit_q8: bool = False, emit_rowstats: bool = False):
        if x8 is not None:
            wq, cs, b = self.packed_fp8()
            M = x8.data.shape[0]
            if colstats:
                rpb = rows_per_batch if rows_per_batch > 0 else M
                colstats = want_stats(M // rpb, rpb, wq.shape[0])
            return ops.linear_mx8(x8, wq, cs, b, residual=residual, flags=flags, out=out, rows_per_batch=rows_per_batch,
                                  colstats=bool(colstats), emit_q8=emit_q8, emit_rowstats=emit_rowstats)
        w, b = self.packed()
        if colstats:
            rpb = rows_per_batch if rows_per_batch > 0 else x.shape[0]
            colstats = want_stats(x.shape[0] // rpb, rpb, w.shape[0])
        return ops.linear(x, w, b, residual=residual, flags=flags, out=out, rowvec=rowvec, rows_per_batch=rows_per_batch,
                          colstats=bool(colstats), emit_q8=emit_q8, emit_rowstats=emit_rowstats)


class Conv2d(_Packed):

    def __init__(self, in_channels: int, out_channels: int, kernel_size: int, stride: int = 1, padding: int = 0):
        super().__init__()
        self.in_channels, self.out_channels = in_channels, out_channels
        self.kernel_size, self.stride, self.padding = kernel_size, stride, padding
        self.weight = nn.Parameter(torch.empty(out_channels, in_channels, kernel_size, kernel_size))
        self.bias = nn.Parameter(torch.empty(out_channels))
        fan_in = in_channels * kernel_size * kernel_size
        _init_uniform_(self.weight, fan_in)
        _init_uniform_(self.bias, fan_in)
        self.segments = None
        self.n_pad = 4
        self.emit_colstats = False

    def _pack(self):
        return packing.pack_conv(self.weight, self.segments, self.n_pad), packing.pad_bias(self.bias, self.n_pad)

    def packed(self):
        return layout(self, "plain", self._pack, self.segments, self.n_pad)

    def packed_up4(self):
        return layout(self, "up4", lambda: packing.pack_conv_up4(self.weight, self.n_pad), self.n_pad)

    def forward(self, x, x2=None, residual=None, rowvec=None, upsample: bool = False, flags: int = 0,
                pad: Optional[tuple] = None, out_hw: Optional[tuple] = None, norm: Optional["GroupNorm"] = None,
                norm_silu: bool = False, colstats: Optional[bool] = None):
        if x2 is not None and self.segments is None and (x.shape[-1] % 64 != 0 or x2.shape[-1] % 64 != 0):
            self.segments = (x.shape[-1], x2.shape[-1])
        w, b = self.packed()
        if pad is None:
            pad = (self.padding, self.padding)
        if colstats is None:
            colstats = self.emit_colstats
        if colstats:
            oh, ow = out_hw if out_hw is not None else ops.conv_out_hw(x.shape[1], x.shape[2], self.kernel_size, self.stride, pad, upsample)
            colstats = want_stats(x.shape[0], oh * ow, w.shape[0])
        colstats = bool(colstats)
        kw = dict(ksize=self.kernel_size, stride=self.stride, pad=pad, upsample=upsample, out_hw=out_hw, residual=residual,
                  rowvec=rowvec, flags=flags, n_out=w.shape[0], colstats=colstats)
        if upsample and norm is None and x2 is None and self.kernel_size == 3 and self.stride == 1:
            kw["w_up4"] = self.packed_up4()
        in_scsh = None
        if norm is not None:
            st1, st2 = ops.gn_stats_of(x), ops.gn_stats_of(x2)
            if (FUSE_GN and st1 is not None and (x2 is None or st2 is not None)
                    and ops.conv2d(x, w, b, x2=x2, probe_in_scsh=True, **kw)):
                B = x.shape[0]
                in_scsh = ops.gn_finalize(st1, x.shape[-1], st2, x2.shape[-1] if x2 is not None else 0, norm.weight,
                                          norm.bias, B, x.shape[1] * x.shape[2], norm.num_groups, norm.eps)
                count_flops("fused_gn_convs", 1)
# ... 63 lines not shown
```

Measured before the change: 10.55 images/s.

## Share first input ResBlock across CFG pair when cond and uncond inputs match

When the unconditional branch has an all-zero text context and otherwise identical inputs, the first input ResBlock and the self-attention prefix of its SpatialTransformer are computed once on half the batch. Tokens are expanded back to the full CFG batch only where text cross-attention makes them diverge. GEMM and tattn kernels gain residual_rows/x_samples wrap-around indexing, so the shared half can be read as both halves. A plan_rows pin keeps tile plans consistent with the full-size shapes. This removes redundant compute on the 64x64 stage at the cost of extra plan logic and shape checks.

```diff
diff --git a/include/udt_kernels.h b/include/udt_kernels.h
--- a/include/udt_kernels.h
+++ b/include/udt_kernels.h
@@ -70,6 +70,8 @@
   float* rowstat_out;
   const float* rowstat_in;
   int32_t rowstat_in_parts;
+  int32_t residual_rows;
+  int32_t plan_rows;
 } udt_gemm_desc;
 
 size_t udt_gemm_workspace_bytes(const udt_gemm_desc* d);
@@ -133,6 +135,9 @@
                       int32_t C, int32_t heads, float scale, void* stream);
 int udt_tattn_fused(const void* x, void* out, const void* A, const float* sc, const void* BmT, const float* bias,
                     int32_t B, int32_t n_tok, int32_t C, int32_t heads, int32_t zero_samples, float eps, void* stream);
+int udt_tattn_fused_src(const void* x, void* out, const void* A, const float* sc, const void* BmT, const float* bias,
+                        int32_t B, int32_t n_tok, int32_t C, int32_t heads, int32_t zero_samples, float eps, int32_t x_samples,
+                        void* stream);
 int32_t udt_tattn_rowstat_parts(int32_t B, int32_t n_tok, int32_t C);
 int udt_tattn_fused_q8(const void* x, void* out, const void* A, const float* sc, const void* BmT, const float* bias,
                        int32_t B, int32_t n_tok, int32_t C, int32_t heads, int32_t zero_samples, float eps, void* q8_out,
diff --git a/udifftext_amd/csrc/gemm.hip b/udifftext_amd/csrc/gemm.hip
--- a/udifftext_amd/csrc/gemm.hip
+++ b/udifftext_amd/csrc/gemm.hip
@@ -421,7 +421,22 @@
   long long total;
   int G, ipw;
   bool fixup;
+  bool bad = false;
 };
+
+inline int plan_m(const udt_gemm_desc* d) { return d->plan_rows > d->M ? d->plan_rows : d->M; }
+inline bool plan_pinned(const udt_gemm_desc* d) { return d->plan_rows > d->M; }
+
+template <class F>
+TilePlan pinned_plan(const udt_gemm_desc* d, F plan) {
+  if (!plan_pinned(d)) return plan(d, false);
+  udt_gemm_desc pd = *d;
+  pd.M = d->plan_rows; pd.plan_rows = 0;
+  const TilePlan tp = plan(&pd, false);
+  TilePlan t = plan(d, true);
+  t.bad = tp.fixup || tp.bm != t.bm || tp.bn != t.bn;
+  return t;
+}
 
 constexpr int MAX_DEVICES = 16;
 std::atomic<int> g_dev_cus[MAX_DEVICES];
@@ -447,7 +462,7 @@
   return s < 2 ? 2 : s;
 }
 
-TilePlan plan_tiles(const udt_gemm_desc* d) {
+TilePlan plan_tiles_rule(const udt_gemm_desc* d, bool whole_only) {
   TilePlan t;
   const int batch = d->batch > 0 ? d->batch : 1;
   const bool tall = d->M >= 1024;
@@ -464,7 +479,9 @@
   t.total = (long long)t.tiles * t.nkt;
   const int slots = resident_slots(d);
   const long long share = (t.total + slots - 1) / slots;
-  if (t.tiles < slots / 2 && t.nkt >= 16) {
+  if (whole_only) {
+    t.ipw = t.nkt;
+  } else if (t.tiles < slots / 2 && t.nkt >= 16) {
     long long G = t.total / 8;
     if (G < 1) G = 1;
     if (G > slots) G = slots;
@@ -480,6 +497,7 @@
   t.fixup = (t.ipw % t.nkt) != 0;
   return t;
 }
+TilePlan plan_tiles(const udt_gemm_desc* d) { return pinned_plan(d, plan_tiles_rule); }
 
 template <int BM, int BN, int WGM, int WGN, bool CONV, bool TRANS>
 hipError_t launch_cfg(const GemmParams& p, const TilePlan& t, hipStream_t s) {
@@ -526,7 +544,7 @@
   return (long long)tiles * 4 >= (long long)(resident_slots(d) / 2) * 3;
 }
 
-TilePlan plan_tiles8(const udt_gemm_desc* d) {
+TilePlan plan_tiles8_rule(const udt_gemm_desc* d, bool whole_only) {
   TilePlan t;
   const int batch = d->batch > 0 ? d->batch : 1;
   const bool geglu_or_trans = (d->flags & (UDT_GEMM_TRANSPOSED | UDT_GEMM_GEGLU)) != 0;
@@ -537,7 +555,7 @@
   t.tiles = t.tiles_m * t.tiles_n * batch;
   t.nkt = d->K / k_tile(d);
   t.total = (long long)t.tiles * t.nkt;
-  const bool whole = t.nkt < 24 || prefer_whole_tiles(d, t.tiles);
+  const bool whole = whole_only || t.nkt < 24 || prefer_whole_tiles(d, t.tiles);
   int slots = (whole ? resident_slots_all() : resident_slots(d)) / 2;
   long long G = t.total / 4;
   if (G < 1) G = 1;
@@ -548,6 +566,7 @@
   t.fixup = (t.ipw % t.nkt) != 0;
   return t;
 }
+TilePlan plan_tiles8(const udt_gemm_desc* d) { return pinned_plan(d, plan_tiles8_rule); }
 
 template <int WGM, int WGN, int TM, int TN, bool CONV, bool TRANS, bool STATS = false>
 hipError_t launch8(const g8::Params& pp, const TilePlan& t, hipStream_t s) {
@@ -591,7 +610,7 @@
   return ge.n_pieces * 8 <= c3p::patch_rows(bn == 160 ? 5 : 2, gn) && ge.n_pieces >= 8;
 }
 
-TilePlan plan_tiles3p(const udt_gemm_desc* d, const c3p::Geo& ge) {
+TilePlan plan_tiles3p_rule(const udt_gemm_desc* d, const c3p::Geo& ge, bool whole_only) {
   TilePlan t;
   t.bm = 256;
   t.bn = (d->N % 160 == 0 && d->N % 128 != 0) ? 160 : 128;
@@ -600,7 +619,7 @@
   t.tiles = t.tiles_m * t.tiles_n;
   t.nkt = ge.chunks;
   t.total = (long long)t.tiles * t.nkt;
-  const bool whole = t.nkt * 9 < 24 || prefer_whole_tiles(d, t.tiles);
+  const bool whole = whole_only || t.nkt * 9 < 24 || prefer_whole_tiles(d, t.tiles);
   const int slots = (whole ? resident_slots_all() : resident_slots(d)) / 2;
   long long G = t.total;
   if (G > slots) G = slots;
@@ -609,6 +628,13 @@
   t.G = round_workgroups((int)((t.total + t.ipw - 1) / t.ipw));
   t.fixup = (t.ipw % t.nkt) != 0;
   return t;
+}
+TilePlan plan_tiles3p(const udt_gemm_desc* d, const c3p::Geo& ge) {
+  return pinned_plan(d, [&](const udt_gemm_desc* q, bool whole_only) {
+    c3p::Geo gq = ge;
+    if (q != d) { gq.B = q->M / (q->Hout * q->Wout); gq.img_groups = (gq.B + gq.NI - 1) / gq.NI; }
+    return plan_tiles3p_rule(q, gq, whole_only);
+  });
 }
 
 template <int WGM, int WGN, int TM, int TN, bool GN, bool STATS, bool UPS = false>
@@ -782,7 +808,7 @@
                                      (long long)d->M * (d->out ? d->ldo : 0) * 2 < (1LL << 31) && (long long)((d->N + 127) / 128) * d->M * 4 < (1LL << 31));
     if (ln && !want_stats && d->K == 320 && d->N % 64 == 0 && !d->residual && !d->rowvec && !conv1 && emit_fits &&
         (reinterpret_cast<uintptr_t>(d->a) & 15) == 0) {
-      const int tiles_m = (d->M + 255) / 256, chunks = d->N / 64;
+      const int tiles_m = (plan_m(d) + 255) / 256, chunks = d->N / 64;
       int ns = (device_cus() + tiles_m - 1) / tiles_m;
       if (ns > chunks / 4) ns = chunks / 4;
       const int cmax = geglu ? 20 : 16;
@@ -791,7 +817,7 @@
       const long long wgs = (long long)tiles_m * ns;
       if (ns >= 1 && (mode == 7 || emit || (geglu ? wgs * 4 >= 3LL * device_cus() : wgs >= device_cus()))) {
         t.cfg = 7; t.stats_rows = 0; t.nw = 4; t.bm = 256; t.bn = 64; t.smem = 0;
-        t.tiles_m = tiles_m; t.kt_per = (chunks + ns - 1) / ns; t.tiles_n = (chunks + t.kt_per - 1) / t.kt_per;
+        t.tiles_m = (d->M + 255) / 256; t.kt_per = (chunks + ns - 1) / ns; t.tiles_n = (chunks + t.kt_per - 1) / t.kt_per;
         t.tiles = t.tiles_m * t.tiles_n; t.nkt = d->K / BK; t.splitk = 1; t.n_block = 1;
         t.G = round_workgroups(t.tiles);
         return true;
@@ -802,7 +828,7 @@
   t.cfg = (mode > 0) ? mode : 1;
   if (!mx8 && !emit) {
   if (!geglu && d->N % 160 == 0 && d->N % 128 != 0 && t.cfg == 1) t.cfg = 5;
-  if (mode <= 0 && d->N >= 768 && (long long)((d->M + 255) / 256) * ((d->N + 255) / 256) >= 2LL * device_cus() &&
+  if (mode <= 0 && d->N >= 768 && (long long)((plan_m(d) + 255) / 256) * ((d->N + 255) / 256) >= 2LL * device_cus() &&
       (d->cu_share <= 1 || lean256_under_lanes())) t.cfg = 6;
   }
   t.stats_rows = 0;
@@ -830,15 +856,16 @@
   t.tiles_n = (d->N + t.bn - 1) / t.bn;
   t.tiles = t.tiles_m * t.tiles_n;
   t.nkt = d->K / KT;
+  const int ptiles_m = (plan_m(d) + t.bm - 1) / t.bm, ptiles = ptiles_m * t.tiles_n;
   int slots = device_cus() * ((t.cfg == 1 || t.cfg == 5) ? 2 : 1) / share_of(d);
   if (slots < 1) slots = 1;
   int sk = 1;
   const int knob = lean_splitk_knob();
-  if (!ln && t.tiles <= 1023) {
+  if (!ln && ptiles <= 1023) {
     if (knob > 1) sk = knob;
-    else if (knob < 0 && t.tiles * 2 <= slots && t.nkt >= (mx8 ? 20 : 40)) { sk = slots / t.tiles; if (sk > t.nkt / (mx8 ? 8 : 16)) sk = t.nkt / (mx8 ? 8 : 16); }
+    else if (knob < 0 && ptiles * 2 <= slots && t.nkt >= (mx8 ? 20 : 40)) { sk = slots / ptiles; if (sk > t.nkt / (mx8 ? 8 : 16)) sk = t.nkt / (mx8 ? 8 : 16); }
     if (sk > t.nkt / 4) sk = t.nkt / 4;
-    while (sk > 1 && (long long)t.tiles * sk * t.bm * t.bn * 4 > (64LL << 20)) --sk;
+    while (sk > 1 && (long long)ptiles * sk * t.bm * t.bn * 4 > (64LL << 20)) --sk;
     if (sk < 1) sk = 1;
   }
   t.kt_per = (t.nkt + sk - 1) / sk;
@@ -846,7 +873,7 @@
   const int units = t.tiles * t.splitk;
   t.G = round_workgroups(units);
   int nb = g_n_block.load(std::memory_order_relaxed);
-  if (nb <= 0) nb = (t.tiles_m <= 8) ? t.tiles_n : 8;
+  if (nb <= 0) nb = (ptiles_m <= 8) ? t.tiles_n : 8;
   if (nb > t.tiles_n) nb = t.tiles_n;
   t.n_block = nb;
   return true;
@@ -918,7 +945,7 @@
     if (wm != 0 && !ups && d->N % 160 == 0 && Wt % 16 == 0 && Ht % 16 == 0) {
       const int cus = device_cus(), share = d->cu_share > 1 ? d->cu_share : 1;
       wide_slots = cus / share > 0 ? cus / share : 1;
-      const long long wt = (long long)(d->M / 256) * (d->N / 160);
+      const long long wt = (long long)(plan_m(d) / 256) * (d->N / 160);
       const long long sk = conv_chunk_slices(wt, wide_slots, d->C1 / 64, lean_splitk_knob());
       const long long units = wt * sk;
       const long long rounds = (units + cus - 1) / cus;
@@ -952,8 +979,9 @@
   c.tiles = c.tiles_m * c.tiles_n;
   c.chunks = c.C / 64;
   const int slots = wide ? wide_slots : (2 * device_cus() / share_of(d) > 0 ? 2 * device_cus() / share_of(d) : 1);
-  int sk = conv_chunk_slices((long long)c.tiles * nph, slots, c.chunks, lean_splitk_knob());
-  while (sk > 1 && (long long)c.tiles * nph * sk * c.tw * c.th * c.bn * 4 > (64LL << 20)) --sk;
+  const long long ptiles = (long long)(plan_m(d) / (d->Hout * d->Wout)) * c.tiles_x * c.tiles_y * c.tiles_n;
+  int sk = conv_chunk_slices(ptiles * nph, slots, c.chunks, lean_splitk_knob());
+  while (sk > 1 && ptiles * nph * sk * c.tw * c.th * c.bn * 4 > (64LL << 20)) --sk;
   c.ch_per = (c.chunks + sk - 1) / sk;
   c.splitk = (c.chunks + c.ch_per - 1) / c.ch_per;
   c.G = round_workgroups(c.tiles * nph * c.splitk);
@@ -1148,6 +1176,17 @@
     if (d->N % 64 != 0 || (d->flags & UDT_GEMM_OUT_F32) || d->residual || d->rowvec) return UDT_ERR_BAD_ARG;
   }
   if (d->rowvec && d->rows_per_batch <= 0) return UDT_ERR_BAD_ARG;
+  if (d->plan_rows < 0 || (d->plan_rows > 0 && (d->plan_rows < d->M || d->plan_rows % d->M != 0))) return UDT_ERR_BAD_SHAPE;
+  if (plan_pinned(d) && batch != 1) return UDT_ERR_BAD_ARG;
+  if (d->residual_rows < 0 || d->residual_rows > d->M) return UDT_ERR_BAD_SHAPE;
+  const bool res_wraps = d->residual_rows > 0 && d->residual_rows < d->M;
+  if (res_wraps) {
+    LeanPlan ltr;
+    if (!d->residual || !d->out || !lean_plan(d, ltr, d->colstats != nullptr) || ltr.cfg == 7) return UDT_ERR_BAD_ARG;
+    const uintptr_t r0 = reinterpret_cast<uintptr_t>(d->residual), o0 = reinterpret_cast<uintptr_t>(d->out);
+    const uintptr_t r1 = r0 + (uintptr_t)d->residual_rows * d->ldr * 2, o1 = o0 + (uintptr_t)d->M * d->ldo * 2;
+    if (r0 < o1 && o0 < r1) return UDT_ERR_BAD_ARG;
+  }
 
   hipStream_t s = reinterpret_cast<hipStream_t>(stream);
   if (conv_n4_applies(d)) {
@@ -1235,6 +1274,7 @@
       lp.rowstat_in = d->rowstat_in; lp.rowstat_in_parts = d->rowstat_in_parts;
       lp.q8_out = reinterpret_cast<uint8_t*>(d->q8_out); lp.q8_scale = reinterpret_cast<uint32_t*>(d->q8_scale); lp.ld_q8 = d->ld_q8;
       lp.rowstat_out = d->rowstat_out;
+      lp.res_rows = res_wraps ? d->residual_rows : d->M;
       lp.q8_fixed_col = d->q8_fixed_col > 0 ? d->q8_fixed_col : 0x7fffffff;
       lp.q8_fixed_mul = d->q8_fixed_mul;
       lp.G = lt.G;
@@ -1287,6 +1327,7 @@
     c3p::CParams cp;
     if (conv3p_geometry(d, cp.geo, d->in_scsh != nullptr)) {
       const TilePlan t3 = plan_tiles3p(d, cp.geo);
+      if (t3.bad) return UDT_ERR_BAD_ARG;
       p.tiles_m = t3.tiles_m; p.tiles_n = t3.tiles_n; p.tiles_per_batch = t3.tiles_m * t3.tiles_n;
       {
         const double patch = (double)cp.geo.prows_img * cp.geo.NI * cp.geo.C * 2.0;
@@ -1332,6 +1373,7 @@
   }
   if (use_gemm8(d)) {
     const TilePlan t8 = plan_tiles8(d);
+    if (t8.bad) return UDT_ERR_BAD_ARG;
     p.tiles_m = t8.tiles_m; p.tiles_n = t8.tiles_n; p.tiles_per_batch = t8.tiles_m * t8.tiles_n;
     const int n_block_knob = g_n_block.load(std::memory_order_relaxed);
     if (n_block_knob != 0 && !conv) {
@@ -1383,6 +1425,7 @@
     return UDT_OK;
   }
 
+  if (t.bad) return UDT_ERR_BAD_ARG;
   p.tiles_m = t.tiles_m; p.tiles_n = t.tiles_n; p.tiles_per_batch = t.tiles_m * t.tiles_n;
   p.n_ktiles = t.nkt;
   p.total_iters = t.total;
diff --git a/udifftext_amd/csrc/lean.h b/udifftext_amd/csrc/lean.h
--- a/udifftext_amd/csrc/lean.h
+++ b/udifftext_amd/csrc/lean.h
@@ -480,7 +480,8 @@
           const int m = m0 + row0 + prow0 + row;
           u32x4 z = {0u, 0u, 0u, 0u};
           rv[i] = z;
-          if (col_ok && row < PROWS && m < p.M) rv[i] = *reinterpret_cast<const u32x4*>(p.res + (long long)m * p.ldr + n);
+          const int mr = m < p.res_rows ? m : m % p.res_rows;
+          if (col_ok && row < PROWS && m < p.M) rv[i] = *reinterpret_cast<const u32x4*>(p.res + (long long)mr * p.ldr + n);
         }
       }
 #pragma unroll
diff --git a/udifftext_amd/csrc/lean_params.h b/udifftext_amd/csrc/lean_params.h
--- a/udifftext_amd/csrc/lean_params.h
+++ b/udifftext_amd/csrc/lean_params.h
@@ -34,6 +34,7 @@
   int q8_fixed_col;
   float q8_fixed_mul;
   float* rowstat_out;
+  int res_rows;
 };
 
 struct C3Params {
diff --git a/udifftext_amd/csrc/tattn.hip b/udifftext_amd/csrc/tattn.hip
--- a/udifftext_amd/csrc/tattn.hip
+++ b/udifftext_amd/csrc/tattn.hip
@@ -16,6 +16,7 @@
   const float* bias;
   const uint16_t* zero;
   int M, C, hp, n_tok, zero_samples;
+  int x_rows;
   int nsplit;
   float eps;
   uint8_t* q8_out;
@@ -49,7 +50,7 @@
   const int l31 = lane & 31, hi = lane >> 5;
   const long long tok0 = (long long)blockIdx.x * TT;
   const int b = (int)(tok0 / p.n_tok);
-  const uint16_t* xg = p.x + tok0 * C;
+  const uint16_t* xg = p.x + (tok0 % p.x_rows) * C;
   uint16_t* og = p.out + tok0 * C;
   float* const rst = reinterpret_cast<float*>(pl + (size_t)TT * prs);
   const int ct_lo = (int)blockIdx.y * (C >> 5) / p.nsplit, ct_hi = ((int)blockIdx.y + 1) * (C >> 5) / p.nsplit;
@@ -400,8 +401,14 @@
 int tattn_launch(const void* x, void* out, const void* A, const float* sc, const void* BmT, const float* bias, int32_t B, int32_t n_tok,
                  int32_t C, int32_t heads, int32_t zero_samples, float eps, void* q8_out, void* q8_scale, float* rowstat_out, void* stream,
                  bool with_maps = false, float* maps = nullptr, int32_t L = 0, int32_t map_from = 0, float weight = 0.f,
-                 int32_t accumulate = 0) {
+                 int32_t accumulate = 0, int32_t x_samples = 0) {
   if (with_maps && !maps) return UDT_ERR_BAD_ARG;
+  if (x_samples < 0 || x_samples > B) return UDT_ERR_BAD_SHAPE;
+  if (x_samples > 0 && x_samples < B && x && out) {
+    const uintptr_t x0 = reinterpret_cast<uintptr_t>(x), o0 = reinterpret_cast<uintptr_t>(out);
+    const uintptr_t x1 = x0 + (uintptr_t)x_samples * n_tok * C * 2, o1 = o0 + (uintptr_t)B * n_tok * C * 2;
+    if (x0 < o1 && o0 < x1) return UDT_ERR_BAD_ARG;
+  }
   if (!x || !out || !bias || (zero_samples < B && (!A || !sc || !BmT))) return UDT_ERR_BAD_ARG;
   if (B <= 0 || n_tok <= 0 || heads <= 0 || C != heads * 64 || C > 1280 || zero_samples < 0 || zero_samples > B) return UDT_ERR_BAD_SHAPE;
   const int TT = tattn_tt(C);
@@ -415,6 +422,7 @@
   p.zero = udt_zero_page();
   if (!p.zero) return UDT_ERR_HIP;
   p.M = B * n_tok; p.C = C; p.hp = udt_tattn_hp(heads); p.n_tok = n_tok; p.zero_samples = zero_samples; p.eps = eps;
+  p.x_rows = (x_samples > 0 ? x_samples : B) * n_tok;
   p.q8_out = reinterpret_cast<uint8_t*>(q8_out); p.q8_scale = reinterpret_cast<uint32_t*>(q8_scale); p.rowstat_out = rowstat_out;
   p.maps = maps; p.heads = heads; p.map_L = L; p.map_from = map_from; p.map_acc = accumulate != 0; p.map_scale = weight / (float)heads;
   const size_t smem = (size_t)TT * C * 2 + (size_t)TT * 2 * sizeof(float) + (size_t)TT * (p.hp * 2 + 16) + (q8 ? (size_t)TT * (C / 32) * 8 : 0);
@@ -455,6 +463,13 @@
   return tattn_launch(x, out, A, sc, BmT, bias, B, n_tok, C, heads, zero_samples, eps, nullptr, nullptr, nullptr, stream);
 }
 
+extern "C" int udt_tattn_fused_src(const void* x, void* out, const void* A, const float* sc, const void* BmT, const float* bias,
+                                   int32_t B, int32_t n_tok, int32_t C, int32_t heads, int32_t zero_samples, float eps, int32_t x_samples,
+                                   void* stream) {
+  return tattn_launch(x, out, A, sc, BmT, bias, B, n_tok, C, heads, zero_samples, eps, nullptr, nullptr, nullptr, stream, false, nullptr, 0, 0,
+                      0.f, 0, x_samples);
+}
+
 extern "C" int32_t udt_tattn_rowstat_parts(int32_t B, int32_t n_tok, int32_t C) {
   if (B <= 0 || n_tok <= 0 || (C != 640 && C != 1280)) return 0;
   const int TT = tattn_tt(C);
diff --git a/udifftext_amd/lib.py b/udifftext_amd/lib.py
--- a/udifftext_amd/lib.py
+++ b/udifftext_amd/lib.py
@@ -35,6 +35,7 @@
         ("a_scale", C.c_void_p), ("q8_out", C.c_void_p), ("q8_scale", C.c_void_p), ("ld_q8", C.c_int32),
         ("q8_fixed_col", C.c_int32), ("q8_fixed_mul", C.c_float),
         ("rowstat_out", C.c_void_p), ("rowstat_in", C.c_void_p), ("rowstat_in_parts", C.c_int32),
+        ("residual_rows", C.c_int32), ("plan_rows", C.c_int32),
     ]
 
 
@@ -102,6 +103,7 @@
     "udt_tattn_hp": (_i32, [_i32]),
     "udt_tattn_prepare": (C.c_int, [_vp, _i32, _vp, _i32, _vp, _i32, _fp, _fp, _vp, _fp, _vp, _i32, _i32, _i32, _i32, _f32, _vp]),
     "udt_tattn_fused": (C.c_int, [_vp, _vp, _vp, _fp, _vp, _fp, _i32, _i32, _i32, _i32, _i32, _f32, _vp]),
+    "udt_tattn_fused_src": (C.c_int, [_vp, _vp, _vp, _fp, _vp, _fp, _i32, _i32, _i32, _i32, _i32, _f32, _i32, _vp]),
     "udt_tattn_rowstat_parts": (_i32, [_i32, _i32, _i32]),
     "udt_tattn_fused_q8": (C.c_int, [_vp, _vp, _vp, _fp, _vp, _fp, _i32, _i32, _i32, _i32, _i32, _f32, _vp, _vp, _fp, _vp]),
     "udt_tattn_fused_maps": (C.c_int, [_vp, _vp, _vp, _fp, _vp, _fp, _i32, _i32, _i32, _i32, _i32, _f32, _fp, _i32, _i32, _f32, _i32,
diff --git a/udifftext_amd/ops.py b/udifftext_amd/ops.py
--- a/udifftext_amd/ops.py
+++ b/udifftext_amd/ops.py
@@ -29,6 +29,7 @@
 class _Ctx(threading.local):
     cu_share = 1
     workspace: Optional[Workspace] = None
+    plan_scale = 1
 
 
 _ctx = _Ctx()
@@ -36,16 +37,18 @@
 
 
 @contextlib.contextmanager
-def launch_context(cu_share: Optional[int] = None, workspace: Optional[Workspace] = None):
-    prev = (_ctx.cu_share, _ctx.workspace)
+def launch_context(cu_share: Optional[int] = None, workspace: Optional[Workspace] = None, plan_scale: Optional[int] = None):
+    prev = (_ctx.cu_share, _ctx.workspace, _ctx.plan_scale)
     if cu_share is not None:
         _ctx.cu_share = max(1, int(cu_share))
     if workspace is not None:
         _ctx.workspace = workspace
+    if plan_scale is not None:
+        _ctx.plan_scale = max(1, int(plan_scale))
     try:
         yield
     finally:
-        _ctx.cu_share, _ctx.workspace = prev
+        _ctx.cu_share, _ctx.workspace, _ctx.plan_scale = prev
 
 
 def _stream() -> int:
@@ -123,6 +126,8 @@
     d.cu_share = _ctx.cu_share
     for k, v in kw.items():
         setattr(d, k, v)
+    if _ctx.plan_scale > 1 and d.batch == 1 and d.plan_rows == 0:
+        d.plan_rows = d.M * _ctx.plan_scale
     return d
 
 
@@ -188,7 +193,7 @@
 def linear(x: torch.Tensor, w: torch.Tensor, bias: Optional[torch.Tensor] = None, *, out: Optional[torch.Tensor] = None,
            residual: Optional[torch.Tensor] = None, rowvec: Optional[torch.Tensor] = None, rows_per_batch: int = 0,
            flags: int = 0, alpha: float = 1.0, n_out: Optional[int] = None, colstats: bool = False,
-           emit_q8: bool = False, emit_rowstats: bool = False) -> torch.Tensor:
+           emit_q8: bool = False, emit_rowstats: bool = False, residual_rows: int = 0) -> torch.Tensor:
     _bf16(x); _bf16(w)
     K = x.shape[-1]
     x2 = x.reshape(-1, K) if x.is_contiguous() else x
@@ -211,6 +216,9 @@
                   M=M, N=N, K=K, lda=x2.stride(0), ldo=ldo, ldr=(residual.stride(0) if residual is not None else 0),
                   rows_per_batch=rows_per_batch, ld_rowvec=(rowvec.stride(0) if rowvec is not None else 0), flags=flags,
                   alpha=alpha)
+    if residual_rows:
+        assert residual is not None and residual.shape[0] == residual_rows, (residual.shape, M, residual_rows)
+        d.residual_rows = int(residual_rows)
     if colstats and rows_per_batch > 0 and out.is_contiguous():
         _attach_colstats(d, out, n_cols, rows_per_batch)
     q8 = None
@@ -332,7 +340,7 @@
            out_hw: Optional[tuple] = None, residual: Optional[torch.Tensor] = None,
            rowvec: Optional[torch.Tensor] = None, flags: int = 0, n_out: Optional[int] = None,
            out: Optional[torch.Tensor] = None, colstats: bool = False, in_scsh: Optional[torch.Tensor] = None,
-           in_act: int = 0, probe_in_scsh: bool = False, w_up4: Optional[torch.Tensor] = None):
+           in_act: int = 0, probe_in_scsh: bool = False, w_up4: Optional[torch.Tensor] = None, residual_rows: int = 0):
     _bf16(x); _bf16(w)
     assert x.is_contiguous() and w.is_contiguous()
     B, H, W_, C1 = x.shape
@@ -361,6 +369,9 @@
                   Hin=H, Win=W_, C1=C1, C2=C2, Hout=Ho, Wout=Wo, ksize=ksize, stride=stride, pad_t=pad[0], pad_l=pad[1],
                   upsample=1 if upsample else 0, rows_per_batch=Ho * Wo,
                   ld_rowvec=(rowvec.stride(0) if rowvec is not None else 0), flags=flags | L.GEMM_CONV)
+    if residual_rows:
+        assert residual is not None and residual.numel() == residual_rows * residual.shape[-1], (residual.shape, M, residual_rows)
+        d.residual_rows = int(residual_rows)
     if probe_in_scsh:
         return bool(L.load().udt_gemm_in_scsh_ok(C.byref(d)))
     if w_up4 is not None and upsample and ksize == 3 and x2 is None and in_scsh is None:
@@ -532,10 +543,20 @@
 
 
 def tattn_fused(x: torch.Tensor, tables: Optional[TattnTables], bias: torch.Tensor, heads: int, zero_samples: int, eps: float,
-                out: Optional[torch.Tensor] = None, emit_q8: bool = False) -> torch.Tensor:
+                out: Optional[torch.Tensor] = None, emit_q8: bool = False, out_samples: int = 0) -> torch.Tensor:
     _bf16(x)
     assert x.is_contiguous()
     B, N, Cc = x.shape
+    if out_samples > B:
+        assert not emit_q8 and out_samples % B == 0 and out is not x
+        out = _drop_sidecars(out) if out is not None else torch.empty((out_samples, N, Cc), dtype=x.dtype, device=x.device)
+        assert out.is_contiguous() and out.shape == (out_samples, N, Cc)
+        if tables is not None:
+            assert tables.A.is_contiguous() and tables.sc.is_contiguous() and tables.BmT.is_contiguous() and tables.A.shape[0] == out_samples
+        L.check(L.load().udt_tattn_fused_src(_ptr(x), _ptr(out), _ptr(tables.A) if tables else None, _ptr(tables.sc) if tables else None,
+                                             _ptr(tables.BmT) if tables else None, _ptr(bias), out_samples, N, Cc, heads, zero_samples, eps,
+                                             B, _stream()), "udt_tattn_fused_src")
+        return out
     out = _drop_sidecars(out) if out is not None else torch.empty_like(x)
     assert out.is_contiguous()
     if tables is not None:
diff --git a/udifftext_amd/sgm/modules/attention.py b/udifftext_amd/sgm/modules/attention.py
--- a/udifftext_amd/sgm/modules/attention.py
+++ b/udifftext_amd/sgm/modules/attention.py
@@ -224,11 +224,18 @@
                 and n_tokens % (32 if C >= 640 else 64) == 0)
 
     def forward(self, x, t_context=None, v_context=None, t_kv=None, emit_map: bool = False, zero_ctx_rows: int = 0,
-                t_fused=None, x8=None, emit_rowstats: bool = False, defer_ff_out: bool = False, hw=None):
+                t_fused=None, x8=None, emit_rowstats: bool = False, defer_ff_out: bool = False, hw=None, pair: int = 1):
         fold = H.LN_GEMM
         mx = fold and x8 is not None and H.mx8_width(x.shape[-1])
-        x = self.attn1(x, residual=x, ln=self.norm1, x8=x8 if mx else None) if fold else self.attn1(self.norm1(x), residual=x)
-        if hasattr(self, "t_attn"):
+        if pair > 1:
+            assert fold and not mx and not emit_map and self.char_map is None and t_fused is not None
+            with ops.launch_context(plan_scale=pair):
+                x = self.attn1(x, residual=x, ln=self.norm1)
+            _, bo = self.t_attn.to_out[0].packed()
+            x = ops.tattn_fused(x, t_fused, bo, self.t_attn.heads, int(zero_ctx_rows), self.t_norm.eps, out_samples=pair * x.shape[0])
+        else:
+            x = self.attn1(x, residual=x, ln=self.norm1, x8=x8 if mx else None) if fold else self.attn1(self.norm1(x), residual=x)
+        if pair == 1 and hasattr(self, "t_attn"):
             n0 = 0 if emit_map else min(int(zero_ctx_rows), x.shape[0])
             if self.char_map is not None:
                 if emit_map or t_fused is None or n0 >= x.shape[0] or not self.fused_tattn_ok(x.shape[1]):
@@ -291,35 +298,45 @@
         return [blk.t_attn.prepare_fused(kv, blk.t_norm, out=(out[i] if out is not None else None))
                 for i, (blk, kv) in enumerate(zip(self.transformer_blocks, kv_list))]
 
+    def pair_prefix_ok(self, n_tokens: int, t_fused: Optional[list], emit_map: bool = False) -> bool:
+        blk = self.transformer_blocks[0]
+        return (H.LN_GEMM and not H.FP8_LINEARS and not emit_map and hasattr(blk, "t_attn") and blk.char_map is None
+                and t_fused is not None and t_fused[0] is not None and blk.fused_tattn_ok(n_tokens))
+
     def forward(self, x, t_context=None, v_context=None, t_kv: Optional[list] = None, emit_map: bool = False,
-                zero_ctx_rows: int = 0, t_fused: Optional[list] = None):
+                zero_ctx_rows: int = 0, t_fused: Optional[list] = None, pair: int = 1):
         B, Hh, Ww, C = x.shape
         N = Hh * Ww
         mx = H.mx8_width(self.proj_in.out_features)
-        t2 = self.proj_in(self.norm(x).reshape(B * N, C), emit_q8=mx, emit_rowstats=mx)
+        if pair > 1:
+            with ops.launch_context(plan_scale=pair):
+                t2 = self.proj_in(self.norm(x).reshape(B * N, C))
+        else:
+            t2 = self.proj_in(self.norm(x).reshape(B * N, C), emit_q8=mx, emit_rowstats=mx)
         t = H.carry_mx8(t2.reshape(B, N, -1), t2)
+        Bo, res_rows = pair * B, (B * N if pair > 1 else 0)
         nb = len(self.transformer_blocks)
         defer = FF_PROJ and H.LN_GEMM and not mx
         for i, blk in enumerate(self.transformer_blocks):
             t = blk(t, t_context=t_context, t_kv=(t_kv[i] if t_kv is not None else None), emit_map=emit_map,
                     zero_ctx_rows=zero_ctx_rows, t_fused=(t_fused[i] if t_fused is not None else None),
                     x8=ops.mx8_of(t) if mx else None, emit_rowstats=(i + 1 < nb), defer_ff_out=(defer and i + 1 == nb),
-                    hw=(Hh, Ww))
+                    hw=(Hh, Ww), pair=(pair if i == 0 else 1))
         if isinstance(t, tuple):
             hid, t3 = t
             w, b = self.packed_ffproj()
-            st = H.want_stats(B, N, w.shape[0])
-            out = ops.conv2d(hid.reshape(B, Hh, Ww, -1), w, b, x2=t3.reshape(B, Hh, Ww, -1), ksize=1, pad=(0, 0), residual=x,
-                             n_out=w.shape[0], colstats=st)
+            st = H.want_stats(Bo, N, w.shape[0])
+            out = ops.conv2d(hid.reshape(Bo, Hh, Ww, -1), w, b, x2=t3.reshape(Bo, Hh, Ww, -1), ksize=1, pad=(0, 0), residual=x,
+                             n_out=w.shape[0], colstats=st, residual_rows=res_rows)
             if ops.WORK_COUNTER is not None:
                 inner = hid.shape[-1]
-                H.count_flops("gemm", 2.0 * B * N * C * (inner + C))
-                H.count_flops("gemm_bytes", 2.0 * B * N * (inner + 3 * C) + 2.0 * C * (inner + C))
+                H.count_flops("gemm", 2.0 * Bo * N * C * (inner + C))
+                H.count_flops("gemm_bytes", 2.0 * Bo * N * (inner + 3 * C) + 2.0 * C * (inner + C))
                 H.count_flops("gemm_launches", 1.0)
             return out
-        out = self.proj_out(t.reshape(B * N, -1), residual=x.reshape(B * N, C), rows_per_batch=N, colstats=True,
-                            x8=ops.mx8_of(t) if mx else None)
-        return H.carry_stats(out.reshape(B, Hh, Ww, C), out)
+        out = self.proj_out(t.reshape(Bo * N, -1), residual=x.reshape(B * N, C), rows_per_batch=N, colstats=True,
+                            x8=ops.mx8_of(t) if mx else None, residual_rows=res_rows)
+        return H.carry_stats(out.reshape(Bo, Hh, Ww, C), out)
 
     def _sources(self):
         lin2, po = self.transformer_blocks[-1].ff.net[2], self.proj_out
diff --git a/udifftext_amd/sgm/modules/diffusionmodules/openaimodel.py b/udifftext_amd/sgm/modules/diffusionmodules/openaimodel.py
--- a/udifftext_amd/sgm/modules/diffusionmodules/openaimodel.py
+++ b/udifftext_amd/sgm/modules/diffusionmodules/openaimodel.py
@@ -91,15 +91,19 @@
 
 class TimestepEmbedSequential(nn.Sequential, TimestepBlock):
     def forward(self, x, emb_rows=None, t_context=None, v_context=None, x2=None, t_kv=None, emit_map=False,
-                zero_ctx_rows=0, t_fused=None):
+                zero_ctx_rows=0, t_fused=None, pair=1):
         for layer in self:
             if isinstance(layer, ResBlock):
-                x = layer(x, emb_rows, x2=x2)
+                if pair > 1:
+                    with ops.launch_context(plan_scale=pair):
+                        x = layer(x, emb_rows, x2=x2)
+                else:
+                    x = layer(x, emb_rows, x2=x2)
                 x2 = None
             elif isinstance(layer, SpatialTransformer):
                 kv = t_kv[layer.st_index] if t_kv is not None else None
                 tf = t_fused[layer.st_index] if t_fused is not None else None
-                x = layer(x, t_context, v_context, t_kv=kv, emit_map=emit_map, zero_ctx_rows=zero_ctx_rows, t_fused=tf)
+                x = layer(x, t_context, v_context, t_kv=kv, emit_map=emit_map, zero_ctx_rows=zero_ctx_rows, t_fused=tf, pair=pair)
             else:
                 x = layer(x)
         return x
@@ -300,9 +304,18 @@
         return [st.prepare_fused(kv, out=(out[i] if out is not None else None))
                 for i, (st, kv) in enumerate(zip(self._transformers, t_kv))]
 
+    def pair_prefix_block(self, n_tokens: int, t_fused, emit_maps: bool = False):
+        if len(self.input_blocks) < 2:
+            return None
+        blk = self.input_blocks[1]
+        if len(blk) != 2 or not isinstance(blk[0], ResBlock) or not isinstance(blk[1], SpatialTransformer):
+            return None
+        tf = t_fused[blk[1].st_index] if t_fused is not None else None
+        return blk if blk[1].pair_prefix_ok(n_tokens, tf, emit_maps) else None
+
     def forward_nhwc(self, xin: torch.Tensor, emb_rows: torch.Tensor, t_kv: List[list], emit_maps: bool = False,
                      zero_ctx_rows: int = 0, t_fused: Optional[List[list]] = None, char_maps: Optional[torch.Tensor] = None,
-                     map_from: int = 0, map_layers=None) -> torch.Tensor:
+                     map_from: int = 0, map_layers=None, pair_shared: bool = False) -> torch.Tensor:
         asked = []
         if char_maps is not None:
             B, hl, wl, _ = xin.shape
@@ -320,9 +333,17 @@
         hs = []
         h = xin
         kw = dict(t_kv=t_kv, emit_map=emit_maps, zero_ctx_rows=zero_ctx_rows, t_fused=t_fused)
+        shared = None
+        if pair_shared and H.PAIR_PREFIX and char_maps is None and xin.shape[0] % 2 == 0 and 2 * int(zero_ctx_rows) == xin.shape[0]:
+            shared = self.pair_prefix_block(xin.shape[1] * xin.shape[2], t_fused, emit_maps)
         try:
-            for block in self.input_blocks:
-                h = block(h, emb_rows, **kw)
+            for i, block in enumerate(self.input_blocks):
+                if i == 1 and shared is not None:
+                    half = xin.shape[0] // 2
+                    h = block(H.first_samples(h, half), emb_rows[:half], pair=2, **kw)
+                    H.count_flops("pair_prefix_calls", 1)
+                else:
+                    h = block(h, emb_rows, **kw)
                 hs.append(h)
             h = self.middle_block(h, emb_rows, **kw)
             for block in self.output_blocks:
diff --git a/udifftext_amd/sgm/modules/diffusionmodules/sampling.py b/udifftext_amd/sgm/modules/diffusionmodules/sampling.py
--- a/udifftext_amd/sgm/modules/diffusionmodules/sampling.py
+++ b/udifftext_amd/sgm/modules/diffusionmodules/sampling.py
@@ -71,6 +71,27 @@
 def _all_zero(t: torch.Tensor) -> bool:
     flag = getattr(t, "_udt_all_zero", None)
     return bool(flag) if flag is not None else not bool(t.any())
+
+
+def _same_values(a, b) -> bool:
+    if a is b:
+        return True
+    if not (isinstance(a, torch.Tensor) and isinstance(b, torch.Tensor)):
+        return False
+    return (a.device == b.device and a.dtype == b.dtype and a.shape == b.shape and a.stride() == b.stride()
+            and a.data_ptr() == b.data_ptr())
+
+
+def pair_shares_prefix(cond: dict, uc: dict) -> bool:
+    if "concat" not in cond or "concat" not in uc:
+        return False
+    for k in set(cond) | set(uc):
+        if k == "t_crossattn" or k.startswith("_udt"):
+            continue
+        a, b = cond.get(k), uc.get(k)
+        if (isinstance(a, torch.Tensor) or isinstance(b, torch.Tensor)) and not _same_values(a, b):
+            return False
+    return True
 
 
 class Precond(NamedTuple):
@@ -253,6 +274,7 @@
         self.t_kv = self.unet.project_context(ctx)
         self.t_fused = self.unet.prepare_fused_tattn(self.t_kv)
         self.zero_ctx_rows = batch_size if self.pair and _all_zero(uc["t_crossattn"]) else 0
+        self.pair_shared = self.pair and self.zero_ctx_rows == batch_size and pair_shares_prefix(cond, uc)
         self.dual = self.pair and (DUAL_STREAM if two_streams is None else bool(two_streams))
         if self.dual:
             self.side = torch.cuda.Stream(device=dev)
@@ -305,7 +327,8 @@
         else:
             with ops.launch_context(cu_share=self.cu_share, workspace=self.ws):
                 eps = self.unet.forward_nhwc(self.xin, emb, self.t_kv, emit_maps=emit_maps, zero_ctx_rows=self.zero_ctx_rows,
-                                             t_fused=self.t_fused, char_maps=char_maps, map_from=self.B if self.pair else 0)
+                                             t_fused=self.t_fused, char_maps=char_maps, map_from=self.B if self.pair else 0,
+                                             pair_shared=self.pair_shared)
         return eps, k
 
     def step(self, x: torch.Tensor, sigma: float, sigma_next: float, emit_maps: bool = False,
@@ -396,6 +419,8 @@
         st = self.st
         zero_rows = st.B if st.pair and _all_zero(uc["t_crossattn"]) else 0
         if zero_rows != st.zero_ctx_rows or cond["concat"].shape[0] != st.B:
+            return False
+        if (st.pair and zero_rows == st.B and pair_shares_prefix(cond, uc)) != st.pair_shared:
             return False
         ctx = torch.cat((uc["t_crossattn"], cond["t_crossattn"]), 0) if st.pair else cond["t_crossattn"]
         for dst_list, src_list in zip(st.t_kv, st.unet.project_context(ctx)):
diff --git a/udifftext_amd/sgm/modules/hipnn.py b/udifftext_amd/sgm/modules/hipnn.py
--- a/udifftext_amd/sgm/modules/hipnn.py
+++ b/udifftext_amd/sgm/modules/hipnn.py
@@ -46,6 +46,17 @@
     return FP8_LINEARS and LN_GEMM and c % 128 == 0
 
 LN_GEMM = os.environ.get("UDT_LN_GEMM", "1") != "0" and os.environ.get("UDT_LEAN", "") != "0"
+
+
+PAIR_PREFIX = os.environ.get("UDT_PAIR_PREFIX", "1") != "0"
+
+
+def first_samples(x: torch.Tensor, n: int) -> torch.Tensor:
+    v = x[:n]
+    st = ops.gn_stats_of(x)
+    if st is not None:
+        v.gn_stats = ops.GnStats(st.data[:n * st.slots_per_sample], st.slots_per_sample)
+    return v
 
 
 def carry_stats(dst: torch.Tensor, src: torch.Tensor) -> torch.Tensor:
@@ -157,8 +168,9 @@
         return wq, cs, packing.pad_bias(self.bias)
 
     def forward(self, x, residual=None, flags: int = 0, out=None, rowvec=None, rows_per_batch: int = 0,
-                colstats: bool = False, x8=None, emit_q8: bool = False, emit_rowstats: bool = False):
+                colstats: bool = False, x8=None, emit_q8: bool = False, emit_rowstats: bool = False, residual_rows: int = 0):
         if x8 is not None:
+            assert residual_rows == 0
             wq, cs, b = self.packed_fp8()
             M = x8.data.shape[0]
             if colstats:
@@ -171,7 +183,7 @@
             rpb = rows_per_batch if rows_per_batch > 0 else x.shape[0]
             colstats = want_stats(x.shape[0] // rpb, rpb, w.shape[0])
         return ops.linear(x, w, b, residual=residual, flags=flags, out=out, rowvec=rowvec, rows_per_batch=rows_per_batch,
-                          colstats=bool(colstats), emit_q8=emit_q8, emit_rowstats=emit_rowstats)
+                          colstats=bool(colstats), emit_q8=emit_q8, emit_rowstats=emit_rowstats, residual_rows=residual_rows)
 
 
 class Conv2d(_Packed):
```

Result: no change. 10.55 images/s (-0.0%).
